# ELEKTRONN/ELEKTRONN2

Measured on AMD Instinct MI355X. Metric: training_input_voxels_per_sec, higher is better.
Workload: dtype f32; 1 GPU; neuro3d_lite (1,1,23,183,183)->(1,2,10,37,37) fwd+bwd+Adam, 1 sample/GPU; parallelism=dp1, hipgraph=True, steps_per_launch=10

## Files before the change

### elektronn2_amd/backend.py

```python
from __future__ import annotations

import ctypes as C
import os
from typing import Optional, Sequence

import numpy as np
import torch

_HERE = os.path.dirname(os.path.abspath(__file__))
LIB_PATH = os.environ.get("E2HIP_LIB") or os.path.join(_HERE, "libe2hip.so")

ACT = {"lin": 0, "linear": 0, "relu": 1, "tanh": 2, "sigmoid": 3, "sig": 3, "logistic": 3,
       "abs": 4, "elu": 5, "selu": 6, "soft+": 7}


class E2Error(RuntimeError):
    pass


POOL_MODE = {'avg': 1, 'sum': 2}


class Tensor5(C.Structure):
    _fields_ = [("ptr", C.c_void_p),
                ("n", C.c_int32), ("c", C.c_int32), ("d", C.c_int32),
                ("h", C.c_int32), ("w", C.c_int32),
                ("sn", C.c_int64), ("sc", C.c_int64), ("sd", C.c_int64),
                ("sh", C.c_int64)]


class Bf16Dst(C.Structure):
    _fields_ = [("cl", C.c_void_p), ("cl_kg", C.c_int32), ("cl_d", C.c_int32), ("cl_h", C.c_int32),
                ("cl_w", C.c_int32), ("cl_oz", C.c_int32), ("cl_oy", C.c_int32), ("cl_ox", C.c_int32),
                ("pl", C.c_void_p), ("pl_plane", C.c_int64), ("pl_pitch", C.c_int32)]


def bf16_dst(cl=None, cl_dims=None, cl_off=(0, 0, 0), pl=None, pl_plane=0, pl_pitch=0):
    d = Bf16Dst()
    d.cl = cl.data_ptr() if cl is not None else None
    if cl is not None:
        d.cl_kg, d.cl_d, d.cl_h, d.cl_w = (int(v) for v in cl_dims)
        d.cl_oz, d.cl_oy, d.cl_ox = (int(v) for v in cl_off)
    d.pl = pl.data_ptr() if pl is not None else None
    d.pl_plane, d.pl_pitch = int(pl_plane), int(pl_pitch)
    return d


class NllWeights(C.Structure):
    _fields_ = [("class_w", C.c_void_p), ("example_w", C.POINTER(Tensor5)),
                ("labelled", C.c_void_p), ("not_present", C.c_void_p)]


class LossTerm(C.Structure):
    _fields_ = [("kind", C.c_int), ("margin", C.c_void_p), ("scale_correction", C.c_void_p),
                ("subtract_label_entropy", C.c_int), ("sig_is_log", C.c_int)]


LOSS = {"squared": 0, "abs": 1, "binary_nll": 2, "gauss_nll": 3}
MAX_LOSS_TERMS = 8


def t5_shape(shape):
    n, c, d, h, w = (int(v) for v in shape)
    return Tensor5(None, n, c, d, h, w, c * d * h * w, d * h * w, h * w, w)


def _load():
    if not os.path.exists(LIB_PATH):
        raise E2Error(
            "libe2hip.so not found at %s -- build it with "
            "`python -c 'import __graft_entry__ as g; g.build()'` or "
            "`make -C elektronn2_amd/csrc`.  There is no CPU fallback." % LIB_PATH)
    lib = C.CDLL(LIB_PATH)
    P5 = C.POINTER(Tensor5)
    PW = C.POINTER(NllWeights)
    PL = C.POINTER(LossTerm)
    vp, i, sz, fp = C.c_void_p, C.c_int, C.c_size_t, C.c_void_p
    sig = {
        "e2_ctx_create": (C.c_int, [i, C.POINTER(vp)]),
        "e2_ctx_destroy": (C.c_int, [vp]),
        "e2_ctx_set_stream": (C.c_int, [vp, vp]),
        "e2_last_error": (C.c_char_p, []),
        "e2_version": (C.c_int, []),
        "e2_conv3d_workspace_bytes": (sz, [i, i, i, i, i]),
        "e2_conv3d_fwd": (C.c_int, [vp, P5, fp, i, i, i, i, P5, vp, sz]),
        "e2_conv3d_dgrad": (C.c_int, [vp, P5, fp, i, i, i, i, P5, vp, sz]),
        "e2_conv3d_pack": (C.c_int, [vp, fp, i, i, i, i, i, i, vp, sz]),
        "e2_conv3d_fwd_packed": (C.c_int, [vp, P5, vp, i, i, i, i, P5]),
        "e2_conv3d_dgrad_packed": (C.c_int, [vp, P5, vp, i, i, i, i, P5]),
        "e2_conv3d_fwd_packed_act": (C.c_int, [vp, P5, vp, i, i, i, i, fp, i, P5]),
        "e2_bias_act_bwd_out": (C.c_int, [vp, P5, P5, i, P5, fp]),
        "e2_conv3d_dgrad_packed_actbwd": (C.c_int, [vp, P5, vp, i, i, i, i, P5, i, fp, P5, i, i, i, fp]),
        "e2_conv3d_wgrad": (C.c_int, [vp, P5, P5, fp, i, i, i]),
        "e2_conv3d_wgrad_acc": (C.c_int, [vp, P5, P5, fp, i, i, i]),
        "e2_conv3d_wgrad_pad": (C.c_int, [vp, P5, P5, fp, i, i, i, i]),
        "e2_pack_job_bytes": (sz, []),
        "e2_pack_job_fill": (C.c_int, [vp, fp, vp, i, i, i, i, i, i]),
        "e2_pack_job_set_rows": (C.c_int, [vp, i]),
        "e2_pack_job_set_stride": (C.c_int, [vp, i]),
        "e2_set_image_rows": (C.c_int, [vp, i]),
        "e2_conv3d_pack_multi": (C.c_int, [vp, vp, i]),
        "e2_conv3d_pack_multi_ex": (C.c_int, [vp, vp, i, i]),
        "e2_head_supported": (C.c_int, [i, i]),
        "e2_head_fwd": (C.c_int, [vp, P5, fp, fp, i, P5, P5, fp]),
        "e2_head_bwd_workspace_bytes": (C.c_size_t, [i, i, i, i, i, i]),
        "e2_tail_supported": (C.c_int, [i, i, i]),
        "e2_tail_workspace_bytes": (C.c_size_t, [i, i, i, i, i, i, i]),
        "e2_tail_fwd_bwd": (C.c_int, [vp, P5, fp, fp, fp, i, fp, fp, i, P5, P5, P5, P5, i, P5, fp, fp,
                                      C.c_void_p, C.c_size_t, C.POINTER(C.c_int)]),
        "e2_tail_reduce": (C.c_int, [vp, C.c_void_p, i, i, i, fp, fp, fp, fp, fp, i, fp]),
        "e2_head_bwd": (C.c_int, [vp, P5, fp, P5, P5, fp, P5, i, fp, fp, fp, C.c_void_p,
                                  C.c_size_t]),
        "e2_malis_loss_weights": (C.c_int, [i, C.c_void_p, i, C.c_void_p, C.c_void_p,
                                            C.c_void_p, i, C.c_void_p]),
        "e2_malis_connected_components": (C.c_int, [i, i, C.c_void_p, C.c_void_p, C.c_void_p,
                                                    i, C.c_void_p]),
        "e2_warp_slice": (C.c_int, [vp, P5, C.POINTER(C.c_float), i, C.c_uint,
                                    C.POINTER(C.c_int), C.POINTER(C.c_float), P5]),
        "e2_grey_augment": (C.c_int, [vp, fp, C.c_size_t, C.c_float, C.c_float, C.c_float]),
        "e2_stream_fork": (C.c_int, [vp, C.c_void_p]),
        "e2_stream_join": (C.c_int, [vp, C.c_void_p]),
        "e2_conv1_supported": (C.c_int, [i, i, i, i, i, i, i]),
        "e2_conv1_pool_act_fwd": (C.c_int, [vp, P5, fp, fp, i, i, i, i, i, i, P5]),
        "e2_conv1_bwd_workspace_bytes": (C.c_size_t, [i, i, i, i, i, i, i]),
        "e2_conv1_pool_act_bwd": (C.c_int, [vp, P5, fp, fp, P5, i, i, i, i, i, fp, fp,
                                            C.c_void_p, C.c_size_t]),
        "e2_pool_bias_act_fwd": (C.c_int, [vp, P5, fp, i, i, i, i, P5]),
        "e2_conv3d_fwd_packed_parts": (C.c_int, [vp, P5, vp, i, i, i, i, P5, C.c_int64, i,
                                                 C.POINTER(C.c_int)]),
        "e2_conv3d_dgrad_packed_parts": (C.c_int, [vp, P5, vp, i, i, i, i, P5, C.c_int64, i,
                                                   C.POINTER(C.c_int)]),
        "e2_pool_bias_act_fwd_parts": (C.c_int, [vp, P5, C.c_int64, i, fp, i, i, i, i, P5]),
        "e2_pool_bias_act_bwd_parts": (C.c_int, [vp, P5, C.c_int64, i, P5, fp, i, i, i, i, P5, fp]),
        "e2_bias_act_bwd_out_parts": (C.c_int, [vp, P5, C.c_int64, i, P5, i, P5, fp]),
        "e2_pool_bias_act_bwd": (C.c_int, [vp, P5, P5, fp, i, i, i, i, P5, fp]),
        "e2_maxpool3d_fwd": (C.c_int, [vp, P5, i, i, i, P5]),
        "e2_maxpool3d_bwd": (C.c_int, [vp, P5, P5, i, i, i, P5, i]),
        "e2_pool3d_lin_fwd": (C.c_int, [vp, P5, i, i, i, i, i, i, i, P5]),
        "e2_pool3d_lin_bwd": (C.c_int, [vp, P5, i, i, i, i, i, i, i, P5, i]),
        "e2_upconv3d_workspace_bytes": (sz, [i, i, i, i, i, i, i, i, i]),
        "e2_upconv3d_fwd": (C.c_int, [vp, P5, fp, fp, i, i, i, i, i, P5, vp, sz]),
        "e2_upconv3d_bwd": (C.c_int, [vp, P5, fp, P5, P5, i, i, i, i, P5, fp, fp, vp, sz]),
        "e2_upconv3d_image_bytes": (sz, [i, i, i, i, i]),
        "e2_upconv3d_fwd_packed": (C.c_int, [vp, P5, fp, fp, i, i, i, i, i, P5]),
        "e2_upconv3d_bwd_packed": (C.c_int, [vp, P5, fp, P5, P5, i, i, i, i, P5, fp, fp, vp, sz, i]),
        "e2_transpose_ncdhw_to_ndhwc": (C.c_int, [vp, P5, fp]),
        "e2_transpose_ndhwc_to_ncdhw": (C.c_int, [vp, fp, P5]),
        "e2_copy5": (C.c_int, [vp, P5, P5, i]),
        "e2_set_dgrad_zinset": (C.c_int, [vp, i]),
        "e2_pad5": (C.c_int, [vp, P5, P5, i, i, i, C.c_float, i]),
        "e2_fill": (C.c_int, [vp, fp, sz, C.c_float]),
        "e2_softmax_nll_fwd": (C.c_int, [vp, P5, P5, P5, fp]),
        "e2_softmax_nll_bwd": (C.c_int, [vp, P5, P5, fp, P5, fp]),
        "e2_softmax_nll_fwd_w": (C.c_int, [vp, P5, P5, P5, fp, PW]),
        "e2_softmax_nll_bwd_w": (C.c_int, [vp, P5, P5, fp, P5, fp, PW]),
        "e2_softmax_nll_grouped_fwd": (C.c_int, [vp, P5, P5, P5, i, fp]),
        "e2_softmax_nll_grouped_bwd": (C.c_int, [vp, P5, P5, i, fp, P5, fp]),
        "e2_head_fwd_w": (C.c_int, [vp, P5, fp, fp, i, P5, P5, fp, PW]),
        "e2_head_bwd_w": (C.c_int, [vp, P5, fp, P5, P5, fp, P5, i, fp, fp, fp, C.c_void_p,
                                    sz, PW]),
        "e2_tail_fwd_bwd_w": (C.c_int, [vp, P5, fp, fp, fp, i, fp, fp, i, P5, P5, P5, P5, i, P5,
                                        fp, fp, C.c_void_p, sz, C.POINTER(C.c_int), PW]),
        "e2_malis_nll": (C.c_int, [vp, P5, fp, fp, fp, P5, fp]),
        "e2_fill_multi": (C.c_int, [vp, vp, vp, C.c_int, C.c_float]),
        "e2_set_skip_zero_fill": (C.c_int, [vp, C.c_int]),
        "e2_set_input_slack": (C.c_int, [vp, C.c_int]),
        "e2_conv_last_zero_fill": (C.c_int, [vp, C.POINTER(C.c_void_p), C.POINTER(C.c_size_t)]),
        "e2_set_mfma_dtype": (C.c_int, [vp, C.c_int]),
        "e2_set_tiling": (C.c_int, [vp, C.c_int, C.c_char_p]),
        "e2_last_launch": (C.c_int, [vp, C.c_char_p, C.c_int]),
        "e2_tiling_fallbacks": (C.c_uint, [vp]),
        "e2_conv3d_bf16_workspace_bytes": (sz, [i, i, i, i, i, i, i, i, i]),
        "e2_conv3d_fwd_bf16": (C.c_int, [vp, P5, fp, i, i, i, i, fp, i, P5, vp, sz]),
        "e2_conv3d_dgrad_bf16": (C.c_int, [vp, P5, fp, i, i, i, i, P5, vp, sz]),
        "e2_conv3d_wgrad_bf16_workspace_bytes": (sz, [i, i, i, i, i, i, i, i, i]),
        "e2_conv3d_wgrad_bf16": (C.c_int, [vp, P5, P5, fp, i, i, i, i, vp, sz]),
        "e2_conv3d_bf16_xkeep_bytes": (sz, [i, i, i, i, i, i, i]),
        "e2_conv3d_fwd_bf16_keep": (C.c_int, [vp, P5, fp, i, i, i, i, fp, i, P5, vp, sz, vp, sz]),
        "e2_conv3d_wgrad_bf16_xcl": (C.c_int, [vp, P5, vp, i, P5, fp, i, i, i, i, vp, sz]),
        "e2_pool_bias_act_bwd_bf16": (C.c_int, [vp, P5, C.c_int64, i, P5, fp, i, i, i, i, P5, fp, C.POINTER(Bf16Dst)]),
        "e2_pool_bias_act_fwd_bf16": (C.c_int, [vp, P5, C.c_int64, i, fp, i, i, i, i, P5, C.POINTER(Bf16Dst)]),
        "e2_conv1_pool_act_fwd_bf16": (C.c_int, [vp, P5, fp, fp, i, i, i, i, i, i, P5, vp, i]),
        "e2_conv3d_bf16_wb_bytes": (sz, [i, i, i, i, i, i, i, i, i]),
        "e2_bf16_wjob_bytes": (sz, []),
        "e2_bf16_wjob_fill": (C.c_int, [vp, fp, i, i, i, i, i, i, i, i, i, i, vp, sz]),
        "e2_conv3d_bf16_pack_w_multi": (C.c_int, [vp, vp, i]),
        "e2_conv3d_fwd_bf16_ex": (C.c_int, [vp, P5, fp, i, i, i, i, fp, i, P5, vp, sz, vp, sz, i, vp, vp, i]),
        "e2_conv3d_dgrad_bf16_ex": (C.c_int, [vp, P5, fp, i, i, i, i, P5, vp, sz, vp, vp]),
        "e2_conv3d_wgrad_bf16_geometry": (C.c_int, [i, i, i, i, i, i, i, i, i, C.POINTER(C.c_int64),
                                                    C.POINTER(C.c_size_t), C.POINTER(C.c_size_t)]),
        "e2_conv3d_wgrad_bf16_ex": (C.c_int, [vp, P5, vp, i, P5, vp, fp, fp, i, i, i, i, vp, sz]),
        "e2_dense_fwd": (C.c_int, [vp, fp, fp, fp, i, i, i]),
        "e2_dense_dgrad": (C.c_int, [vp, fp, fp, fp, i, i, i, i]),
        "e2_dense_wgrad": (C.c_int, [vp, fp, fp, fp, i, i, i, i]),
        "e2_batchnorm_act_fwd": (C.c_int, [vp, P5, fp, fp, fp, fp, i, i, i, P5, fp]),
        "e2_batchnorm_act_bwd": (C.c_int, [vp, P5, P5, fp, fp, fp, i, i, P5, fp, fp]),
        "e2_get_mfma_dtype": (C.c_int, [vp]),
        "e2_dropout_fwd": (C.c_int, [vp, P5, P5, i, fp, vp, C.c_uint32]),
        "e2_dropout_bwd": (C.c_int, [vp, P5, P5, i, fp, vp, C.c_uint32]),
        "e2_dropout_tick": (C.c_int, [vp, vp]),
        "e2_act_fwd": (C.c_int, [vp, P5, fp, i, P5]),
        "e2_act_bwd": (C.c_int, [vp, P5, P5, fp, i, P5, fp]),
        "e2_loss_partials": (sz, [vp, P5]),
        "e2_loss_fwd": (C.c_int, [vp, PL, P5, P5, P5, fp]),
        "e2_loss_mix": (C.c_int, [vp, i, PL, C.POINTER(C.c_void_p), C.POINTER(sz),
                                  C.POINTER(C.c_int64), fp, fp, fp, fp, fp]),
        "e2_loss_bwd": (C.c_int, [vp, PL, P5, P5, P5, fp, P5, P5, i]),
        "e2_adam_step": (C.c_int, [vp, fp, fp, fp, fp, sz, vp, fp, i, fp]),
        "e2_sgd_step": (C.c_int, [vp, fp, fp, fp, sz, vp, fp, i, fp]),
        "e2_set_loss_grad_mode": (C.c_int, [vp, i, fp]),
        "e2_upd_job_bytes": (sz, []),
        "e2_upd_rest_bytes": (sz, []),
        "e2_upd_job_fill": (C.c_int, [vp, C.c_long, vp, vp, i, i, i, i, i, C.c_float, i,
                                      C.POINTER(C.c_int), C.POINTER(C.c_size_t)]),
        "e2_upd_rest_fill": (C.c_int, [vp, C.c_long, C.c_long, C.c_float]),
        "e2_adam_pack_step": (C.c_int, [vp, fp, fp, fp, fp, vp, i, i, vp, i, fp, fp, C.c_float, i, sz]),
        "e2_adam_step_ex": (C.c_int, [vp, fp, fp, fp, fp, sz, vp, fp, i, fp, fp, C.c_float, i]),
        "e2_sgd_step_ex": (C.c_int, [vp, fp, fp, fp, sz, vp, fp, i, fp, fp, C.c_float, i]),
        "e2_step_prologue": (C.c_int, [vp, fp, i, C.c_size_t, fp, fp, i, fp, i, vp]),
        "e2_graph_begin": (C.c_int, [vp]),
        "e2_graph_end": (C.c_int, [vp, C.POINTER(vp)]),
        "e2_graph_launch": (C.c_int, [vp, vp]),
        "e2_graph_destroy": (C.c_int, [vp]),
        "e2_graph_debug_dot": (C.c_int, [vp, C.c_char_p, i]),
        "e2_event_create": (C.c_int, [C.POINTER(vp)]),
        "e2_event_record": (C.c_int, [vp, vp]),
        "e2_event_elapsed_ms": (C.c_int, [vp, vp, C.POINTER(C.c_float)]),
        "e2_event_destroy": (C.c_int, [vp]),
        "e2_stream_synchronize": (C.c_int, [vp]),
    }
    for name, (res, args) in sig.items():
        fn = getattr(lib, name)
        fn.restype = res
        fn.argtypes = args
    return lib, sorted(sig)


_lib, EXPORTED_SYMBOLS = _load()


def lib():
    return _lib


def _chk(rc: int, what: str):
    if rc != 0:
        msg = _lib.e2_last_error()
        raise E2Error("%s failed (rc=%d): %s" % (what, rc, msg.decode() if msg else "?"))


def t5(t: torch.Tensor) -> Tensor5:
    if t.dim() != 5:
        raise TypeError("expected a 5-D (b,f,z,x,y) tensor, got %s" % (tuple(t.shape),))
    if t.dtype != torch.float32:
        raise TypeError("expected float32, got %s" % t.dtype)
    if not t.is_cuda:
        raise E2Error("tensor is on %s; the HIP path needs a GPU tensor (no CPU fallback)"
                      % t.device)
    s = t.stride()
    if t.shape[4] > 1 and s[4] != 1:
        raise TypeError("innermost stride must be 1, got %s" % (s,))
    return Tensor5(t.data_ptr(), t.shape[0], t.shape[1], t.shape[2], t.shape[3],
                   t.shape[4], s[0], s[1], s[2], s[3])


def nll_weights(class_w=None, example_w=None, labelled=None, not_present=None):
    w = NllWeights()
    w._keep = (class_w, example_w, labelled, not_present)
    w.class_w = _fp(class_w)
    if example_w is not None:
        w._ew = t5(example_w)
        w.example_w = C.pointer(w._ew)
    w.labelled = _fp(labelled)
    w.not_present = _fp(not_present)
    return w


def loss_term(kind, margin=None, scale_correction=None, subtract_label_entropy=False,
              sig_is_log=False):
    if kind not in LOSS:
        raise ValueError("loss_term: unknown kind %r (one of %s)" % (kind, sorted(LOSS)))
    t = LossTerm()
    t._keep = (margin, scale_correction)
    t.kind = LOSS[kind]
    t.margin = _fp(margin)
    t.scale_correction = _fp(scale_correction)
    t.subtract_label_entropy = int(bool(subtract_label_entropy))
    t.sig_is_log = int(bool(sig_is_log))
    return t


def _fp(t: Optional[torch.Tensor]):
    if t is None:
        return None
    if t.dtype != torch.float32 or not t.is_cuda or not t.is_contiguous():
        raise TypeError("expected a contiguous float32 GPU tensor")
    return C.c_void_p(t.data_ptr())


class Context:

    def __init__(self, device: int = 0, stream: Optional[torch.cuda.Stream] = None):
        if not torch.cuda.is_available():
            raise E2Error("no GPU visible: the elektronn2_amd hot path is HIP-only")
        torch.cuda.set_device(device)
        h = C.c_void_p()
        _chk(_lib.e2_ctx_create(device, C.byref(h)), "e2_ctx_create")
        self.h = h
        self.device = torch.device("cuda", device)
        self.stream = None
        self.set_stream(stream if stream is not None else torch.cuda.current_stream(device))
        self._ws = {}

    def set_stream(self, stream: torch.cuda.Stream):
        self.stream = stream
        _chk(_lib.e2_ctx_set_stream(self.h, C.c_void_p(stream.cuda_stream)),
             "e2_ctx_set_stream")

    def stream_fork(self, side: torch.cuda.Stream):
        _chk(_lib.e2_stream_fork(self.h, C.c_void_p(side.cuda_stream)), "e2_stream_fork")

    def stream_join(self, side: torch.cuda.Stream):
        _chk(_lib.e2_stream_join(self.h, C.c_void_p(side.cuda_stream)), "e2_stream_join")

    def synchronize(self):
        _chk(_lib.e2_stream_synchronize(self.h), "e2_stream_synchronize")

    def workspace(self, key, nbytes: int) -> torch.Tensor:
        w = self._ws.get(key)
        if w is None or w.numel() * 4 < nbytes:
            w = torch.empty((nbytes + 3) // 4 + 64, dtype=torch.float32, device=self.device)
            self._ws[key] = w
        return w

    def conv_ws_bytes(self, cout, cin, k):
        return int(_lib.e2_conv3d_workspace_bytes(cout, cin, k[0], k[1], k[2]))

    def conv3d_fwd(self, x, w, y, ws=None):
        cout, cin, kd, kh, kw = w.shape
        nb = self.conv_ws_bytes(cout, cin, (kd, kh, kw))
        ws = ws if ws is not None else self.workspace("conv", nb)
        _chk(_lib.e2_conv3d_fwd(self.h, C.byref(t5(x)), _fp(w), cout, kd, kh, kw,
                                C.byref(t5(y)), C.c_void_p(ws.data_ptr()), ws.numel() * 4),
             "e2_conv3d_fwd")

    def conv3d_dgrad(self, dy_pad, w, dx, ws=None):
        cout, cin, kd, kh, kw = w.shape
        nb = self.conv_ws_bytes(cout, cin, (kd, kh, kw))
        ws = ws if ws is not None else self.workspace("conv", nb)
        _chk(_lib.e2_conv3d_dgrad(self.h, C.byref(t5(dy_pad)), _fp(w), cin, kd, kh, kw,
                                  C.byref(t5(dx)), C.c_void_p(ws.data_ptr()),
                                  ws.numel() * 4), "e2_conv3d_dgrad")

    def conv3d_pack(self, w, mode, ws):
        cout, cin, kd, kh, kw = w.shape
        _chk(_lib.e2_conv3d_pack(self.h, _fp(w), cout, cin, kd, kh, kw, mode,
                                 C.c_void_p(ws.data_ptr()), ws.numel() * 4),
             "e2_conv3d_pack")

    def conv3d_fwd_packed(self, x, wp, cout, k, y):
        _chk(_lib.e2_conv3d_fwd_packed(self.h, C.byref(t5(x)), C.c_void_p(wp.data_ptr()),
                                       cout, k[0], k[1], k[2], C.byref(t5(y))),
             "e2_conv3d_fwd_packed")

    def conv3d_dgrad_packed(self, dy_pad, wp, cin, k, dx):
        _chk(_lib.e2_conv3d_dgrad_packed(self.h, C.byref(t5(dy_pad)),
                                         C.c_void_p(wp.data_ptr()), cin, k[0], k[1], k[2],
                                         C.byref(t5(dx))), "e2_conv3d_dgrad_packed")

    def conv3d_fwd_packed_parts(self, x, wp, cout, k, y_parts):
        n = C.c_int(0)
        _chk(_lib.e2_conv3d_fwd_packed_parts(self.h, C.byref(t5(x)), C.c_void_p(wp.data_ptr()),
# ... 37 lines not shown

    def conv3d_dgrad_packed_actbwd(self, dy_pad, wp, cin, k, out_prev, act_prev, dy_pad_prev,
                                   pad_prev, dbias_prev, bias_prev=None):
        _chk(_lib.e2_conv3d_dgrad_packed_actbwd(
            self.h, C.byref(t5(dy_pad)), C.c_void_p(wp.data_ptr()), int(cin), int(k[0]),
            int(k[1]), int(k[2]), C.byref(t5(out_prev)), ACT[act_prev],
            _fp(bias_prev) if bias_prev is not None else None, C.byref(t5(dy_pad_prev)),
            int(pad_prev[0]), int(pad_prev[1]), int(pad_prev[2]),
            _fp(dbias_prev) if dbias_prev is not None else None),
            "e2_conv3d_dgrad_packed_actbwd")

    def bias_act_bwd_out(self, dout, out, act, dy, dbias):
        _chk(_lib.e2_bias_act_bwd_out(self.h, C.byref(t5(dout)), C.byref(t5(out)), ACT[act],
                                      C.byref(t5(dy)), _fp(dbias)), "e2_bias_act_bwd_out")

    def warp_slice(self, src, minv, perspective, nearest_mask, dest_off, src_off, dst):
        m = (C.c_float * 16)(*[float(v) for v in np.asarray(minv, np.float32).ravel()])
        do = (C.c_int * 3)(*[int(v) for v in dest_off])
        so = (C.c_float * 3)(*[float(v) for v in src_off])
        _chk(_lib.e2_warp_slice(self.h, C.byref(t5(src[None])), m, 1 if perspective else 0,
                                int(nearest_mask), do, so, C.byref(t5(dst[None]))),
             "e2_warp_slice")

    def grey_augment(self, chan, alpha, c, gamma):
        if not chan.is_contiguous():
            raise TypeError("grey_augment needs a dense channel")
        _chk(_lib.e2_grey_augment(self.h, _fp(chan), chan.numel(), float(alpha), float(c),
                                  float(gamma)), "e2_grey_augment")

    @staticmethod
    def head_supported(cin, ncls):
        return bool(_lib.e2_head_supported(int(cin), int(ncls)))

    def head_fwd(self, x, w, bias, target, probs, stats, weights=None):
        args = (self.h, C.byref(t5(x)), _fp(w), _fp(bias), probs.shape[1],
                C.byref(t5(target)) if target is not None else None,
                C.byref(t5(probs)), _fp(stats) if stats is not None else None)
        if weights is None:
            _chk(_lib.e2_head_fwd(*args), "e2_head_fwd")
        else:
            _chk(_lib.e2_head_fwd_w(*(args + (C.byref(weights),))), "e2_head_fwd_w")

    @staticmethod
    def head_bwd_ws_bytes(x_shape, ncls):
        n, cin, d, h, w = (int(v) for v in x_shape)
        return int(_lib.e2_head_bwd_workspace_bytes(n, cin, int(ncls), d, h, w))

    def head_bwd(self, x, w, probs, target, stats, dx, accumulate_dx, dw, dbias, loss_out,
                 ws=None, weights=None):
        if ws is None:
            ws = torch.empty(self.head_bwd_ws_bytes(x.shape, probs.shape[1]) // 4 + 16,
                             dtype=torch.float32, device=self.device)
        args = (self.h, C.byref(t5(x)), _fp(w), C.byref(t5(probs)),
                C.byref(t5(target)), _fp(stats),
                C.byref(t5(dx)) if dx is not None else None,
                1 if accumulate_dx else 0, _fp(dw), _fp(dbias),
                _fp(loss_out) if loss_out is not None else None,
                C.c_void_p(ws.data_ptr()), ws.numel() * 4)
        if weights is None:
            _chk(_lib.e2_head_bwd(*args), "e2_head_bwd")
        else:
            _chk(_lib.e2_head_bwd_w(*(args + (C.byref(weights),))), "e2_head_bwd_w")

    @staticmethod
    def tail_supported(c1, c2, ncls):
        return bool(_lib.e2_tail_supported(int(c1), int(c2), int(ncls)))

    @staticmethod
    def tail_ws_bytes(x_shape, c2, ncls):
        n, c1, d, h, w = (int(v) for v in x_shape)
        return int(_lib.e2_tail_workspace_bytes(n, c1, int(c2), int(ncls), d, h, w))

    def tail_fwd_bwd(self, x, wp_fwd, wp_dgrad, bias1, w_head, b_head, target, probs, dpre, dx,
                     stats, ws, gm_mode=0, gm_src=None, gm_bias=None, weights=None):
        n_slots = C.c_int(0)
        args = (self.h, C.byref(t5(x)), _fp(wp_fwd), _fp(wp_dgrad), _fp(bias1),
                dpre.shape[1], _fp(w_head), _fp(b_head), probs.shape[1],
                C.byref(t5(target)), C.byref(t5(probs)), C.byref(t5(dpre)),
                C.byref(t5(dx)) if dx is not None else None, int(gm_mode),
                C.byref(t5(gm_src)) if gm_src is not None else None,
                _fp(gm_bias), _fp(stats),
                C.c_void_p(ws.data_ptr()), ws.numel() * 4, C.byref(n_slots))
        if weights is None:
            _chk(_lib.e2_tail_fwd_bwd(*args), "e2_tail_fwd_bwd")
        else:
            _chk(_lib.e2_tail_fwd_bwd_w(*(args + (C.byref(weights),))), "e2_tail_fwd_bwd_w")
        return int(n_slots.value)

    def tail_reduce(self, ws, n_slots, c2, ncls, dw_head, db_head, db1, stats, loss_out,
                    db_parent=None):
        _chk(_lib.e2_tail_reduce(self.h, C.c_void_p(ws.data_ptr()), int(n_slots), int(c2),
                                 int(ncls), _fp(dw_head), _fp(db_head), _fp(db1), _fp(stats),
                                 _fp(loss_out) if loss_out is not None else None,
                                 0 if db_parent is None else int(db_parent.numel()),
                                 _fp(db_parent)), "e2_tail_reduce")

    def conv3d_wgrad(self, x, dy, dw, accumulate=False):
        kd, kh, kw = dw.shape[2:]
        fn = _lib.e2_conv3d_wgrad_acc if accumulate else _lib.e2_conv3d_wgrad
        _chk(fn(self.h, C.byref(t5(x)), C.byref(t5(dy)), _fp(dw), kd, kh, kw),
             "e2_conv3d_wgrad")

    def conv3d_wgrad_pad(self, x, dy_pad, dw, accumulate=False):
        kd, kh, kw = dw.shape[2:]
        _chk(_lib.e2_conv3d_wgrad_pad(self.h, C.byref(t5(x)), C.byref(t5(dy_pad)), _fp(dw),
                                      kd, kh, kw, 1 if accumulate else 0),
             "e2_conv3d_wgrad_pad")

    def set_image_rows(self, rows):
        _chk(_lib.e2_set_image_rows(self.h, int(rows or 0)), "e2_set_image_rows")

    def make_pack_jobs(self, jobs, rows=None, strides=None):
        rec = int(_lib.e2_pack_job_bytes())
        buf = (C.c_char * (rec * len(jobs)))()
        for n, (w, wp, mode) in enumerate(jobs):
            cout, cin, kd, kh, kw = w.shape
            _chk(_lib.e2_pack_job_fill(C.byref(buf, n * rec), _fp(w), C.c_void_p(wp.data_ptr()),
                                       cout, cin, kd, kh, kw, mode), "e2_pack_job_fill")
            if strides is not None and strides[n]:
                _chk(_lib.e2_pack_job_set_stride(C.byref(buf, n * rec), int(strides[n])), "e2_pack_job_set_stride")
            if rows is not None and rows[n]:
                _chk(_lib.e2_pack_job_set_rows(C.byref(buf, n * rec), int(rows[n])), "e2_pack_job_set_rows")
        host = torch.frombuffer(bytearray(buf), dtype=torch.uint8)
        dev = host.to(self.device)
        dev.max_taps = max(int(w.shape[2] * w.shape[3] * w.shape[4]) for w, _, _ in jobs)
        dev.keep = [(w, wp) for w, wp, _ in jobs]
        return dev, len(jobs)

    def conv3d_pack_multi(self, jobs_dev, njobs):
        _chk(_lib.e2_conv3d_pack_multi_ex(self.h, C.c_void_p(jobs_dev.data_ptr()), njobs,
                                          int(getattr(jobs_dev, 'max_taps', 248))),
             "e2_conv3d_pack_multi_ex")

    @staticmethod
    def conv1_supported(cin, k, pool):
        return bool(_lib.e2_conv1_supported(cin, k[0], k[1], k[2], pool[0], pool[1], pool[2]))

    def conv1_pool_act_fwd(self, x, w, bias, pool, act, out):
        _chk(_lib.e2_conv1_pool_act_fwd(self.h, C.byref(t5(x)), _fp(w), _fp(bias), w.shape[0],
                                        w.shape[3], w.shape[4], pool[1], pool[2], ACT[act],
                                        C.byref(t5(out))), "e2_conv1_pool_act_fwd")

    def conv1_pool_act_fwd_bf16(self, x, w, bias, pool, act, out, next_xb, next_kg):
        _chk(_lib.e2_conv1_pool_act_fwd_bf16(self.h, C.byref(t5(x)), _fp(w), _fp(bias), w.shape[0],
                                             w.shape[3], w.shape[4], pool[1], pool[2], ACT[act],
                                             C.byref(t5(out)), C.c_void_p(next_xb.data_ptr()),
                                             int(next_kg)), "e2_conv1_pool_act_fwd_bf16")

    @staticmethod
    def conv1_bwd_ws_bytes(dout_shape, k):
        n, cout, d, ho, wo = (int(v) for v in dout_shape)
        return int(_lib.e2_conv1_bwd_workspace_bytes(n, cout, d, ho, wo, k[1], k[2]))

    def conv1_pool_act_bwd(self, x, w, bias, dout, pool, act, dw, dbias, ws=None):
        if ws is None:
            ws = torch.empty(self.conv1_bwd_ws_bytes(dout.shape, w.shape[2:]) // 4 + 16,
                             dtype=torch.float32, device=self.device)
        _chk(_lib.e2_conv1_pool_act_bwd(self.h, C.byref(t5(x)), _fp(w), _fp(bias),
                                        C.byref(t5(dout)), w.shape[3], w.shape[4], pool[1],
                                        pool[2], ACT[act], _fp(dw), _fp(dbias),
                                        C.c_void_p(ws.data_ptr()), ws.numel() * 4),
             "e2_conv1_pool_act_bwd")

    def pool_bias_act_fwd(self, y, bias, pool, act, out):
        _chk(_lib.e2_pool_bias_act_fwd(self.h, C.byref(t5(y)), _fp(bias), pool[0], pool[1],
                                       pool[2], ACT[act], C.byref(t5(out))),
             "e2_pool_bias_act_fwd")

    def pool_bias_act_bwd(self, dout, y, bias, pool, act, dy, dbias):
        _chk(_lib.e2_pool_bias_act_bwd(self.h, C.byref(t5(dout)), C.byref(t5(y)), _fp(bias),
                                       pool[0], pool[1], pool[2], ACT[act], C.byref(t5(dy)),
                                       _fp(dbias)), "e2_pool_bias_act_bwd")

    def act_fwd(self, pre, bias, act, out):
        _chk(_lib.e2_act_fwd(self.h, C.byref(t5(pre)), _fp(bias), ACT[act], C.byref(t5(out))),
             "e2_act_fwd")

    def loss_partials(self, pred):
        n = int(_lib.e2_loss_partials(self.h, C.byref(t5(pred))))
        if n <= 0:
            raise E2Error("e2_loss_partials: empty prediction %s" % (tuple(pred.shape),))
        return n

    def loss_fwd(self, term, pred, sig, target, partials):
        if partials.numel() < 4 * self.loss_partials(pred):
            raise E2Error("loss_fwd: the partials slab is too small for this prediction")
        _chk(_lib.e2_loss_fwd(self.h, C.byref(term), C.byref(t5(pred)),
                              None if sig is None else C.byref(t5(sig)), C.byref(t5(target)),
                              _fp(partials)), "e2_loss_fwd")

    def loss_mix(self, terms, partials, n_tot, mix, coef, term_loss, count, loss_out):
        k = len(terms)
        if not (len(partials) == len(n_tot) == k):
            raise E2Error("loss_mix: %d terms, %d slabs, %d sizes" % (k, len(partials), len(n_tot)))
        if k > MAX_LOSS_TERMS:
            raise E2Error("loss_mix: %d terms, at most %d are supported" % (k, MAX_LOSS_TERMS))
        for t in (mix, coef, term_loss, count):
            if t.numel() < k:
                raise E2Error("loss_mix: mix / coef / term_loss / count need %d floats" % k)
        if loss_out.numel() < 1:
            raise E2Error("loss_mix: loss_out needs one float")
        ta = (LossTerm * max(k, 1))(*terms)
        pa = (C.c_void_p * max(k, 1))(*[_fp(p) for p in partials])
        ra = (C.c_size_t * max(k, 1))(*[int(p.numel()) // 4 for p in partials])
        na = (C.c_int64 * max(k, 1))(*[int(n) for n in n_tot])
        _chk(_lib.e2_loss_mix(self.h, k, ta, pa, ra, na, _fp(mix), _fp(coef), _fp(term_loss),
                              _fp(count), _fp(loss_out)), "e2_loss_mix")

    def loss_bwd(self, term, pred, sig, target, coef, dpred, dsig=None, accumulate=False):
        opt = lambda t: None if t is None else C.byref(t5(t))
        _chk(_lib.e2_loss_bwd(self.h, C.byref(term), C.byref(t5(pred)), opt(sig),
                              C.byref(t5(target)), _fp(coef), opt(dpred), opt(dsig),
                              int(bool(accumulate))), "e2_loss_bwd")

    def act_bwd(self, dout, pre, bias, act, dpre, dbias):
        _chk(_lib.e2_act_bwd(self.h, C.byref(t5(dout)), C.byref(t5(pre)), _fp(bias), ACT[act],
                             C.byref(t5(dpre)), _fp(dbias)), "e2_act_bwd")

    def maxpool3d_fwd(self, x, pool, out):
        _chk(_lib.e2_maxpool3d_fwd(self.h, C.byref(t5(x)), pool[0], pool[1], pool[2],
                                   C.byref(t5(out))), "e2_maxpool3d_fwd")

    def maxpool3d_bwd(self, dout, x, pool, dx, accumulate=False):
        _chk(_lib.e2_maxpool3d_bwd(self.h, C.byref(t5(dout)), C.byref(t5(x)), pool[0],
                                   pool[1], pool[2], C.byref(t5(dx)), int(accumulate)),
             "e2_maxpool3d_bwd")

    def pool_lin_fwd(self, x, pool, stride, mode, out):
        _chk(_lib.e2_pool3d_lin_fwd(self.h, C.byref(t5(x)), int(pool[0]), int(pool[1]),
                                    int(pool[2]), int(stride[0]), int(stride[1]), int(stride[2]),
                                    POOL_MODE.get(mode, mode), C.byref(t5(out))),
             "e2_pool3d_lin_fwd")

    def pool_lin_bwd(self, dout, pool, stride, mode, dx, accumulate=False):
        _chk(_lib.e2_pool3d_lin_bwd(self.h, C.byref(t5(dout)), int(pool[0]), int(pool[1]),
                                    int(pool[2]), int(stride[0]), int(stride[1]), int(stride[2]),
                                    POOL_MODE.get(mode, mode), C.byref(t5(dx)),
                                    int(bool(accumulate))), "e2_pool3d_lin_bwd")

    def upconv_ws_bytes(self, cout, cin, pool, x_shape):
        return int(_lib.e2_upconv3d_workspace_bytes(cout, cin, pool[0], pool[1], pool[2],
                                                    x_shape[0], x_shape[2], x_shape[3],
                                                    x_shape[4]))

    def upconv3d_fwd(self, x, w, bias, pool, act, y, ws=None):
        cout, cin = w.shape[:2]
        nb = self.upconv_ws_bytes(cout, cin, pool, x.shape)
        ws = ws if ws is not None else self.workspace("upconv", nb)
        _chk(_lib.e2_upconv3d_fwd(self.h, C.byref(t5(x)), _fp(w), _fp(bias), cout, pool[0],
                                  pool[1], pool[2], ACT[act], C.byref(t5(y)),
                                  C.c_void_p(ws.data_ptr()), ws.numel() * 4),
             "e2_upconv3d_fwd")

    def upconv3d_bwd(self, x, w, y, dout, pool, act, dx, dw, dbias, ws=None):
        cout, cin = w.shape[:2]
        nb = self.upconv_ws_bytes(cout, cin, pool, x.shape)
        ws = ws if ws is not None else self.workspace("upconv", nb)
        _chk(_lib.e2_upconv3d_bwd(self.h, C.byref(t5(x)), _fp(w), C.byref(t5(y)),
                                  C.byref(t5(dout)), pool[0], pool[1], pool[2], ACT[act],
                                  C.byref(t5(dx)) if dx is not None else None,
                                  _fp(dw), _fp(dbias), C.c_void_p(ws.data_ptr()),
                                  ws.numel() * 4), "e2_upconv3d_bwd")

    @staticmethod
    def upconv_image_bytes(cout, cin, pool):
        return int(_lib.e2_upconv3d_image_bytes(int(cout), int(cin), pool[0], pool[1], pool[2]))

    def upconv3d_fwd_packed(self, x, wp_fwd, bias, cout, pool, act, y):
        _chk(_lib.e2_upconv3d_fwd_packed(self.h, C.byref(t5(x)), _fp(wp_fwd), _fp(bias), int(cout),
                                         pool[0], pool[1], pool[2], ACT[act], C.byref(t5(y))),
             "e2_upconv3d_fwd_packed")

    def upconv3d_bwd_packed(self, x, wp_dgrad, y, dout, pool, act, dx, dw, dbias, ws,
                            accumulate=False):
        _chk(_lib.e2_upconv3d_bwd_packed(self.h, C.byref(t5(x)), _fp(wp_dgrad), C.byref(t5(y)),
                                         C.byref(t5(dout)), pool[0], pool[1], pool[2], ACT[act],
                                         C.byref(t5(dx)) if dx is not None else None,
                                         _fp(dw), _fp(dbias), C.c_void_p(ws.data_ptr()),
                                         ws.numel() * 4, int(bool(accumulate))),
             "e2_upconv3d_bwd_packed")

    def to_ndhwc(self, src, dst):
        _chk(_lib.e2_transpose_ncdhw_to_ndhwc(self.h, C.byref(t5(src)), _fp(dst)),
             "e2_transpose_ncdhw_to_ndhwc")

    def to_ncdhw(self, src, dst):
        _chk(_lib.e2_transpose_ndhwc_to_ncdhw(self.h, _fp(src), C.byref(t5(dst))),
             "e2_transpose_ndhwc_to_ncdhw")

    def copy5(self, src, dst, accumulate=False):
        _chk(_lib.e2_copy5(self.h, C.byref(t5(src)), C.byref(t5(dst)), int(accumulate)),
             "e2_copy5")

    def set_dgrad_zinset(self, planes):
        _chk(_lib.e2_set_dgrad_zinset(self.h, int(planes)), "e2_set_dgrad_zinset")

    def pad5(self, src, dst, pad, value=0.0, frame_only=False):
        _chk(_lib.e2_pad5(self.h, C.byref(t5(src)) if src is not None else None, C.byref(t5(dst)),
                          int(pad[0]), int(pad[1]), int(pad[2]), float(value), int(bool(frame_only))),
             "e2_pad5")

    def fill(self, t, value=0.0):
        if not t.is_contiguous():
            raise TypeError("fill needs a contiguous tensor")
        _chk(_lib.e2_fill(self.h, C.c_void_p(t.data_ptr()), t.numel(), float(value)),
             "e2_fill")

    @staticmethod
    def _drop_state(state):
        if not (isinstance(state, torch.Tensor) and state.is_cuda and state.dtype == torch.int32
                and state.numel() >= 4 and state.is_contiguous() and state.data_ptr() % 16 == 0):
            raise TypeError("dropout state: four int32 words in device memory, 16-byte aligned")
        return C.c_void_p(state.data_ptr())

    def dropout_fwd(self, x, out, rate, state, stream, feature_mode=False):
# ... 171 lines not shown
        _chk(_lib.e2_conv3d_wgrad_bf16_geometry(n, cin, d, h, w, int(cout), k[0], k[1], k[2],
                                                C.byref(pd), C.byref(db), C.byref(sb)),
             "e2_conv3d_wgrad_bf16_geometry")
        return int(pd.value), int(db.value), int(sb.value)

    def conv3d_wgrad_bf16_ex(self, x, dy, dw, accumulate=False, ws=None, xcl=None, dyc=None, sums=None):
        cout, cin, kd, kh, kw = dw.shape
        if ws is None and not (xcl is not None and dyc is not None and sums is not None):
            ws = self.workspace("wgrad_bf16", self.wgrad_bf16_ws_bytes(x.shape, cout, (kd, kh, kw)))
        _chk(_lib.e2_conv3d_wgrad_bf16_ex(
            self.h, C.byref(t5(x)), C.c_void_p(xcl.data_ptr()) if xcl is not None else None,
            (cin + 15) // 16 * 2, C.byref(t5(dy)),
            C.c_void_p(dyc.data_ptr()) if dyc is not None else None, _fp(sums), _fp(dw),
            kd, kh, kw, int(accumulate),
            C.c_void_p(ws.data_ptr()) if ws is not None else None,
            ws.numel() * ws.element_size() if ws is not None else 0), "e2_conv3d_wgrad_bf16_ex")

    def pool_bias_act_bwd_bf16(self, dout, src, bias, pool, act, dy, dbias, dst, parts=1, part_stride=0):
        dyv = t5(dy) if dy is not None else Tensor5(None, 0, 0, 0, 0, 0, 0, 0, 0, 0)
        _chk(_lib.e2_pool_bias_act_bwd_bf16(self.h, C.byref(t5(dout)), int(part_stride), int(parts),
                                            C.byref(t5(src)), _fp(bias), pool[0], pool[1], pool[2],
                                            ACT[act], C.byref(dyv), _fp(dbias), C.byref(dst)),
             "e2_pool_bias_act_bwd_bf16")

    def pool_bias_act_fwd_bf16(self, y, bias, pool, act, out, dst, parts=1, part_stride=0):
        _chk(_lib.e2_pool_bias_act_fwd_bf16(self.h, C.byref(t5(y)), int(part_stride), int(parts),
                                            _fp(bias), pool[0], pool[1], pool[2], ACT[act],
                                            C.byref(t5(out)), C.byref(dst)),
             "e2_pool_bias_act_fwd_bf16")

    def dense_fwd(self, x, w, y):
        n, k = x.shape
        _chk(_lib.e2_dense_fwd(self.h, _fp(x), _fp(w), _fp(y), n, k, w.shape[1]), "e2_dense_fwd")

    def dense_dgrad(self, dy, w, dx, accumulate=False):
        n, m = dy.shape
        _chk(_lib.e2_dense_dgrad(self.h, _fp(dy), _fp(w), _fp(dx), n, w.shape[0], m,
                                 int(accumulate)), "e2_dense_dgrad")

    def dense_wgrad(self, x, dy, dw, accumulate=False):
        n, k = x.shape
        _chk(_lib.e2_dense_wgrad(self.h, _fp(x), _fp(dy), _fp(dw), n, k, dy.shape[1],
                                 int(accumulate)), "e2_dense_wgrad")

    def batchnorm_act_fwd(self, x, gamma, bias, run_mean, run_std, train, update_running, act,
                          out, save=None):
        _chk(_lib.e2_batchnorm_act_fwd(self.h, C.byref(t5(x)), _fp(gamma), _fp(bias),
                                       _fp(run_mean), _fp(run_std), int(bool(train)),
                                       int(bool(update_running)), ACT[act], C.byref(t5(out)),
                                       _fp(save)), "e2_batchnorm_act_fwd")

    def batchnorm_act_bwd(self, dout, x, gamma, bias, save, train, act, dx, dgamma, dbias):
        _chk(_lib.e2_batchnorm_act_bwd(self.h, C.byref(t5(dout)), C.byref(t5(x)), _fp(gamma),
                                       _fp(bias), _fp(save), int(bool(train)), ACT[act],
                                       C.byref(t5(dx)) if dx is not None else None,
                                       _fp(dgamma), _fp(dbias)), "e2_batchnorm_act_bwd")

    def set_tiling(self, kind, cfg):
        code = {'igemm': 0, 'wgrad': 1}[kind]
        _chk(_lib.e2_set_tiling(self.h, code, (cfg or "").encode()), "e2_set_tiling")
        self._tiling = getattr(self, '_tiling', {})
        self._tiling[kind] = cfg or ""

    def last_launch(self):
        buf = C.create_string_buffer(160)
        _chk(_lib.e2_last_launch(self.h, buf, 160), "e2_last_launch")
        parts = buf.value.decode().split(" ")
        return tuple(parts) if len(parts) == 3 else None

    def tiling_fallbacks(self):
        return int(_lib.e2_tiling_fallbacks(self.h))

    def bf16_memory_form(self):
        return getattr(self, '_tiling', {}).get('igemm', '').startswith('32,')

    def set_mfma_dtype(self, dtype):
        code = {'f32': 0, 'float32': 0, 'bf16': 1, 'bfloat16': 1}.get(dtype)
        if code is None:
            raise ValueError("mfma dtype must be 'f32' or 'bf16', got %r" % (dtype,))
        _chk(_lib.e2_set_mfma_dtype(self.h, code), "e2_set_mfma_dtype")
        self._mfma = 'bf16' if code else 'f32'

    @property
    def mfma_dtype(self):
        m = getattr(self, '_mfma', None)
        if m is None:
            m = self._mfma = 'bf16' if _lib.e2_get_mfma_dtype(self.h) == 1 else 'f32'
        return m

    def malis_nll(self, probs, pos, neg, norm, dlogits, loss_sum):
        _chk(_lib.e2_malis_nll(self.h, C.byref(t5(probs)), _fp(pos), _fp(neg), _fp(norm),
                               C.byref(t5(dlogits)) if dlogits is not None else None,
                               _fp(loss_sum)), "e2_malis_nll")

    def set_loss_grad_mode(self, sum_mode, count_out=None):
        _chk(_lib.e2_set_loss_grad_mode(self.h, int(bool(sum_mode)), _fp(count_out)),
             "e2_set_loss_grad_mode")

    def adam_step(self, p, g, m, s, seg_off, seg_reg, hyper, gdiv=None, gmul=1.0, zero_g=False):
        _chk(_lib.e2_adam_step_ex(self.h, _fp(p), _fp(g), _fp(m), _fp(s), p.numel(),
                                  C.c_void_p(seg_off.data_ptr()), _fp(seg_reg),
                                  seg_reg.numel(), _fp(hyper), _fp(gdiv), float(gmul),
                                  int(bool(zero_g))), "e2_adam_step_ex")

    def make_upd_jobs(self, jobs, rests):
        rj, rr = int(_lib.e2_upd_job_bytes()), int(_lib.e2_upd_rest_bytes())
        bj = (C.c_char * max(rj * len(jobs), 1))()
        br = (C.c_char * max(rr * len(rests), 1))()
        tile0, lds = 0, 16
        keep = []
        for n, (off, wf, wd_, shape, reg) in enumerate(jobs):
            nt, lb = C.c_int(), C.c_size_t()
            cout, cin, kd, kh, kw = (int(v) for v in shape)
            _chk(_lib.e2_upd_job_fill(C.byref(bj, n * rj), int(off),
                                      C.c_void_p(wf.data_ptr()) if wf is not None else None,
                                      C.c_void_p(wd_.data_ptr()) if wd_ is not None else None,
                                      cout, cin, kd, kh, kw, float(reg), tile0, C.byref(nt), C.byref(lb)),
                 "e2_upd_job_fill")
            tile0 += nt.value
            lds = max(lds, int(lb.value))
            keep += [wf, wd_]
        for n, (off, cnt, reg) in enumerate(rests):
            _chk(_lib.e2_upd_rest_fill(C.byref(br, n * rr), int(off), int(cnt), float(reg)), "e2_upd_rest_fill")
        return dict(jobs=torch.frombuffer(bytearray(bj), dtype=torch.uint8).to(self.device), njobs=len(jobs),
                    ntiles=tile0, rest=torch.frombuffer(bytearray(br), dtype=torch.uint8).to(self.device),
                    nrest=len(rests), lds=lds, keep=keep)

    def adam_pack_step(self, p, g, m, s, upd, hyper, gdiv=None, gmul=1.0, zero_g=False):
        _chk(_lib.e2_adam_pack_step(self.h, _fp(p), _fp(g), _fp(m), _fp(s),
                                    C.c_void_p(upd['jobs'].data_ptr()), upd['njobs'], upd['ntiles'],
                                    C.c_void_p(upd['rest'].data_ptr()), upd['nrest'], _fp(hyper),
                                    _fp(gdiv), float(gmul), int(bool(zero_g)), upd['lds']),
             "e2_adam_pack_step")

    def sgd_step(self, p, g, d, seg_off, seg_reg, hyper, gdiv=None, gmul=1.0, zero_g=False):
        _chk(_lib.e2_sgd_step_ex(self.h, _fp(p), _fp(g), _fp(d), p.numel(),
                                 C.c_void_p(seg_off.data_ptr()), _fp(seg_reg),
                                 seg_reg.numel(), _fp(hyper), _fp(gdiv), float(gmul),
                                 int(bool(zero_g))), "e2_sgd_step_ex")

    def step_prologue(self, state, ring=None, dst=None, src=None, hist=None):
        assert state.dtype == torch.int64 and state.numel() >= 2 and state.is_contiguous()
        if ring is not None:
            assert ring.dim() == 2 and ring.is_contiguous() and ring.dtype == torch.float32
            assert dst is not None and dst.is_contiguous() and dst.numel() >= ring.shape[1]
        if hist is not None:
            assert hist.dim() == 2 and hist.is_contiguous() and src is not None and src.numel() >= hist.shape[1]
        _chk(_lib.e2_step_prologue(self.h, _fp(ring), int(ring.shape[0]) if ring is not None else 0,
                                   int(ring.shape[1]) if ring is not None else 0, _fp(dst), _fp(src),
                                   int(hist.shape[1]) if hist is not None else 0, _fp(hist),
                                   int(hist.shape[0]) if hist is not None else 0,
                                   C.c_void_p(state.data_ptr())), "e2_step_prologue")

    def graph_begin(self):
        _chk(_lib.e2_graph_begin(self.h), "e2_graph_begin")

    def graph_end(self):
        g = C.c_void_p()
        _chk(_lib.e2_graph_end(self.h, C.byref(g)), "e2_graph_end")
        return g

    def graph_launch(self, g):
        _chk(_lib.e2_graph_launch(self.h, g), "e2_graph_launch")

    def graph_destroy(self, g):
        _chk(_lib.e2_graph_destroy(g), "e2_graph_destroy")

    def graph_debug_dot(self, g, path, verbose=True):
        _chk(_lib.e2_graph_debug_dot(g, str(path).encode(), 1 if verbose else 0), "e2_graph_debug_dot")

    def event(self):
        e = C.c_void_p()
        _chk(_lib.e2_event_create(C.byref(e)), "e2_event_create")
        return e

    def record(self, e):
        _chk(_lib.e2_event_record(self.h, e), "e2_event_record")

    def elapsed_ms(self, e0, e1) -> float:
        ms = C.c_float()
        _chk(_lib.e2_event_elapsed_ms(e0, e1, C.byref(ms)), "e2_event_elapsed_ms")
        return float(ms.value)
```

### elektronn2_amd/csrc/conv_first.hip

```cpp
#include "common.hpp"
#include <algorithm>

struct First {
  const float* x;
  const float* w;
  const float* bias;
  float* out;
  const float* dout;
  float* dw;
  float* dbias;
  int N, Cout, D, Ho, Wo;
  long xsN, xsD, xsH;
  long osN, osC, osD, osH;
  int act;
  int tilesX, tilesY;
};

template <int KH, int KW, int PY, int PX>
__device__ __forceinline__ float first_conv(const float (&win)[PY + KH - 1][PX + KW - 1],
                                            const float* __restrict__ wc, int a, int b) {
  float s = 0.f;
#pragma unroll
  for (int ty = 0; ty < KH; ++ty)
#pragma unroll
// ... 100 lines not shown
      for (int i = 0; i < 16; ++i) {
        const int t = t0 + i;
        float acc = 0.f;
        if (t < T) {
          const int ty = t / KW, tx = t % KW;
#pragma unroll
          for (int a = 0; a < PY; ++a)
#pragma unroll
            for (int b = 0; b < PX; ++b)
              acc = fmaf((c[a][b] == m) ? g : 0.f, win[a + ty][b + tx], acc);
        }
        v[i] = acc;
      }
      ff_butterfly16(v, lane);
      const int l15 = lane & 15;
      const int tap = t0 + ((l15 & 1) << 3 | (l15 & 2) << 1 | (l15 & 4) >> 1 | (l15 & 8) >> 3);
      if (tap < T) rb[grp][tap] = v[0];
    }
    float gs = g;
#pragma unroll
    for (int o = 8; o > 0; o >>= 1) gs += __shfl_xor(gs, o, 64);
    if ((lane & 15) == 0) rb[grp][T] = gs;
    __syncthreads();
    if (threadIdx.x <= T) {
      float sum = 0.f;
#pragma unroll
      for (int k = 0; k < 16; ++k) sum += rb[k][threadIdx.x];
      part[((long)tile * p.Cout + co) * (T + 1) + threadIdx.x] = sum;
    }
  }
}

__global__ __launch_bounds__(256) void first_bwd_reduce_kernel(const float* __restrict__ part,
                                                               int nTiles, int Cout, int T,
                                                               float* dw, float* dbias) {
  const int per = (nTiles + gridDim.y - 1) / gridDim.y;
  const int t0 = blockIdx.y * per, t1 = min(t0 + per, nTiles);
  const int idx = blockIdx.x * blockDim.x + threadIdx.x;
  const int total = Cout * (T + 1);
  if (idx >= total) return;
  float s = 0.f;
  for (int t = t0; t < t1; ++t) s += part[(long)t * total + idx];
  const int co = idx / (T + 1), k = idx - co * (T + 1);
  if (s != 0.f) {
    if (k < T) unsafeAtomicAdd(dw + co * T + (T - 1 - k), s);
    else unsafeAtomicAdd(dbias + co, s);
  }
}

__global__ __launch_bounds__(256) void first_bwd_reduce_sm_kernel(const float* __restrict__ part,
                                                                  int nSlots, int Cout, int T,
                                                                  float* dw, float* dbias) {
  const int idx = blockIdx.x * 4 + (threadIdx.x >> 6), lane = threadIdx.x & 63;
  if (idx >= Cout * (T + 1)) return;
  const float* row = part + (long)idx * nSlots;
  float s = 0.f;
#pragma unroll 4
  for (int b = lane; b < nSlots; b += 64) s += row[b];
#pragma unroll
  for (int o = 32; o > 0; o >>= 1) s += __shfl_xor(s, o, 64);
  if (lane != 0) return;
  const int co = idx / (T + 1), k = idx - co * (T + 1);
  if (k < T) dw[co * T + (T - 1 - k)] += s;
  else dbias[co] += s;
}

int e2i_firstm_mg(int cout);
size_t e2i_firstm_ws_floats(long nTiles, int cout, int T);
int e2i_firstm_fwd(e2_ctx*, int v, const e2_tensor5* x, const float* w, const float* bias, int cout,
                   int py, int px, int act, const e2_tensor5* out, void* next_xb, int next_kg);
int e2i_firstm_bwd(e2_ctx*, int v, const e2_tensor5* x, const float* w, const float* bias,
                   const e2_tensor5* dout, int py, int px, int act, float* part, int* nslots);

static int first_supported(int kd, int kh, int kw, int pz, int py, int px) {
  if (kd != 1 || pz != 1) return 0;
  if (kh == 4 && kw == 4 && py == 2 && px == 2) return 1;
  if (kh == 6 && kw == 6 && py == 2 && px == 2) return 2;
  if (kh == 3 && kw == 3 && py == 1 && px == 1) return 3;
  return 0;
}

extern "C" int e2_conv1_supported(int cin, int kd, int kh, int kw, int pz, int py, int px) {
  return cin == 1 && first_supported(kd, kh, kw, pz, py, px) != 0;
}

static int first_fill(First& p, const e2_tensor5* x, const e2_tensor5* o, int cout, int kh,
                      int kw, int py, int px, const char* name) {
  E2_REQUIRE(x && x->ptr && o && o->ptr, "%s: null tensor", name);
  E2_REQUIRE(x->c == 1, "%s: needs exactly one input channel", name);
  E2_REQUIRE(o->n == x->n && o->c == cout && o->d == x->d &&
                 o->h == (x->h - kh + 1) / py && o->w == (x->w - kw + 1) / px &&
                 (x->h - kh + 1) % py == 0 && (x->w - kw + 1) % px == 0,
             "%s: pooled output is (%d,%d,%d,%d,%d), input (%d,1,%d,%d,%d), kernel %dx%d pool %dx%d",
             name, o->n, o->c, o->d, o->h, o->w, x->n, x->d, x->h, x->w, kh, kw, py, px);
  p.x = x->ptr;
  p.N = x->n; p.Cout = cout; p.D = x->d; p.Ho = o->h; p.Wo = o->w;
  p.xsN = x->sn; p.xsD = x->sd; p.xsH = x->sh;
  p.osN = o->sn; p.osC = o->sc; p.osD = o->sd; p.osH = o->sh;
  p.tilesX = e2_cdiv(o->w, 32);
  p.tilesY = e2_cdiv(o->h, 8);
  return 0;
}

static int conv1_fwd(e2_ctx* ctx, const e2_tensor5* x, const float* w, const float* bias, int cout,
                     int kh, int kw, int py, int px, int act, const e2_tensor5* out, void* next_xb,
                     int next_kg);

extern "C" int e2_conv1_pool_act_fwd(e2_ctx* ctx, const e2_tensor5* x, const float* w,
                                     const float* bias, int cout, int kh, int kw, int py,
                                     int px, int act, const e2_tensor5* out) {
  return conv1_fwd(ctx, x, w, bias, cout, kh, kw, py, px, act, out, nullptr, 0);
}

extern "C" int e2_conv1_pool_act_fwd_bf16(e2_ctx* ctx, const e2_tensor5* x, const float* w,
                                          const float* bias, int cout, int kh, int kw, int py,
                                          int px, int act, const e2_tensor5* out, void* next_xb,
                                          int next_kg) {
  E2_REQUIRE(next_xb, "conv1_pool_act_fwd_bf16: null copy");
  return conv1_fwd(ctx, x, w, bias, cout, kh, kw, py, px, act, out, next_xb, next_kg);
}

static int conv1_fwd(e2_ctx* ctx, const e2_tensor5* x, const float* w, const float* bias, int cout,
                     int kh, int kw, int py, int px, int act, const e2_tensor5* out, void* next_xb,
                     int next_kg) {
  E2_REQUIRE(ctx && w && bias, "conv1_pool_act_fwd: null argument");
  const int v = first_supported(1, kh, kw, 1, py, px);
  E2_REQUIRE(v, "conv1_pool_act_fwd: unsupported kernel/pool %dx%d / %dx%d", kh, kw, py, px);
  First p{};
  if (int rc = first_fill(p, x, out, cout, kh, kw, py, px, "conv1_pool_act_fwd")) return rc;
  p.w = w; p.bias = bias; p.out = out->ptr; p.act = act;
  if (e2i_firstm_mg(cout) && (next_xb || !e2_dbg_env("E2_FIRST_VALU")))
    return e2i_firstm_fwd(ctx, v, x, w, bias, cout, py, px, act, out, next_xb, next_kg);
  E2_REQUIRE(!next_xb, "conv1_pool_act_fwd_bf16: %d output channels (matrix-core form: <= 32)", cout);
  const long nTiles = (long)p.N * p.D * p.tilesY * p.tilesX;
  const int grid = (int)std::min<long>(nTiles, ctx->num_cu * 8);
  if (v == 1)
    hipLaunchKernelGGL((first_fwd_kernel<4, 4, 2, 2>), dim3(grid), dim3(256), 0, ctx->stream, p, (int)nTiles);
  else if (v == 2)
    hipLaunchKernelGGL((first_fwd_kernel<6, 6, 2, 2>), dim3(grid), dim3(256), 0, ctx->stream, p, (int)nTiles);
  else
    hipLaunchKernelGGL((first_fwd_kernel<3, 3, 1, 1>), dim3(grid), dim3(256), 0, ctx->stream, p, (int)nTiles);
  E2_CHECK_HIP(hipGetLastError());
  return 0;
}

extern "C" size_t e2_conv1_bwd_workspace_bytes(int n, int cout, int d, int ho, int wo, int kh,
                                               int kw) {
  const long tiles = (long)n * d * e2_cdiv(ho, 8) * e2_cdiv(wo, 32);
  const long tilesM = (long)n * d * e2_cdiv(ho, 4) * e2_cdiv(wo * 2, 64);
  const size_t valu = (size_t)tiles * cout * (kh * kw + 1);
  return sizeof(float) * std::max(valu, e2i_firstm_ws_floats(tilesM, cout, kh * kw));
}

extern "C" int e2_conv1_pool_act_bwd(e2_ctx* ctx, const e2_tensor5* x, const float* w,
                                     const float* bias, const e2_tensor5* dout, int kh, int kw,
                                     int py, int px, int act, float* dw, float* dbias,
                                     void* ws, size_t ws_bytes) {
  E2_REQUIRE(ctx && w && bias && dw && dbias && ws, "conv1_pool_act_bwd: null argument");
  const int v = first_supported(1, kh, kw, 1, py, px);
  E2_REQUIRE(v, "conv1_pool_act_bwd: unsupported kernel/pool %dx%d / %dx%d", kh, kw, py, px);
  First p{};
  if (int rc = first_fill(p, x, dout, dout ? dout->c : 0, kh, kw, py, px, "conv1_pool_act_bwd"))
    return rc;
  p.w = w; p.bias = bias; p.dout = dout->ptr; p.dw = dw; p.dbias = dbias; p.act = act;
  const long nTiles = (long)p.N * p.D * p.tilesY * p.tilesX;
  E2_REQUIRE(nTiles < (1L << 31), "conv1_pool_act_bwd: too many tiles");
  E2_REQUIRE(ws_bytes >= e2_conv1_bwd_workspace_bytes(p.N, p.Cout, p.D, p.Ho, p.Wo, kh, kw),
             "conv1_pool_act_bwd: workspace too small");
  float* part = (float*)ws;
  if (e2i_firstm_mg(p.Cout) && !e2_dbg_env("E2_FIRST_VALU")) {
    int nslots = 0;
    if (int rc = e2i_firstm_bwd(ctx, v, x, w, bias, dout, py, px, act, part, &nslots)) return rc;
    const int T = kh * kw, total = p.Cout * (T + 1);
    hipLaunchKernelGGL(first_bwd_reduce_sm_kernel, dim3(e2_cdiv(total, 4)), dim3(256), 0, ctx->stream,
                       part, nslots, p.Cout, T, dw, dbias);
    E2_CHECK_HIP(hipGetLastError());
    return 0;
  }
  if (v == 1)
    hipLaunchKernelGGL((first_bwd_kernel<4, 4, 2, 2>), dim3((int)nTiles), dim3(256), 0, ctx->stream, p, part);
  else if (v == 2)
    hipLaunchKernelGGL((first_bwd_kernel<6, 6, 2, 2>), dim3((int)nTiles), dim3(256), 0, ctx->stream, p, part);
  else
    hipLaunchKernelGGL((first_bwd_kernel<3, 3, 1, 1>), dim3((int)nTiles), dim3(256), 0, ctx->stream, p, part);
  E2_CHECK_HIP(hipGetLastError());
  const int T = kh * kw, total = p.Cout * (T + 1);
  const int slices = (int)std::min<long>(nTiles, 64);
  hipLaunchKernelGGL(first_bwd_reduce_kernel, dim3(e2_cdiv(total, 256), slices), dim3(256), 0,
                     ctx->stream, part, (int)nTiles, p.Cout, T, dw, dbias);
  E2_CHECK_HIP(hipGetLastError());
  return 0;
}
```

### elektronn2_amd/neuromancer/loss.py

```python
from __future__ import annotations

import numpy as np

from .graphutils import TaggedShape, floatX
from .node_basic import Node, Sym
from .variables import VariableParam

__all__ = ['Softmax', 'MultinoulliNLL', 'MalisNLL', 'SquaredLoss', 'AbsLoss', 'BinaryNLL',
           'GaussianNLL', 'AggregateLoss', 'Classification', 'Errors']

MAX_LOSS_TERMS = 8

EPS = 1e-5


class Softmax(Node):
    def __init__(self, parent, n_class='auto', n_indep=1, name="softmax", print_repr=True):
        super(Softmax, self).__init__(parent, name, print_repr)
        n_f = parent.shape['f']
        if hasattr(parent, 'activation_func'):
            if parent.activation_func != 'lin':
                raise ValueError("The parent of a Softmax-node must have a "
                                 "linear activation function.")
        if n_class == 'auto':
# ... 65 lines not shown
                parents.append(extra)
        super(MultinoulliNLL, self).__init__(parents, name, print_repr)
        if not isinstance(pred, Softmax):
            raise ValueError("The prob input to a MultinoulliNLL-node must be "
                             "a Softmax-Node.")
        if pred.n_indep != 1 and (len(parents) > 2 or cw_param is not None):
            raise NotImplementedError("MultinoulliNLL over n_indep > 1 takes the plain sparse "
                                      "target only: the other options have no defined meaning "
                                      "for several independent softmaxes")
        if weakness:
            raise NotImplementedError("weak training (weakness != 0) is outside the HIP "
                                      "hot path")
        if not target_is_sparse:
            raise NotImplementedError("dense (one-hot) targets are outside the HIP hot path")
        self.target = target
        self.pred = pred
        self.axis = pred.shape.tag2index('f')
        self.n_class = pred.n_class
        self.n_indep = pred.n_indep
        self.target_is_sparse = target_is_sparse
        k = self.n_class
        if self.n_indep != 1:
            want = tuple(self.n_indep if t == 'f' else s
                         for s, t in zip(pred.shape.shape, pred.shape.tags))
            if tuple(target.shape.tags) != tuple(pred.shape.tags) or \
                    tuple(target.shape.shape) != want:
                raise ValueError("MultinoulliNLL over %i independent softmaxes: the sparse target "
                                 "must be %s (one class id per softmax) for the prediction %s, "
                                 "got %s" % (self.n_indep, want, pred.shape, target.shape))
        if cw_param is not None:
            if cw_param.shape != (k,):
                raise ValueError("class_weights: %i values given, the prediction has %i "
                                 "classes" % (int(np.prod(cw_param.shape)), k))
            self.params['class_weights'] = cw_param
            class_weights = cw_param
        elif class_weights is not None:
            if tuple(class_weights.shape.tags) != ('f',) or \
                    tuple(class_weights.shape.shape) != (k,):
                raise ValueError("class_weights node: an Input((%i,), 'f') is needed, got %s"
                                 % (k, class_weights.shape))
        for what, m in (('mask_class_labeled', mask_class_labeled),
                        ('mask_class_not_present', mask_class_not_present)):
            if m is not None and (tuple(m.shape.tags) != ('b', 'f') or m.shape['f'] != k
                                  or m.shape['b'] != pred.shape['b']):
                raise ValueError("%s: an Input((%r, %i), 'b,f') is needed, got %s"
                                 % (what, pred.shape['b'], k, m.shape))
        if example_weights is not None:
            tags = tuple(t for t in pred.shape.tags if t != 'f')
            shape = tuple(s for s, t in zip(pred.shape.shape, pred.shape.tags) if t != 'f')
            if tuple(example_weights.shape.tags) != tags or \
                    tuple(example_weights.shape.shape) != shape:
                raise ValueError("example_weights: an Input(%s, '%s') is needed (the target's "
                                 "shape without the class axis), got %s"
                                 % (shape, ",".join(tags), example_weights.shape))
        self.class_weights = class_weights
        self.example_weights = example_weights
        self.weakness = 0
        self.mask_class_labeled = mask_class_labeled
        self.mask_class_not_present = mask_class_not_present

    @property
    def weighted(self):
        return any(v is not None for v in (self.class_weights, self.example_weights,
                                           self.mask_class_labeled,
                                           self.mask_class_not_present))

    def _weights(self, plan):
        if not self.weighted:
            return None
        w = plan.scratch.get((self, 'weights'))
        if w is None:
            from .. import backend
            cw = self.class_weights
            if isinstance(cw, VariableParam):
                cw = plan.param(cw).reshape(-1)
            elif cw is not None:
                cw = plan.out[cw].reshape(-1)
            dev = lambda node: None if node is None else plan.out[node]
            lab, npr = dev(self.mask_class_labeled), dev(self.mask_class_not_present)
            w = backend.nll_weights(class_w=cw, example_w=dev(self.example_weights),
                                    labelled=None if lab is None else lab.reshape(lab.shape[0], -1),
                                    not_present=None if npr is None else npr.reshape(npr.shape[0], -1))
            plan.scratch[self, 'weights'] = w
        return w

    def _calc_shape(self):
        self.shape = self.parent[0].shape.updateshape(self.axis, 1)

    def _calc_comp_cost(self):
        self.computational_cost = self.parent[0].shape.stripnone_prod

    def _plan_alloc(self, plan):
        plan.scratch[self.pred, 'fused_nll'] = True
        plan.scratch[self, 'loss'] = plan.zeros_flat(1)
        head = self.pred._head(plan)
        if head is not None and plan.training and self._tail(plan) is None:
            nb = plan.ctx.head_bwd_ws_bytes(plan.out_shape(head.parent), self.n_class)
            plan.scratch[self, 'head_ws'] = plan.empty_flat(nb // 4 + 16)
        plan.out[self] = None

    def _tail(self, plan):
        head = self.pred._head(plan)
        if head is None:
            return None
        c = head.parent
        f = getattr(c, '_tail', None)
        t = f(plan) if f is not None else None
        return c if (t is not None and t[2] is self) else None

    def _plan_fwd(self, plan):
        stats = plan.scratch[self.pred, 'stats']
        tail = self._tail(plan)
        if tail is not None:
            head = self.pred._head(plan)
            par = tail.parent
            plan.join_side()
            dx = plan.grad[par] if plan.needs_grad(par) else None
            gm = tail._tail_gm(plan) if dx is not None else None
            kw = {}
            if gm is not None:
                dx = plan.scratch[par, 'dy']
                kw = dict(gm_mode=gm[0], gm_src=gm[1], gm_bias=gm[2])
            with plan.loss_grad_mode():
                plan.scratch[self, 'tail_slots'] = plan.ctx.tail_fwd_bwd(
                    plan.out[par], plan.scratch[tail, 'wp_f'], plan.scratch.get((tail, 'wp_d')),
                    plan.param(tail.b), plan.param(head.w).reshape(head.n_f, -1),
                    plan.param(head.b), plan.out[self.target], plan.out[self.pred],
                    plan.scratch[tail, 'dy'], dx, stats, plan.scratch[tail, 'tail_ws'],
                    weights=self._weights(plan), **kw)
            return
        plan.zero_early(stats)
        head = self.pred._head(plan)
        if head is not None:
            plan.ctx.head_fwd(plan.out[head.parent], plan.param(head.w), plan.param(head.b),
                              plan.out[self.target], plan.out[self.pred], stats,
                              weights=self._weights(plan))
            return
        if self.n_indep != 1:
            plan.ctx.softmax_nll_grouped_fwd(plan.out[self.pred.parent], plan.out[self.target],
                                             plan.out[self.pred], self.n_indep, stats)
            return
        plan.ctx.softmax_nll_fwd(plan.out[self.pred.parent], plan.out[self.target],
                                 plan.out[self.pred], stats, weights=self._weights(plan))

    def _plan_bwd(self, plan):
        with plan.loss_grad_mode():
            self._plan_bwd_launches(plan)

    def _plan_bwd_launches(self, plan):
        head = self.pred._head(plan)
        tail = self._tail(plan)
        if tail is not None:
            par = tail.parent
            gm = tail._tail_gm(plan) if plan.needs_grad(par) else None
            plan.ctx.tail_reduce(plan.scratch[tail, 'tail_ws'], plan.scratch[self, 'tail_slots'],
                                 tail.n_f, head.n_f, plan.pgrad(head.w).reshape(head.n_f, -1),
                                 plan.pgrad(head.b), plan.pgrad(tail.b),
                                 plan.scratch[self.pred, 'stats'], plan.scratch[self, 'loss'],
                                 db_parent=plan.pgrad(par.b) if gm is not None else None)
            return
        if head is not None:
            dst, first = (plan.grad_slot(head.parent) if plan.needs_grad(head.parent)
                          else (None, True))
            plan.ctx.head_bwd(plan.out[head.parent], plan.param(head.w), plan.out[self.pred],
                              plan.out[self.target], plan.scratch[self.pred, 'stats'], dst,
                              not first, plan.pgrad(head.w), plan.pgrad(head.b),
                              plan.scratch[self, 'loss'], ws=plan.scratch[self, 'head_ws'],
                              weights=self._weights(plan))
            return
        logits = self.pred.parent
        dst, first = plan.grad_slot(logits)
        if not first:
            raise NotImplementedError("logits consumed by several nodes")
        if self.n_indep != 1:
            plan.ctx.softmax_nll_grouped_bwd(plan.out[self.pred], plan.out[self.target],
                                             self.n_indep, plan.scratch[self.pred, 'stats'], dst,
                                             plan.scratch[self, 'loss'])
            return
        plan.ctx.softmax_nll_bwd(plan.out[self.pred], plan.out[self.target],
                                 plan.scratch[self.pred, 'stats'], dst,
                                 plan.scratch[self, 'loss'], weights=self._weights(plan))

    def loss_value(self, plan):
        s = plan.scratch[self.pred, 'stats']
        return s[0] / (s[1] + EPS)


class MalisNLL(Node):

    def __init__(self, pred, aff_gt, seg_gt, nhood, unrestrict_neg=True, class_weights=None,
                 example_weights=None, name="nll", print_repr=True):
        super(MalisNLL, self).__init__([pred, aff_gt, seg_gt], name, print_repr)
        if not isinstance(pred, Softmax):
            raise ValueError("The prob input to a MultinoulliNLL-node must be "
                             "a Softmax-Node.")
        if pred.shape['b'] != 1:
            raise NotImplementedError("Malis can only be used with batch size 1.")
        if class_weights is not None or example_weights is not None:
            raise NotImplementedError("class / example weights are outside the HIP hot path")
        if pred.n_class != 2:
            raise NotImplementedError("MalisNLL needs 2-class softmaxes (one per edge)")
        self.aff_gt = aff_gt
        self.seg_gt = seg_gt
        self.pred = pred
        self.nhood = np.asarray(nhood, dtype=np.int32)
        if self.nhood.shape != (pred.n_indep, 3):
            raise ValueError("nhood must be (%i, 3) for this prediction" % pred.n_indep)
        self.unrestrict_neg = unrestrict_neg
        self.axis = pred.shape.tag2index('f')
        self.n_class = pred.n_class
        self.n_indep = pred.n_indep
        self.class_weights = None
        self.example_weights = None
        self.rand_index = self.false_splits = self.false_merges = None
        self.pos_count = self.neg_count = None

    def _calc_shape(self):
        self.shape = self.parent[0].shape.updateshape(self.axis, 1)

    def _calc_comp_cost(self):
        self.computational_cost = self.parent[0].shape.stripnone_prod

    def _plan_alloc(self, plan):
        plan.scratch[self.pred, 'loss_writes_dlogits'] = True
        sh = plan.out_shape(self.pred)
        n = self.n_indep * int(np.prod(sh[2:]))
        plan.scratch[self, 'pos'] = plan.zeros_flat(n)
        plan.scratch[self, 'neg'] = plan.zeros_flat(n)
        plan.scratch[self, 'norm'] = plan.zeros_flat(4)
        plan.scratch[self, 'loss'] = plan.zeros_flat(1)
        plan.out[self] = None

    def _plan_fwd(self, plan):
        pass

    def _plan_host(self, plan):
        import torch
        from .. import malis
        plan.stream.synchronize()
        probs = plan.out[self.pred]
        aff = probs[0, 1::2].cpu().numpy()
        aff_gt = plan.out[self.aff_gt][0].cpu().numpy().astype(np.int16)
        seg_gt = plan.out[self.seg_gt][0, 0].cpu().numpy().astype(np.int32)
        pos, neg = malis.malis_weights(aff, aff_gt, seg_gt, self.nhood, self.unrestrict_neg)
        n_pos, n_neg = float(pos.sum(dtype=np.float64)), float(neg.sum(dtype=np.float64))
        n_tot = n_pos + n_neg
        norm = np.array([1.0 / (n_tot + EPS), n_tot, n_pos, n_neg], np.float32)
        plan.scratch[self, 'pos'].copy_(torch.from_numpy(pos.astype(np.float32).ravel()))
        plan.scratch[self, 'neg'].copy_(torch.from_numpy(neg.astype(np.float32).ravel()))
        plan.scratch[self, 'norm'].copy_(torch.from_numpy(norm))
        self.pos_count, self.neg_count = pos, neg
        self.false_splits = int(pos[aff < 0.5].sum(dtype=np.uint64))
        self.false_merges = int(neg[aff > 0.5].sum(dtype=np.uint64))
        self.rand_index = np.float32((self.false_splits + self.false_merges) / (n_tot + EPS))

    def _launch(self, plan, dlogits):
        plan.ctx.fill(plan.scratch[self, 'loss'], 0.0)
        plan.ctx.malis_nll(plan.out[self.pred], plan.scratch[self, 'pos'],
                           plan.scratch[self, 'neg'], plan.scratch[self, 'norm'], dlogits,
                           plan.scratch[self, 'loss'])

    def _plan_fwd_post(self, plan):
        if not plan.training:
            self._launch(plan, None)

    def _plan_bwd(self, plan):
        logits = self.pred.parent
        dst, first = plan.grad_slot(logits)
        if not first:
            raise NotImplementedError("logits consumed by several nodes")
        self._launch(plan, dst)

    def loss_value(self, plan):
        return plan.scratch[self, 'loss'][0]


class _ElementLoss(Node):
    kind = None

    def _check_shapes(self, pred, others):
        if 's' in pred.shape.tags:
            raise NotImplementedError("%s: the 's' sample axis is outside the HIP hot path"
                                      % type(self).__name__)
        for what, n in others:
            if tuple(n.shape.shape) != tuple(pred.shape.shape) or \
                    tuple(n.shape.tags) != tuple(pred.shape.tags):
                raise ValueError("%s: the %s must have the prediction's shape %s, got %s"
                                 % (type(self).__name__, what, pred.shape, n.shape))
        self._last_plan = None

    def _calc_comp_cost(self):
        self.computational_cost = self.parent[0].shape.stripnone_prod

    def _views(self, plan):
        return plan.out[self.pred], None, plan.out[self.target]

    def _grad_targets(self):
        return (self.pred,)

    def _term(self, plan):
        t = plan.scratch.get((self, 'term'))
        if t is None:
            from .. import backend
            dev = lambda p: None if p is None else plan.param(p).reshape(-1)
            t = backend.loss_term(self.kind, margin=dev(getattr(self, 'margin', None)),
                                  scale_correction=dev(getattr(self, 'scale_correction', None)),
# ... 266 lines not shown
```

### elektronn2_amd/neuromancer/neural.py

```python
from __future__ import annotations

import logging

import numpy as np

from .graphutils import floatX, TaggedShape
from .. import autotune
from . import bf16_ahead
from .node_basic import Node, Concat, Add, Sym
from .variables import VariableWeight, ConstantParam, VariableParam

logger = logging.getLogger('elektronn2log')

__all__ = ['Conv', 'UpConv', 'Pool', 'Crop', 'Pad', 'AutoMerge', 'UpConvMerge', 'NeuralLayer',
           'FragmentsToDense', 'Perceptron']

_PLAIN_ACTS = ('relu', 'lin', 'linear')
_HIP_ACTS = _PLAIN_ACTS + ('tanh', 'sigmoid', 'sig', 'logistic', 'abs', 'elu', 'selu', 'soft+')


def check_activation(activation_func):
    if activation_func not in _HIP_ACTS:
        raise NotImplementedError("activation_func=%r: only %s are on the HIP hot path"
                                  % (activation_func, _HIP_ACTS))
# ... 531 lines not shown
        if not any(q):
            return dyp
        D, H, W = dyp.shape[2:]
        return dyp[:, :, q[0]:D - q[0], q[1]:H - q[1], q[2]:W - q[2]]

    def _sig_wgrad(self, plan):
        x, dy = self._x(plan), plan.scratch[self, 'dy']
        return (self.n_f, self.parent.shape['f']) + tuple(self._k3) + tuple(dy.shape[2:]) + \
            (x.stride(3), dy.stride(3))

    def _need_f32_dy(self, plan):
        b = plan.bf16a.get((self, 'dy'))
        if b is not None and not b['want_f32'] and plan._dy_ready.get(self):
            raise RuntimeError("bf16 mode: the tiling of a gradient launch of %s changed after its "
                               "operands were planned as bf16 images only (re-build the plan)" % self.name)

    def _bf16_fwd(self, plan, x, out, bias=None, act='lin'):
        ctx = plan.ctx
        a = plan.bf16a.get((self, 'fwd'))
        w5 = self._w5(plan.param(self.w))
        if a is None or a['tile'] != ctx.current_tiling('igemm'):
            ctx.conv3d_fwd_bf16(x, w5, out, bias=bias, act=act, ws=plan.bf16_ws(self),
                                xkeep=plan.bf16_xkeep(self))
            return
        nx = bf16_ahead.next_image(plan, self) if bias is not None else None
        plan.ensure_wb()
        ctx.conv3d_fwd_bf16_ex(x, w5, out, bias=bias, act=act, ws=plan.bf16_ws(self),
                               xkeep=plan.bf16_xkeep(self), x_ready=plan._xb_ready.get(self, False),
                               wb=a['wb'] if plan._wb_ready else None,
                               next_xb=nx[0] if nx else None, next_kg=nx[1] if nx else 0)
        if nx:
            plan._xb_ready[nx[2]] = True

    def _plan_fwd(self, plan):
        ctx = plan.ctx
        if self._fused_head(plan) is not None:
            return
        x = self._x(plan)
        if plan.scratch.get((self, 'xf_launch')):
            ctx.pad5(plan.out[self.parent], x, self._q3)
        if self._fused_first(plan):
            nx = bf16_ahead.next_image(plan, self)
            if nx is not None:
                ctx.conv1_pool_act_fwd_bf16(x, self._w5(plan.param(self.w)), plan.param(self.b),
                                            self._p3, self.activation_func, plan.out[self], nx[0], nx[1])
                plan._xb_ready[nx[2]] = True
            else:
                ctx.conv1_pool_act_fwd(x, self._w5(plan.param(self.w)), plan.param(self.b), self._p3,
                                       self.activation_func, plan.out[self])
            return
        if self._tail(plan) is not None:
            return
        wp = plan.scratch[self, 'wp_f']
        plan.join_side()
        cin = self.parent.shape['f']
        if self._fused_act(plan):
            out = plan.out[self]
            sig = (2, self.n_f, cin) + tuple(self._k3) + tuple(out.shape[2:]) + \
                (x.stride(3),)
            def fwd_act():
                if ctx.bf16_memory_form():
                    self._bf16_fwd(plan, x, out, bias=plan.param(self.b), act=self.activation_func)
                    plan.bf16_xkeep_valid(self, True)
                else:
                    plan.bf16_xkeep_valid(self, False)
                    with plan.image(wp):
                        ctx.conv3d_fwd_packed_act(x, wp, self.n_f, self._k3, plan.param(self.b),
                                                  self.activation_func, out)
            plan.tuned('igemm', sig,
                       autotune.igemm_candidates(self.n_f, cin, self._k3,
                                                 out.shape[2:], split_k=False) +
                       plan.bf16_cands(cin), fwd_act)
            return
        y = plan.scratch[self, 'y']
        sig = (0, self.n_f, cin) + tuple(self._k3) + tuple(y.shape[2:]) + \
            (x.stride(3),)
        yp = plan.scratch[self, 'y_parts']
        got = [1]

        def fwd_plain():
            plan.bf16_xkeep_valid(self, ctx.bf16_memory_form())
            if ctx.bf16_memory_form():
                self._bf16_fwd(plan, x, y)
                got[0] = 1
            elif yp.shape[0] > 1:
                with plan.image(wp):
                    got[0] = ctx.conv3d_fwd_packed_parts(x, wp, self.n_f, self._k3, yp)
            else:
                with plan.image(wp):
                    ctx.conv3d_fwd_packed(x, wp, self.n_f, self._k3, y)
        plan.tuned('igemm', sig,
                   autotune.igemm_candidates(self.n_f, cin, self._k3, y.shape[2:]) +
                   plan.bf16_cands(cin), fwd_plain, out=y)
        y_nparts = got[0]
        if self._bn():
            lin = y
            if any(p != 1 for p in self._p3):
                if self._mfp_pool():
                    raise NotImplementedError("MFP together with batch normalisation")
                lin = plan.scratch[self, 'lin']
                ctx.maxpool3d_fwd(y, self._p3, lin)
            train = self.batch_normalisation == 'train'
            pre = plan.scratch.get((self, 'pre'), plan.out[self])
            ctx.batchnorm_act_fwd(lin, plan.param(self.gamma), plan.param(self.b),
                                  plan.param(self.mean), plan.param(self.std), train,
                                  train and plan.step in ('SGD', 'Adam'), self._lin_act(),
                                  pre, plan.scratch[self, 'bn_save'])
            if not self._plain_act():
                ctx.act_fwd(pre, None, self.activation_func, plan.out[self])
            return
        if self._mfp_pool():
            from itertools import product
            out, n_in = plan.out[self], y.shape[0]
            pz, px, py = self._p3
            D, H, W = y.shape[2:]
            for i, (iz, ix, iy) in enumerate(product(range(pz), range(px), range(py))):
                src = y[:, :, iz:iz + D - pz + 1, ix:ix + H - px + 1, iy:iy + W - py + 1]
                ctx.pool_bias_act_fwd(src, plan.param(self.b), self._p3,
                                      self._lin_act(), out[i * n_in:(i + 1) * n_in])
            if not self._plain_act():
                ctx.act_fwd(out, None, self.activation_func, out)
            return
        if not self._plain_act():
            out = plan.out[self]
            if all(p == 1 for p in self._p3):
                ctx.act_fwd(y, plan.param(self.b), self.activation_func, out)
            elif (self, 'lin') in plan.scratch:
                ctx.maxpool3d_fwd(y, self._p3, plan.scratch[self, 'lin'])
                ctx.act_fwd(plan.scratch[self, 'lin'], plan.param(self.b), self.activation_func, out)
            else:
                ctx.pool_bias_act_fwd(y, plan.param(self.b), self._p3, 'lin', out)
                ctx.act_fwd(out, None, self.activation_func, out)
            return
        ndst = bf16_ahead.next_dst(plan, self)
        if ndst is not None:
            ctx.pool_bias_act_fwd_bf16(yp[0], plan.param(self.b), self._p3, self.activation_func,
                                       plan.out[self], ndst, parts=y_nparts, part_stride=yp.stride(0))
            plan._xb_ready[plan.bf16a[self, 'next']['consumer']] = True
        elif y_nparts > 1:
            ctx.pool_bias_act_fwd_parts(yp, y_nparts, plan.param(self.b), self._p3,
                                        self.activation_func, plan.out[self])
        else:
            ctx.pool_bias_act_fwd(y, plan.param(self.b), self._p3, self.activation_func,
                                  plan.out[self])

    def _plan_bwd(self, plan):
        ctx = plan.ctx
        if self._fused_head(plan) is not None:
            return
        x = self._x(plan)
        if self._fused_first(plan):
            if plan.opt['side_join_first']:
                plan.join_side()
            ctx.conv1_pool_act_bwd(x, self._w5(plan.param(self.w)), plan.param(self.b), plan.grad[self],
                                   self._p3, self.activation_func, plan.pgrad(self.w),
                                   plan.pgrad(self.b), ws=plan.scratch[self, 'ws1'])
            return
        dy = plan.scratch[self, 'dy']
        tail = self._tail(plan) is not None
        if tail:
            if plan.needs_grad(self.parent):
                plan.grad_slot(self.parent)
                if self._tail_gm(plan) is not None:
                    plan.scratch[self.parent, 'dy_by_tail'] = True
        elif self._bn():
            train = self.batch_normalisation == 'train'
            pooled = any(p != 1 for p in self._p3)
            lin = plan.scratch[self, 'lin'] if pooled else plan.scratch[self, 'y']
            dlin = plan.scratch[self, 'dlin'] if pooled else dy
            if not self._plain_act():
                ctx.act_bwd(plan.grad[self], plan.scratch[self, 'pre'], None, self.activation_func,
                            plan.grad[self], None)
            ctx.batchnorm_act_bwd(plan.grad[self], lin, plan.param(self.gamma),
                                  plan.param(self.b), plan.scratch[self, 'bn_save'], train,
                                  self._lin_act(), dlin,
                                  plan.pgrad(self.gamma) if self.gamma.apply_train else None,
                                  plan.pgrad(self.b))
            if pooled:
                ctx.maxpool3d_bwd(dlin, plan.scratch[self, 'y'], self._p3, dy)
        elif not self._plain_act():
            g = plan.grad[self]
            if all(p == 1 for p in self._p3):
                ctx.act_bwd(g, plan.scratch[self, 'y'], plan.param(self.b), self.activation_func,
                            dy, plan.pgrad(self.b))
            else:
                dlin = plan.scratch[self, 'dlin']
                ctx.act_bwd(g, plan.scratch[self, 'lin'], plan.param(self.b),
                            self.activation_func, dlin, plan.pgrad(self.b))
                ctx.maxpool3d_bwd(dlin, plan.scratch[self, 'y'], self._p3, dy)
        elif plan.scratch.get((self, 'dy_done')) or plan.scratch.get((self, 'dy_by_tail')):
            pass
        elif (self, 'dy') in plan.bf16a:
            b = plan.bf16a[self, 'dy']
            gn = plan.scratch.get((self, 'grad_nparts'), 1)
            gp = plan.scratch.get((self, 'grad_parts'))
            dout = gp[0] if (gn > 1 and gp is not None) else plan.grad[self]
            fused = self._fused_act(plan)
            ctx.pool_bias_act_bwd_bf16(dout, plan.out[self] if fused else plan.scratch[self, 'y'],
                                       None if fused else plan.param(self.b), self._p3,
                                       self.activation_func, dy if b['want_f32'] else None,
                                       plan.pgrad(self.b), b['dst'], parts=gn,
                                       part_stride=gp.stride(0) if (gn > 1 and gp is not None) else 0)
            plan._dy_ready[self] = True
        elif self._fused_act(plan):
            gn = plan.scratch.get((self, 'grad_nparts'), 1)
            if gn > 1:
                ctx.bias_act_bwd_out_parts(plan.scratch[self, 'grad_parts'], gn, plan.out[self],
                                           self.activation_func, dy, plan.pgrad(self.b))
            else:
                ctx.bias_act_bwd_out(plan.grad[self], plan.out[self], self.activation_func, dy,
                                     plan.pgrad(self.b))
        else:
            gn = plan.scratch.get((self, 'grad_nparts'), 1)
            if gn > 1:
                ctx.pool_bias_act_bwd_parts(plan.scratch[self, 'grad_parts'], gn,
                                            plan.scratch[self, 'y'], plan.param(self.b),
                                            self._p3, self.activation_func, dy,
                                            plan.pgrad(self.b))
            else:
                ctx.pool_bias_act_bwd(plan.grad[self], plan.scratch[self, 'y'],
                                      plan.param(self.b), self._p3, self.activation_func, dy,
                                      plan.pgrad(self.b))
        cin = self.parent.shape['f']
        dw = self._w5(plan.pgrad(self.w))
        dyp = plan.scratch[self, 'dy_pad']
        sigw = (self.n_f, cin) + tuple(self._k3) + tuple(dy.shape[2:]) + \
            (x.stride(3), dy.stride(3))
        wcands = plan.bf16_wgrad_cands(cin, self._k3)
        wws = plan.bf16_wgrad_ws(self) if wcands else None

        def wgrad(accumulate):
            if ctx.bf16_memory_wgrad():
                aw = plan.bf16a.get((self, 'wgrad'))
                if aw is not None and plan._dy_ready.get(self) and aw['tile'] == ctx.current_tiling('wgrad'):
                    ctx.conv3d_wgrad_bf16_ex(x, dy, dw, accumulate=accumulate, ws=wws,
                                             xcl=plan.bf16_xkeep(self, only_valid=True),
                                             dyc=aw['dyc'], sums=aw['sums'])
                else:
                    self._need_f32_dy(plan)
                    ctx.conv3d_wgrad_bf16(x, dy, dw, accumulate=accumulate, ws=wws,
                                          xcl=plan.bf16_xkeep(self, only_valid=True))
            else:
                self._need_f32_dy(plan)
                ctx.conv3d_wgrad_pad(x, dyp, dw, accumulate=accumulate)
        slack = min(4 * plan.SLACK, plan.slack_behind(x))

        def wgrad_launch():
            ctx.set_input_slack(slack)
            try:
                plan.tuned('wgrad', sigw,
                           autotune.wgrad_candidates(self.n_f, cin, self._k3, dy.shape[2:]) + wcands,
                           lambda: wgrad(True), fn_tune=lambda: wgrad(False))
            finally:
                ctx.set_input_slack(0)
        plan.on_side(wgrad_launch, defer=True, force=plan.side_forced(self))
        if plan.needs_grad(self.parent) and not tail:
            wp = plan.scratch[self, 'wp_d']
            dyp = plan.scratch[self, 'dy_pad']
            par = self.parent
            if self._actbwd_into_parent(plan):
                pdyp = plan.scratch[par, 'dy_pad']
                ppad = [kk - 1 for kk in par._k3]
                if par._fused_act(plan):
                    src, pb = plan.out[par], None
                else:
                    src, pb = plan.scratch[par, 'y'], plan.param(par.b)
                osp = plan.out_shape(par)[2:]
                sig = (1, cin, self.n_f) + tuple(self._k3) + tuple(osp) + \
                    (dyp.stride(3),)
                plan._grad_written.add(id(par))
                plan.scratch[par, 'dy_done'] = True

                def launch(dbias):
                    with plan.image(wp):
                        ctx.conv3d_dgrad_packed_actbwd(dyp, wp, cin, self._k3, src,
                                                       par.activation_func, pdyp, ppad, dbias,
                                                       bias_prev=pb)
                plan.tuned('igemm', sig,
                           autotune.igemm_candidates(cin, self.n_f, self._k3, osp),
                           lambda: launch(plan.pgrad(par.b)), fn_tune=lambda: launch(None),
                           fn_once=lambda: launch(plan.pgrad(par.b)), out=pdyp)
                return
            dst, first = plan.grad_slot(self.parent)
            out = dst if first else plan.tmp_like(dst)
            gparts = plan.scratch.get((self.parent, 'grad_parts')) if first else None
            got = [1]
            sig = (1, cin, self.n_f) + tuple(self._k3) + tuple(out.shape[2:]) + \
                (dyp.stride(3),)
            dyi = self._dy_inset(plan)
            zin = self._q3[0]

            def dgrad():
                if zin:
                    ctx.set_dgrad_zinset(zin)
                try:
                    dgrad_launch()
                finally:
                    if zin:
                        ctx.set_dgrad_zinset(0)

            def dgrad_launch():
                if ctx.bf16_memory_form():
                    ad = plan.bf16a.get((self, 'dgrad'))
                    if ad is not None and plan._dy_ready.get(self) and ad['tile'] == ctx.current_tiling('igemm'):
                        plan.ensure_wb()
                        ctx.conv3d_dgrad_bf16_ex(dyi, self._w5(plan.param(self.w)), out,
                                                 ws=plan.bf16_ws(self), dy_cl=ad['cl'],
                                                 wb=ad['wb'] if plan._wb_ready else None)
                    else:
# ... 513 lines not shown
```

### elektronn2_amd/neuromancer/optimiser.py

```python
from __future__ import annotations

import numpy as np

from . import graphutils
from .variables import VariableParam

__all__ = ['Optimiser', 'SGD', 'Adam']


class Optimiser(object):
    global_lr = VariableParam(value=1, name='lr', dtype=graphutils.floatX)
    global_weight_decay = VariableParam(value=0, name='weight_decay', dtype=graphutils.floatX)
    global_mom = VariableParam(value=0.9, name='mom', dtype=graphutils.floatX)

    @classmethod
    def setlr(cls, val):
        cls.global_lr.set_value(graphutils.as_floatX(val))

    @classmethod
    def setwd(cls, val):
        cls.global_weight_decay.set_value(graphutils.as_floatX(val))

    @classmethod
    def setmom(cls, val):
# ... 61 lines not shown
    def steps(self, k, sync=True):
        plan = self.step.func
        if plan is None or not plan._built:
            raise RuntimeError("steps: run one ordinary step first (it builds the plan)")
        import torch
        plan.stream.wait_stream(torch.cuda.current_stream(plan.ctx.device))
        with torch.cuda.stream(plan.stream):
            self._ensure_state(plan)
            self._sync_hyper(plan)
        plan.keep_loss_history()
        n0 = plan._n_runs
        plan.run_steps(k)
        one = plan._n_runs - n0 == k
        if sync:
            losses = plan.loss_history(k)
            t = plan.ctx.elapsed_ms(plan._ev0, plan._ev1) * 1e-3 if one else 0.0
            self.last_exec_time = t
            self.step.last_exec_time = t
            self._steps_async = None
            return losses, t
        a = getattr(self, '_steps_async', None)
        if a is None:
            ns = plan._hist.shape[0]
            a = self._steps_async = dict(n=0, slots=[dict(
                hist=torch.empty(ns, dtype=torch.float32).pin_memory(),
                state=torch.empty(2, dtype=torch.int64).pin_memory(),
                loss=torch.empty(1, dtype=torch.float32).pin_memory(),
                ev=torch.cuda.Event(), k=0, evs=None) for _ in range(2)])
        cur, prev = a['slots'][a['n'] & 1], a['slots'][(a['n'] & 1) ^ 1]
        with torch.cuda.stream(plan.stream):
            cur['hist'].copy_(plan._hist[:, 0], non_blocking=True)
            cur['state'].copy_(plan._step_state, non_blocking=True)
            cur['loss'].copy_(plan._loss_dev().reshape(1), non_blocking=True)
            cur['ev'].record(plan.stream)
        cur['k'], cur['evs'] = k, (plan._ev0, plan._ev1) if one else None
        a['n'] += 1
        if prev['k'] == 0:
            return None, None
        prev['ev'].synchronize()
        t_cnt, ns, kk = int(prev['state'][0]), prev['hist'].numel(), prev['k']
        h = prev['hist'].numpy()
        import numpy as np
        losses = np.array([h[(t_cnt - kk + j) % ns] for j in range(kk - 1)] + [float(prev['loss'][0])], np.float32)
        t = plan.ctx.elapsed_ms(*prev['evs']) * 1e-3 if prev['evs'] else 0.0
        prev['k'] = 0
        self.last_exec_time = t
        self.step.last_exec_time = t
        return losses, t

    def _ensure_state(self, plan):
        raise NotImplementedError

    def device_update(self, plan):
        raise NotImplementedError

    def _grad_scaling(self, plan):
        kw = dict(zero_g=plan._upd_zeroes_g())
        sc = plan._dp_scale()
        if sc is not None:
            if sc[0] == 'sum':
                kw['gdiv'] = self.model.G_spare
            else:
                kw['gmul'] = sc[1]
        return kw

    def state_dict(self):
        return {}

    def load_state_dict(self, d):
        pass

    def _apply_pending_hyper(self):
        pass


class SGD(Optimiser):
    step_name = 'SGD'

    def __init__(self, *a):
        self.last_dir = None
        self._pending = None
        super(SGD, self).__init__(*a)

    def _ensure_state(self, plan):
        if self.last_dir is None:
            self.last_dir = plan.zeros_flat(max(self.model.n_train, 4))
        if self._pending is not None:
            self._apply(self._pending)
            self._pending = None

    def device_update(self, plan):
        m = self.model
        plan.ctx.sgd_step(m.P[:m.n_train] if m.n_train < m.P.numel() else m.P, m.G,
                          self.last_dir, m.seg_off, m.seg_reg, self._hyper,
                          **self._grad_scaling(plan))

    def clear_last_dir(self):
        if self.last_dir is not None:
            self.last_dir.zero_()

    def state_dict(self):
        if self.last_dir is None:
            if self._pending is not None and 'last_dir' in self._pending:
                return {'last_dir': np.array(self._pending['last_dir'], dtype=np.float32)}
            return {}
        return {'last_dir': self.last_dir.cpu().numpy()}

    def _apply(self, d):
        import torch
        if 'last_dir' in d:
            v = np.ascontiguousarray(d['last_dir'], dtype=np.float32)
            if v.size != self.last_dir.numel():
                raise ValueError("SGD state of %i elements does not fit this model (%i)"
                                 % (v.size, self.last_dir.numel()))
            self.last_dir.copy_(torch.from_numpy(v))

    def load_state_dict(self, d):
        if self.last_dir is None:
            self._pending = dict(d)
        else:
            self._apply(d)


class Adam(Optimiser):
    step_name = 'Adam'

    def __init__(self, *a):
        self.beta2 = VariableParam(value=0.999, name='beta2', dtype=graphutils.floatX)
        self.squared_accum = None
        self.momentum = None
        self._pending = None
        self._pending_t = None
        super(Adam, self).__init__(*a)
        self.meta_params['beta2'] = self.beta2

    def _beta2(self):
        return self.beta2.get_value()

    def _ensure_state(self, plan):
        if self.momentum is None:
            n = max(self.model.n_train, 4)
            self.momentum = plan.zeros_flat(n)
            self.squared_accum = plan.zeros_flat(n)
        if self._pending is not None:
            self._apply(self._pending)
            self._pending = None

    def device_update(self, plan):
        m = self.model
        if getattr(plan, '_upd', None) is not None:
            plan.ctx.adam_pack_step(m.P, m.G, self.momentum, self.squared_accum, plan._upd,
                                    self._hyper, **self._grad_scaling(plan))
            return
        plan.ctx.adam_step(m.P[:m.n_train] if m.n_train < m.P.numel() else m.P, m.G,
                           self.momentum, self.squared_accum, m.seg_off, m.seg_reg,
                           self._hyper, **self._grad_scaling(plan))

    @property
    def t(self):
        if self._hyper is None:
            return 0.0 if self._pending_t is None else float(self._pending_t)
        return float(self._hyper[4].item())

    def state_dict(self):
        if self.momentum is None:
            if self._pending is not None and 'm' in self._pending:
                return {'m': np.array(self._pending['m'], dtype=np.float32),
                        's': np.array(self._pending['s'], dtype=np.float32),
                        't': np.array(self.t)}
            return {}
        return {'m': self.momentum.cpu().numpy(), 's': self.squared_accum.cpu().numpy(),
                't': np.array(self.t)}

    def _apply(self, d):
        import torch
        if 'm' in d:
            m = np.ascontiguousarray(d['m'], dtype=np.float32)
            s = np.ascontiguousarray(d['s'], dtype=np.float32)
            if m.size != self.momentum.numel() or s.size != self.momentum.numel():
                raise ValueError("Adam state of %i elements does not fit this model (%i)"
                                 % (m.size, self.momentum.numel()))
            self.momentum.copy_(torch.from_numpy(m))
            self.squared_accum.copy_(torch.from_numpy(s))

    def _apply_pending_hyper(self):
        if self._pending_t is not None:
            self._hyper[4] = float(self._pending_t)
            self._pending_t = None

    def load_state_dict(self, d):
        if self.momentum is None:
            self._pending = {k: d[k] for k in ('m', 's') if k in d} or None
        else:
            self._apply(d)
        if 't' in d:
            self._pending_t = float(np.asarray(d['t']))
            if self._hyper is not None:
                self._apply_pending_hyper()
```

### elektronn2_amd/neuromancer/options.py

```python
import contextlib
import os


def _b(v):
    return str(v).strip().lower() not in ("0", "", "false", "off", "no")


def _tri(v):
    return None if v is None or str(v) == "" else _b(v)


SPEC = {
    "graph": ("E2_NO_GRAPH", lambda v: not _b(v), True,
              "capture the step into hipGraphs after one eager call (E2_NO_GRAPH=1 turns it off)"),
    "side_stream": ("E2_SIDE_STREAM", _tri, None,
                    "weight gradients on a second stream; None = only in bf16 mode (DESIGN finding 7)"),
    "side_join_first": ("E2_SIDE_JOIN_FIRST", _b, False,
                        "side stream on: the fused first layer's backward waits for the weight gradients on the "
                        "side stream (it runs 62 instead of 35 us beside them, VERDICT r4 weak 9) -- measured: "
                        "bf16 lite183 0.813 -> 0.821 ms, neuro3d 1.144 -> 1.149, unet132 equal: the overlap is "
                        "worth more than the slowdown; off"),
    "side_defer": ("E2_SIDE_DEFER", _b, True,
                   "side stream on: a weight gradient's launches are ISSUED behind the main stream's next "
                   "launches (same dependencies): in the captured graph the main chain then stays on one "
                   "hardware queue (DESIGN finding 54)"),
    "side_mask": ("E2_SIDE_MASK", int, 0,
                  "side stream OFF (f32 mode): bit r set = the weight gradient of the r-th conv layer (forward "
                  "order, fused first layer and head not counted) runs on the side stream all the same"),
    "side_table": ("E2_SIDE_TABLE", _b, True,
                   "side stream OFF (f32 mode): weight gradients whose problem carries a 'side|...' entry in the "
                   "tuning table run on the side stream (tools/tune_side.py measured them inside the step: "
                   "neuro3d_lite's three 200-channel layers, -1.3 % of its step; DESIGN finding 56)"),
    "debug_poison": ("E2_DEBUG_POISON", _b, False,
                     "debugging: the plan's uninitialised buffers (Plan.empty / empty_flat) start as NaN, so "
                     "that a launch reading one before its first writer shows up in the results"),
    "wb_on_side": ("E2_WB_ON_SIDE", _b, True,
                   "bf16 mode: the per-step pack of the bf16 filter rows runs on the side stream beside the "
                   "fused first layer (with the f32 image repack) instead of behind it (finding 54)"),
    "side_pack": ("E2_SIDE_PACK", _b, False, "weight repack as a parallel branch (measured slower)"),
    "fuse_actbwd": ("E2_FUSE_ACTBWD", int, 0, "relu backward in the consumer's dgrad epilogue (finding 17)"),
    "fuse_tail": ("E2_FUSE_TAIL", _b, True, "last 1x1x1 conv + head + loss in one launch (finding 33)"),
    "bf16_tail": ("E2_BF16_TAIL", _b, True,
                  "bf16 mode: the tail launch too (its two GEMMs round their operands in registers)"),
    "tail_gm": ("E2_TAIL_GM", _b, True, "the tail launch carries its parent's activation backward"),
    "upconv_packed": ("E2_UPCONV_PACKED", _b, True, "UpConv weight images packed by the plan's one repack launch"),
    "concat_alias": ("E2_CONCAT_ALIAS", _b, True, "a concat hands channel slices to parents only it consumes"),
    "pad_inplace": ("E2_PAD_INPLACE", _b, True,
                    "a 'same' / 'full' conv finds its parent's output inside its zero-framed input image "
                    "wherever the parent's producing launch writes a strided view (no pad launch); off: "
                    "every such conv pads by one e2_pad5 launch per step"),
    "zero_in_update": ("E2_ZERO_IN_UPDATE", _b, True, "the optimiser launch clears the gradient arena (finding 38)"),
    "image_stride": ("E2_IMAGE_STRIDE", _b, True,
                     "once a conv launch's tiling is known its packed weight image gets rows as long as that "
                     "tiling's tiles reach (+ 16), not the any-tiling formula (e2_set_image_rows; finding 52)"),
    "pack_rows": ("E2_PACK_ROWS", _b, False,
                  "the repack rewrites the padding rows the TUNED tiling of each launch fetches, not the "
                  "worst case over all tilings (e2_pack_job_set_rows): the repack itself 31 -> 24 us on "
                  "neuro3d, in the step -7 us (neuro3d), -13 us (unet3d_lite), +6 us (neuro3d_lite), "
                  "+-0 (unet3d) -- below the gate; off (DESIGN finding 51)"),
    "adam_pack": ("E2_ADAM_PACK", _b, False,
                  "the Adam launch writes the packed weight images (e2_adam_pack_step); measured slower "
                  "than the two launches it replaces (DESIGN finding 46): off"),
    "dp_overlap": ("E2_DP_OVERLAP", _b, True, "exchange the late layers' gradients under the early backward"),
    "dp_fused_scale": ("E2_DP_FUSED_SCALE", _b, True, "collectives only sum, the optimiser kernel normalises"),
    "bf16_ahead": ("E2_BF16_AHEAD", _b, True, "bf16 mode: producers write the GEMM operands (finding 43)"),
    "bf16_ahead_min": ("E2_BF16_AHEAD_MIN", float, 0.0,
                       "... only when this share of the GEMM launches are memory forms (round 4: 0.6, neuro3d's "
                       "11 of 25 stayed out; with the side stream on a queue of its own -- finding 54 -- engaging "
                       "them pays there too: neuro3d 0.948 -> 0.930 ms, unet3d 6.12 -> 5.84, neuro3d_lite 0.682 -> "
                       "0.640; unet3d_lite 2.44 -> 2.47 is the one that loses)"),
    "bf16_ahead_wgrad_only": ("E2_BF16_AHEAD_WGRAD_ONLY", _b, False, "... gradient images for the weight gradient alone"),
    "bf16_xkeep": ("E2_BF16_XKEEP", _b, True, "bf16 mode: the forward's channels-last copy of x serves the wgrad"),
    "bf16_wpack": ("E2_BF16_WPACK", str, "step", "'step': one filter-row pack launch per step; 'call': per launch"),
    "dense_act_gib": ("E2_DENSE_ACT_GIB", float, 48.0, "activation budget of tiled dense prediction (GiB)"),
}

_set = {}


def get(name):
    if name in _set:
        return _set[name]
    env, parse, default, _ = SPEC[name]
    v = os.environ.get(env)
    return default if v is None else parse(v)


def snapshot(overrides=None):
    d = {k: get(k) for k in SPEC}
    for k, v in (overrides or {}).items():
        if k not in SPEC:
            raise KeyError("unknown plan option %r (known: %s)" % (k, ", ".join(sorted(SPEC))))
        d[k] = v
    return d


def set_plan_options(**kw):
    reset = kw.pop("reset", ())
    for k in reset:
        _set.pop(k, None)
    for k, v in kw.items():
        if k not in SPEC:
            raise KeyError("unknown plan option %r (known: %s)" % (k, ", ".join(sorted(SPEC))))
        if v is None and k != "side_stream":
            _set.pop(k, None)
        else:
            _set[k] = v


@contextlib.contextmanager
def plan_options(**kw):
    old = dict(_set)
    try:
        set_plan_options(**kw)
        yield
    finally:
        _set.clear()
        _set.update(old)
```

### elektronn2_amd/neuromancer/plan.py

```python
from __future__ import annotations

import os

import numpy as np
import torch

from .. import backend

_ctx = None


def get_ctx():
    global _ctx
    if _ctx is None:
        import os
        from .. import parallel
        dev = parallel.local_device()
        _ctx = backend.Context(dev)
        if os.environ.get("E2_MFMA_DTYPE", "f32") not in ("f32", "float32"):
            _ctx.set_mfma_dtype(os.environ["E2_MFMA_DTYPE"])
    return _ctx


def set_mfma_dtype(dtype):
# ... 268 lines not shown
            uniq = [(p, n) for p, n in lst if ptrs.count(p) == 1]
            if len(uniq) < 2:
                continue
            dev = self.ctx.device
            jobs[seg] = (torch.tensor([p for p, _ in uniq], dtype=torch.int64, device=dev),
                         torch.tensor([n for _, n in uniq], dtype=torch.int64, device=dev),
                         len(uniq))
            self._zero_batched[seg] = set(p for p, _ in uniq)
        return jobs

    def on_side(self, fn, always=False, defer=False, force=False):
        if not (self.use_side or force or (always and self.use_side_pack)):
            return fn()
        self._flush_side()
        self.ctx.stream_fork(self.side)
        self._side_dirty = True
        if defer and self.opt['side_defer']:
            self._side_pending = fn
            return
        self._run_side(fn)

    def side_rank(self, node):
        if self._side_order is None:
            from .neural import Conv
            self._side_order = [n for n in self.nodes if type(n) is Conv and hasattr(n, '_k3')
                                and n.parent is not None and not n._fused_first(self)
                                and n._fused_head(self) is None]
        try:
            return self._side_order.index(node)
        except ValueError:
            return 1 << 30

    def side_forced(self, node):
        if self.use_side or self.opt['side_stream'] is False:
            return False
        m = int(self.opt['side_mask'])
        if m:
            r = self.side_rank(node)
            return r < 62 and bool((m >> r) & 1)
        if not self.opt['side_table']:
            return False
        from .. import autotune
        try:
            return autotune.side_flag(self.ctx, node._sig_wgrad(self))
        except Exception:
            return False

    def _run_side(self, fn):
        ctx = self.ctx
        main = ctx.stream
        ctx.set_stream(self.side)
        try:
            with torch.cuda.stream(self.side):
                fn()
        finally:
            ctx.set_stream(main)

    def _flush_side(self):
        fn, self._side_pending = self._side_pending, None
        if fn is not None:
            self._run_side(fn)

    def join_side(self):
        self._flush_side()
        if self._side_dirty:
            self.ctx.stream_join(self.side)
            self._side_dirty = False

    def grad_slot(self, node):
        first = id(node) not in self._grad_written
        self._grad_written.add(id(node))
        return self.grad[node], first

    def add_grad(self, node, src):
        if not self.needs_grad(node):
            return
        dst, first = self.grad_slot(node)
        self.ctx.copy5(src, dst, accumulate=not first)

    def add_grad_region(self, node, slicer, src):
        if not self.needs_grad(node):
            return
        dst, first = self.grad_slot(node)
        if first:
            self.zero_early(dst)
        self.ctx.copy5(src, dst[slicer], accumulate=True)

    def build(self, batch):
        self.ctx = get_ctx()
        for g in list(getattr(self, '_graphs', None) or []) + list(getattr(self, '_multi', {}).values()):
            self.ctx.graph_destroy(g)
        self._graphs = None
        self.batch = int(batch)
        self.stream = torch.cuda.Stream(device=self.ctx.device)
        self.side = torch.cuda.Stream(device=self.ctx.device)
        self._side_dirty = False
        self._side_pending = None
        self._side_order = None
        self.use_side = self.opt['side_stream'] if self.opt['side_stream'] is not None else \
            (getattr(self.ctx, 'mfma_dtype', 'f32') == 'bf16')
        self.use_side_pack = bool(self.opt['side_pack'])
        self.fuse_actbwd = int(self.opt['fuse_actbwd'])
        self.out, self.grad, self.scratch = {}, {}, {}
        self.bf16a, self._bf16_wjobs = {}, None
        self._xb_ready, self._dy_ready, self._wb_ready = {}, {}, False
        self._bf16_ahead_on = bool(self.opt['bf16_ahead'])
        self._xkeep_valid = {}
        self.pack_jobs = []
        self.pack_nodes = {}
        self._pack_rows_done = False
        self._img_stride = {}
        self.model.ensure_arena(self.ctx)
        order = dict((id(n), i) for i, n in enumerate(self.model.dropout_nodes()))
        self._drop_ordinal = dict((n, order[id(n)]) for n in self._drop_nodes)
        if self._drop_nodes:
            self.model.dropout_state_dev()
        with torch.cuda.stream(self.stream):
            offs, tot = [], 0
            for n in self.inputs:
                offs.append(tot)
                tot += (int(np.prod(self.out_shape(n))) + 3) // 4 * 4
            self.input_arena = self.empty_flat(max(tot, 4))
            self.input_slices = {}
            for n, o in zip(self.inputs, offs):
                sh = self.out_shape(n)
                self.out[n] = self.input_arena[o:o + int(np.prod(sh))].view(sh)
                self.input_slices[n] = (o, int(np.prod(sh)))
            for n in self.nodes:
                n._plan_alloc(self)
            if getattr(self.ctx, 'mfma_dtype', 'f32') == 'bf16':
                self._bf16_ws_alloc()
            self._pack_dev = self._pack_dev_up = self._upd = None
            if self.pack_jobs:
                jobs = [(self._w5(self.param(w)), wp, mode) for (w, wp, mode) in self.pack_jobs]
                self._pack_dev = self.ctx.make_pack_jobs(jobs)
                self._plan_fused_update(jobs)
        self._graphs = None
        self._segs = None
        self._segs_key = None
        self._dp_scale_mode = False
        self._seg_idx = 0
        self._zero_seen, self._zero_batched, self._zero_keep = [], {}, None
        self._capturing = False
        self._calls = 0
        self._grad_written = set()
        self._ev_pairs = [(self.ctx.event(), self.ctx.event()), (self.ctx.event(), self.ctx.event())]
        self._ev_idx = 0
        self._n_runs = 0
        self._async = None
        self._ring = None
        self._hist = None
        self._step_state = None
        self._multi = {}
        self._built = True

    @property
    def _ev0(self):
        return self._ev_pairs[self._ev_idx][0]

    @property
    def _ev1(self):
        return self._ev_pairs[self._ev_idx][1]

    def _plan_fused_update(self, jobs):
        if self.step != 'Adam' or not self.opt['adam_pack']:
            return
        m = self.model
        by_param, order, up = {}, [], []
        for (w, wp, mode), (w5, _, _) in zip(self.pack_jobs, jobs):
            if mode in (0, 1):
                if id(w) not in by_param:
                    if not getattr(w, 'apply_train', False) or id(w) not in m._slots:
                        return
                    by_param[id(w)] = [w, tuple(int(v) for v in w5.shape), None, None]
                    order.append(id(w))
                by_param[id(w)][2 + mode] = wp
            else:
                up.append((w5, wp, mode))
        if not order:
            return

        def mult(p):
            r = p.apply_reg
            return float(r) if (r and r is not True) else (1.0 if r else 0.0)
        ujobs = [(m._slots[k][0], by_param[k][2], by_param[k][3], by_param[k][1], mult(by_param[k][0]))
                 for k in order]
        rests = [(m._slots[id(p)][0], m._slots[id(p)][1], mult(p)) for p in m._param_list
                 if p.apply_train and id(p) not in by_param]
        self._upd = self.ctx.make_upd_jobs(ujobs, rests)
        self._pack_dev_up = self.ctx.make_pack_jobs(up) if up else None

    def image(self, wp):
        plan, rows = self, self._img_stride.get(id(wp), 0)

        class _I(object):
            def __enter__(self_):
                if rows:
                    plan.ctx.set_image_rows(rows)

            def __exit__(self_, *a):
                if rows:
                    plan.ctx.set_image_rows(0)
        return _I()

    @staticmethod
    def _tile_rows(tiling, m):
        if not tiling:
            return 0
        try:
            v = [int(t) for t in tiling.split(",")]
        except ValueError:
            return 0
        if len(v) == 4:
            per = 16 * v[0]
        elif len(v) == 8 and v[0] == 4:
            per = 4 * v[1] * v[5]
        elif len(v) in (3, 5) and v[0] == 1:
            per = 16 * v[1]
        elif v[0] == 32:
            per = 16
        else:
            return 0
        return -(-(-(-m // per) * per) // 32) * 32

    def _refine_pack_rows(self):
        self._pack_rows_done = True
        want_rows, want_stride = self.opt['pack_rows'], self.opt['image_stride'] and self._upd is None
        if not (want_rows or want_stride) or self._pack_dev is None:
            return
        from .. import autotune
        rows, strides, any_ = [], [], False
        self._img_stride = {}
        for (w, wp, mode) in self.pack_jobs:
            r = st = 0
            ent = self.pack_nodes.get(id(wp))
            if ent is not None:
                node, md = ent
                try:
                    if md == 0:
                        t, m = autotune.known(self.ctx, 'igemm', node._sig_fwd(self)), node.n_f
                    elif self.needs_grad(node.parent):
                        t, m = autotune.known(self.ctx, 'igemm', node._sig_dgrad(self)), node.parent.shape['f']
                    else:
                        t, m = None, 0
                    r = self._tile_rows(t, m)
                    v = [int(q) for q in t.split(",")] if t else []
                    if want_stride and r and (len(v) == 4 or (len(v) in (3, 5) and v[0] == 1)):
                        st = -(-max(r, -(-m // 16) * 16) // 16) * 16
                except Exception:
                    r = st = 0
            rows.append(r if want_rows else 0)
            strides.append(st)
            if st:
                self._img_stride[id(wp)] = st
            any_ = any_ or st > 0 or (want_rows and r > 0)
        if any_:
            jobs = [(self._w5(self.param(w)), wp, mode) for (w, wp, mode) in self.pack_jobs]
            for (w5, wp, mode), st in zip(jobs, strides):
                if st:
                    wp.zero_()
            self._pack_dev = self.ctx.make_pack_jobs(jobs, rows, strides)

    def _emit_forward(self):
        if self._upd is not None:
            if self._pack_dev_up is not None:
                self.on_side(lambda: self.ctx.conv3d_pack_multi(*self._pack_dev_up), always=True)
        self._xb_ready, self._dy_ready = {}, {}
        self._wb_ready = False
        if self._upd is None and self._pack_dev is not None:
            def packs():
                self.ctx.conv3d_pack_multi(*self._pack_dev)
                if self.use_side and self.opt['wb_on_side']:
                    self.ensure_wb()
            self.on_side(packs, always=True)
        drop = self._drop_ids
        for n in self.nodes:
            n._plan_fwd(self)
            if id(n) in drop:
                n._drop_fwd(self)
        self.join_side()

    def ensure_wb(self):
        if not self._wb_ready and self._bf16_wjobs is not None and \
                self.opt['bf16_wpack'] == "step":
            self.ctx.conv3d_bf16_pack_w_multi(*self._bf16_wjobs)
            self._wb_ready = True
        return self._wb_ready

    def _bwd_nodes(self):
        return [n for n in reversed(self.nodes)
                if id(n) in self._loss_anc and (self.needs_grad(n) or n is self.loss_node)]

    def _emit_backward(self, part=None):
        nodes = self._bwd_nodes()
        if part is not None:
            k = self._dp_cut()[0]
            nodes = nodes[:k] if part == 0 else nodes[k:]
        if part in (None, 0):
            if not self._upd_zeroes_g():
                self.zero_early(self.model.G)
            self._grad_written = set()
        drop = self._drop_ids
        for n in nodes:
            if id(n) in drop:
                n._drop_bwd(self)
            n._plan_bwd(self)
        self.join_side()

    def _dp_cut(self):
        if self._dp_cut_cache is not False:
            return self._dp_cut_cache
        self._dp_cut_cache = None
        m = self.model
        if not self.opt['dp_overlap'] or m.n_train < (1 << 16):
            return None
        nodes = self._bwd_nodes()
        last = {}
        for i, n in enumerate(nodes):
            for p in n.params.values():
                if getattr(p, 'apply_train', False) and id(p) in m._slots:
                    last[id(p)] = i
        slots = sorted(((m._slots[q][0], q) for q in last), reverse=True)
        for k in range(1, len(nodes) - 1):
            lo = m.n_train
            for off, q in slots:
                if last[q] >= k:
                    break
                lo = off
            if m.n_train - lo >= 0.75 * m.n_train:
                self._dp_cut_cache = (k, lo)
                break
        return self._dp_cut_cache

    def _labelled_count(self):
        ln = self.loss_node
        kids = ln.parent if isinstance(ln.parent, (list, tuple)) else [ln.parent]
        if len(kids) != 1 or type(kids[0]).__name__ != 'MultinoulliNLL':
            return None
        st = self.scratch.get((kids[0].pred, 'stats'))
        return None if st is None else st[1:2]

    def _emit_update(self):
        if self.step in ('Adam', 'SGD'):
            self.model.optimisers[self.step].device_update(self)

    def _upd_zeroes_g(self):
        return (self.training and self.step in ('Adam', 'SGD') and bool(self.opt['zero_in_update']))

    def _dp_key(self):
        m = self.model
        rank = (m.dp_rank(),) if self._drop_nodes else ()
        if not self.training:
            return (1,) + rank
        return (m.dp_world(), bool(getattr(m, '_dp_weighted', False)), bool(getattr(m, '_dp_force', False)),
                id(getattr(m, '_dp_group', None))) + rank

    def _dp_scale_now(self):
        if not (self.training and self.step in ('Adam', 'SGD') and self.model.dp_world() > 1
                and self.opt['dp_fused_scale'] and self.model.G.is_cuda):
            return None
        if getattr(self.model, '_dp_weighted', False):
            return ('sum',) if self._labelled_count() is not None else None
        import torch.distributed as dist
        return ('mean', 1.0 / dist.get_world_size(self.model._dp_group))

    def _dp_scale(self):
        if self._dp_scale_mode is False:
            self._dp_scale_mode = self._dp_scale_now()
        return self._dp_scale_mode

    def loss_grad_mode(self):
        plan = self

        class _M(object):
            def __enter__(self_):
                self_.on = plan._dp_scale() == ('sum',)
                if self_.on:
                    plan.ctx.set_loss_grad_mode(True, plan.model.G_spare)

            def __exit__(self_, *a):
                if self_.on:
                    plan.ctx.set_loss_grad_mode(False, None)
        return _M()

    def _segments(self):
        dp = self.training and self.step in ('Adam', 'SGD') and self.model.dp_world() > 1
        self._dp_scale_mode = self._dp_scale_now()
        host = [n for n in self.nodes if hasattr(n, '_plan_host')]
        upd = self.training and self.step in ('Adam', 'SGD')
        segs = []
        if host:
            def host_steps():
                for n in host:
                    n._plan_host(self)

            def rest():
                for n in host:
                    n._plan_fwd_post(self)
                if self.training:
                    self._emit_backward()
                    if upd and not dp:
                        self._emit_update()
            segs.append((self._emit_forward, host_steps))
            segs.append((rest, (lambda: self.model.allreduce_grads(
                self._labelled_count(), raw=self._dp_scale() is not None)) if dp else None))
            if dp:
                segs.append((self._emit_update, None))
            return segs
        cut = self._dp_cut() if dp else None
        if cut:
            n_train = self.model.G.numel()

            def seg0():
                self._emit_forward()
                self._emit_backward(0)

            def start_tail():
                self._ex = self.model.grad_exchange(self._labelled_count(),
                                                    raw=self._dp_scale() is not None)
                self._ex.start(cut[1], n_train)

            def finish():
                self._ex.start(0, cut[1])
                self._ex.finish()
            return [(seg0, start_tail), (lambda: self._emit_backward(1), finish),
                    (self._emit_update, None)]

        def whole():
            self._emit_forward()
            if self.training:
                self._emit_backward()
                if upd and not dp:
                    self._emit_update()
        segs.append((whole, (lambda: self.model.allreduce_grads(
            self._labelled_count(), raw=self._dp_scale() is not None)) if dp else None))
        if dp:
            segs.append((self._emit_update, None))
        return segs

    def _run_device(self):
        ctx = self.ctx
        key = self._dp_key()
        if self._segs is None or self._segs_key != key:
            self._segs, self._segs_key = self._segments(), key
            for g in list(self._graphs or []) + list(self._multi.values()):
                ctx.graph_destroy(g)
            self._multi = {}
            if self._graphs is not None:
                self._calls = 0
            self._graphs = None
            self._dp_cut_cache = False
        if self.training:
            if self._upd_zeroes_g() and not self.model._g_clean:
                ctx.fill(self.model.G, 0.0)
            self.model._g_clean = False
        if self._upd is not None and getattr(self.model, '_img_owner', None) is not self:
            ctx.conv3d_pack_multi(*self._pack_dev)
        if self._graphs is None:
            from . import bf16_ahead
            bf16_ahead.prepare(self)
            if self._calls >= 1 and not self._pack_rows_done:
                self._refine_pack_rows()
            elif self._calls == 0 and self._img_stride:
                self._img_stride, self._pack_rows_done = {}, False
                jobs = [(self._w5(self.param(w)), wp, mode) for (w, wp, mode) in self.pack_jobs]
                for (_, wp, _) in jobs:
                    wp.zero_()
                self._pack_dev = self.ctx.make_pack_jobs(jobs)
        capture = self.use_graph and self._calls >= 1
        if capture and self._graphs is None:
            graphs = []
            zero_jobs = self._zero_jobs()
            self._zero_keep = zero_jobs
            ctx.record(self._ev0)
            try:
                for i, (emit, after) in enumerate(self._segs):
                    self._seg_idx = i
                    self._capturing = True
                    ctx.graph_begin()
                    try:
                        self._emit_seg(i, emit, zero_jobs)
                    except BaseException:
                        self._capturing = False
                        try:
                            ctx.graph_destroy(ctx.graph_end())
                        except Exception:
                            pass
                        raise
                    g = ctx.graph_end()
                    self._capturing = False
                    graphs.append(g)
                    ctx.graph_launch(g)
                    if after is not None:
                        after()
            except BaseException:
                for g in graphs:
                    ctx.graph_destroy(g)
                raise
            self._graphs = graphs
            from .. import autotune
            autotune.save()
            ctx.record(self._ev1)
            self._calls += 1
            self.model._g_clean = self._upd_zeroes_g()
            self.model._img_owner = self if self._upd is not None else None
            return
        ctx.record(self._ev0)
        if not capture:
            self._zero_seen = []
        for i, (emit, after) in enumerate(self._segs):
            self._seg_idx = i
            if capture:
                ctx.graph_launch(self._graphs[i])
            else:
                self._emit_seg(i, emit, None)
            if after is not None:
                after()
        ctx.record(self._ev1)
        self._calls += 1
        if self.training:
            self.model._g_clean = self._upd_zeroes_g()
            if self.step in ('Adam', 'SGD'):
                self.model._img_owner = self if self._upd is not None else None

    def _emit_seg(self, i, emit, zero_jobs):
        ctx = self.ctx
        if i == 0 and self._drop_nodes:
            ctx.dropout_tick(self.model.dropout_state_dev())
        if i == 0 and (self._ring is not None or self._hist is not None):
            ctx.step_prologue(self._step_state, ring=self._ring, dst=self.input_arena,
                              src=self._loss_dev() if self._hist is not None else None, hist=self._hist)
        if zero_jobs and i in zero_jobs:
            ctx.fill_multi(*zero_jobs[i])
        emit()

    def _loss_dev(self):
        f = getattr(self.loss_node, 'loss_dev', None)
        if f is not None:
            return f(self)
        nll = self.loss_node.parent[0] if isinstance(self.loss_node.parent, (list, tuple)) \
            else self.loss_node.parent
        return self.scratch[nll, 'loss']

    def _drop_graphs(self):
        if self._graphs or self._multi:
            self.stream.synchronize()
        for g in list(self._graphs or []) + list(self._multi.values()):
            self.ctx.graph_destroy(g)
        self._graphs, self._multi = None, {}

    def set_input_ring(self, ring):
        if ring is not None:
            if not self._built:
                raise RuntimeError("set_input_ring: build the plan first (set_inputs / one step)")
            if not (isinstance(ring, torch.Tensor) and ring.is_cuda and ring.dtype == torch.float32
                    and ring.dim() == 2 and ring.is_contiguous()
                    and ring.shape[1] == self.input_arena.numel() and ring.data_ptr() % 16 == 0):
                raise ValueError("set_input_ring: a contiguous float32 device tensor (n_slots, %d) is needed"
                                 % self.input_arena.numel())
            self._ring = ring
        else:
            self._ring = None
        self._state_alloc()
        self._drop_graphs()

    def _state_alloc(self):
        if self._step_state is None:
            self._step_state = torch.zeros(2, dtype=torch.int64, device=self.ctx.device)

    def ring_position(self):
        if self._step_state is None:
            return 0
        self.stream.synchronize()
        return int(self._step_state[0].item())

    def keep_loss_history(self, n_slots=256):
        if not self.training:
            raise RuntimeError("keep_loss_history: a training plan is needed")
        if self._hist is None or self._hist.shape[0] != int(n_slots):
            self._hist = torch.zeros(int(n_slots), 1, device=self.ctx.device)
            self._state_alloc()
            self._hist_from = self.ring_position()
            self._drop_graphs()

    def loss_history(self, n):
        if self._hist is None:
            raise RuntimeError("loss_history: call keep_loss_history() before the steps")
        t = self.ring_position()
        ns = self._hist.shape[0]
        if n < 1 or n > min(t - self._hist_from, ns + 1):
            raise ValueError("loss_history: %d steps asked for, %d kept" % (n, min(t - self._hist_from, ns + 1)))
        h = self._hist[:, 0].cpu().numpy()
        out = [h[(t - n + j) % ns] for j in range(n - 1)] + [float(self._loss_dev().item())]
        return np.array(out, np.float32)

    def run_steps(self, k):
        k = int(k)
        if k < 1:
            return
        if not self.training:
            raise RuntimeError("run_steps: a training plan is needed")
        if self._hist is None:
            self.keep_loss_history()
        while k > 0 and (self._graphs is None or not self.use_graph or len(self._segs) != 1
                         or self._segs[0][1] is not None or self._segs_key != self._dp_key()):
            self.run()
            k -= 1
            if not self.use_graph or (self._segs is not None and
                                      (len(self._segs) != 1 or self._segs[0][1] is not None)):
                for _ in range(k):
                    self.run()
                return
        if k == 0:
            return
        if k == 1:
            return self.run()
        self._ev_idx ^= 1
        ctx = self.ctx
        old = ctx.stream
        ctx.set_stream(self.stream)
        try:
            with torch.cuda.stream(self.stream):
                if self._upd_zeroes_g() and not self.model._g_clean:
                    ctx.fill(self.model.G, 0.0)
                self.model._g_clean = False
                if self._upd is not None and getattr(self.model, '_img_owner', None) is not self:
                    ctx.conv3d_pack_multi(*self._pack_dev)
                g = self._multi.get(k)
                if g is None:
                    emit = self._segs[0][0]
                    self._seg_idx = 0
                    self._capturing = True
                    ctx.graph_begin()
                    try:
                        for _ in range(k):
                            self._emit_seg(0, emit, self._zero_keep)
                    except BaseException:
                        self._capturing = False
                        try:
                            ctx.graph_destroy(ctx.graph_end())
                        except Exception:
                            pass
                        raise
                    g = ctx.graph_end()
                    self._capturing = False
                    self._multi[k] = g
                ctx.record(self._ev0)
                ctx.graph_launch(g)
                ctx.record(self._ev1)
                self._calls += k
                self._n_runs += k
                self.model._g_clean = self._upd_zeroes_g()
                if self.step in ('Adam', 'SGD'):
                    self.model._img_owner = self if self._upd is not None else None
        finally:
            ctx.set_stream(old)

    def set_inputs(self, args):
        if len(args) != len(self.inputs):
            raise TypeError("%s: %i inputs required, %i were given."
                            % (self.name, len(self.inputs), len(args)))
        batch = None
        for node, a in zip(self.inputs, args):
            decl = node.shape.shape
            if len(a.shape) != len(decl):
                raise TypeError("input '%s': rank %i given, %i required"
                                % (node.name, len(a.shape), len(decl)))
            for d, (s, g) in enumerate(zip(decl, a.shape)):
                if s is None:
                    if node.shape.tags[d] == 'b':
                        batch = g if batch is None else batch
                elif int(s) != int(g):
                    raise TypeError("input '%s': shape %s given, %s required"
                                    % (node.name, tuple(a.shape), tuple(decl)))
            if node.shape.hastag('b') and decl[node.shape.tag2index('b')] is not None:
                batch = decl[node.shape.tag2index('b')] if batch is None else batch
        if batch is None:
            batch = 1
        if not self._built or batch != self.batch:
            self.build(batch)
        self.stream.wait_stream(torch.cuda.current_stream(self.ctx.device))
        with torch.cuda.stream(self.stream):
            for node, a in zip(self.inputs, args):
                dst = self.out[node]
                if isinstance(a, torch.Tensor):
                    if a.data_ptr() == dst.data_ptr():
                        continue
                    if a.is_cuda:
                        a.record_stream(self.stream)
                    dst.copy_(a.to(torch.float32).reshape(dst.shape), non_blocking=True)
                else:
                    h = torch.from_numpy(np.ascontiguousarray(a, dtype=np.float32))
                    dst.copy_(h.reshape(dst.shape), non_blocking=False)

    def run(self):
        self._ev_idx ^= 1
        self._n_runs += 1
        old = self.ctx.stream
        self.ctx.set_stream(self.stream)
        try:
            with torch.cuda.stream(self.stream):
                self._run_device()
        finally:
            self.ctx.set_stream(old)

    def fetch(self):
        self.stream.synchronize()
        self.last_device_time = self.ctx.elapsed_ms(self._ev0, self._ev1) * 1e-3
        rets = []
        with torch.cuda.stream(self.stream):
            for o in self.outputs:
                if self.training and o is self.loss_node:
                    rets.append(np.float32(self._loss_dev().item()))
                elif hasattr(o, 'host_value'):
                    rets.append(o.host_value(self))
                elif self.out.get(o) is None:
                    raise NotImplementedError("output of node %s is not materialised"
                                              % (o.name,))
                else:
                    rets.append(self.user_view(o, self.out[o]).detach().cpu().numpy().copy())
        if self.step == 'grad':
            return [g.detach().cpu().numpy().copy()
                    for g in self.model.device_grads_list()]
        return rets

    def fetch_async(self):
        if not self.training:
            raise RuntimeError("fetch_async: a training plan is needed")
        dev_loss = self._loss_dev()
        if self._async is None:
            self._async = dict(pin=[torch.empty(1, dtype=torch.float32).pin_memory() for _ in range(2)],
                               ev=[torch.cuda.Event(), torch.cuda.Event()], n=0, run=[-1, -1])
        a = self._async
        slot = a['n'] & 1
        with torch.cuda.stream(self.stream):
            a['pin'][slot].copy_(dev_loss.reshape(1), non_blocking=True)
            a['ev'][slot].record(self.stream)
        a['run'][slot] = self._n_runs
        prev = None, None
        if a['n'] > 0 and a['run'][slot ^ 1] == self._n_runs - 1:
            a['ev'][slot ^ 1].synchronize()
            e0, e1 = self._ev_pairs[self._ev_idx ^ 1]
            prev = np.float32(a['pin'][slot ^ 1].item()), self.ctx.elapsed_ms(e0, e1) * 1e-3
        a['n'] += 1
        return prev

    def __call__(self, *args):
        self.set_inputs(args)
        self.run()
        return self.fetch()

    def input_buffer(self, node, batch=1):
        if not self._built or (batch is not None and int(batch) != self.batch):
            self.build(batch)
        return self.out[node]


def _input_alloc(self, plan):
    if self not in plan.out:
        plan.out[self] = plan.empty(plan.out_shape(self))


from .node_basic import Input as _Input
_Input._plan_alloc = _input_alloc
```

### include/e2hip.h

```cpp
#ifndef E2HIP_H
#define E2HIP_H

#include <stddef.h>
#include <stdint.h>

#ifdef __cplusplus
extern "C" {
#endif

typedef struct e2_ctx e2_ctx;

typedef struct e2_tensor5 {
  float*  ptr;
  int32_t n, c, d, h, w;
  int64_t sn, sc, sd, sh;
} e2_tensor5;

enum { E2_ACT_LIN = 0, E2_ACT_RELU = 1, E2_ACT_TANH, E2_ACT_SIGMOID, E2_ACT_ABS,
       E2_ACT_ELU, E2_ACT_SELU, E2_ACT_SOFTPLUS };
enum { E2_MFMA_F32 = 0, E2_MFMA_BF16 = 1 };
enum { E2_TILING_IGEMM = 0, E2_TILING_WGRAD = 1 };

int  e2_ctx_create(int device, e2_ctx** out);
int  e2_ctx_destroy(e2_ctx* ctx);
int  e2_ctx_set_stream(e2_ctx* ctx, void* stream);
const char* e2_last_error(void);
int  e2_version(void);
int  e2_set_mfma_dtype(e2_ctx* ctx, int dtype);
int  e2_get_mfma_dtype(const e2_ctx* ctx);
int  e2_set_tiling(e2_ctx* ctx, int kind, const char* cfg);
int  e2_last_launch(e2_ctx* ctx, char* buf, int n);
unsigned e2_tiling_fallbacks(const e2_ctx* ctx);

size_t e2_conv3d_workspace_bytes(int cout, int cin, int kd, int kh, int kw);

int e2_conv3d_fwd(e2_ctx*, const e2_tensor5* x, const float* w,
                  int cout, int kd, int kh, int kw,
                  const e2_tensor5* y, void* ws, size_t ws_bytes);

int e2_conv3d_dgrad(e2_ctx*, const e2_tensor5* dy_pad, const float* w,
                    int cin, int kd, int kh, int kw,
                    const e2_tensor5* dx, void* ws, size_t ws_bytes);

int e2_conv3d_pack(e2_ctx*, const float* w, int cout, int cin, int kd, int kh,
                   int kw, int mode, void* ws, size_t ws_bytes);
int e2_conv3d_fwd_packed(e2_ctx*, const e2_tensor5* x, const void* wp, int cout,
                         int kd, int kh, int kw, const e2_tensor5* y);
int e2_conv3d_dgrad_packed(e2_ctx*, const e2_tensor5* dy_pad, const void* wp,
                           int cin, int kd, int kh, int kw, const e2_tensor5* dx);
int e2_conv3d_fwd_packed_act(e2_ctx*, const e2_tensor5* x, const void* wp, int cout,
                             int kd, int kh, int kw, const float* bias, int act,
                             const e2_tensor5* out);
int e2_bias_act_bwd_out(e2_ctx*, const e2_tensor5* dout, const e2_tensor5* out, int act,
                        const e2_tensor5* dy, float* dbias);
int e2_conv3d_dgrad_packed_actbwd(e2_ctx*, const e2_tensor5* dy_pad, const void* wp, int cin,
                                  int kd, int kh, int kw, const e2_tensor5* out_prev,
                                  int act_prev, const float* bias_prev,
                                  const e2_tensor5* dy_pad_prev, int pd, int ph, int pw,
                                  float* dbias_prev);

int e2_conv3d_wgrad(e2_ctx*, const e2_tensor5* x, const e2_tensor5* dy,
                    float* dw, int kd, int kh, int kw);
int e2_conv3d_wgrad_acc(e2_ctx*, const e2_tensor5* x, const e2_tensor5* dy,
                        float* dw, int kd, int kh, int kw);
int e2_conv3d_wgrad_pad(e2_ctx*, const e2_tensor5* x, const e2_tensor5* dy_pad,
                        float* dw, int kd, int kh, int kw, int accumulate);

size_t e2_pack_job_bytes(void);
int e2_pack_job_fill(void* rec, const float* w, void* wp, int cout, int cin,
                     int kd, int kh, int kw, int mode);
int e2_set_image_rows(e2_ctx* ctx, int rows);
int e2_pack_job_set_stride(void* rec, int rows);
int e2_pack_job_set_rows(void* rec, int rows);
int e2_conv3d_pack_multi(e2_ctx*, const void* jobs_dev, int njobs);
int e2_conv3d_pack_multi_ex(e2_ctx*, const void* jobs_dev, int njobs, int max_taps);

int e2_conv1_supported(int cin, int kd, int kh, int kw, int pz, int py, int px);
int e2_conv1_pool_act_fwd(e2_ctx*, const e2_tensor5* x, const float* w,
                          const float* bias, int cout, int kh, int kw, int py,
                          int px, int act, const e2_tensor5* out);
size_t e2_conv1_bwd_workspace_bytes(int n, int cout, int d, int ho, int wo, int kh, int kw);
int e2_conv1_pool_act_bwd(e2_ctx*, const e2_tensor5* x, const float* w,
                          const float* bias, const e2_tensor5* dout, int kh,
                          int kw, int py, int px, int act, float* dw, float* dbias,
                          void* ws, size_t ws_bytes);

int e2_conv3d_fwd_packed_parts(e2_ctx*, const e2_tensor5* x, const void* wp, int cout, int kd,
                               int kh, int kw, const e2_tensor5* y, int64_t part_stride,
                               int max_parts, int* nparts);
int e2_conv3d_dgrad_packed_parts(e2_ctx*, const e2_tensor5* dy_pad, const void* wp, int cin,
                                 int kd, int kh, int kw, const e2_tensor5* dx,
                                 int64_t part_stride, int max_parts, int* nparts);
int e2_pool_bias_act_fwd_parts(e2_ctx*, const e2_tensor5* y, int64_t part_stride, int nparts,
                               const float* bias, int pz, int py, int px, int act,
                               const e2_tensor5* out);
int e2_pool_bias_act_bwd_parts(e2_ctx*, const e2_tensor5* dout, int64_t dout_part_stride,
                               int dout_parts, const e2_tensor5* y, const float* bias, int pz,
                               int py, int px, int act, const e2_tensor5* dy, float* dbias);
int e2_bias_act_bwd_out_parts(e2_ctx*, const e2_tensor5* dout, int64_t dout_part_stride,
                              int dout_parts, const e2_tensor5* out, int act,
                              const e2_tensor5* dy, float* dbias);

int e2_pool_bias_act_fwd(e2_ctx*, const e2_tensor5* y, const float* bias,
                         int pz, int py, int px, int act,
                         const e2_tensor5* out);
int e2_pool_bias_act_bwd(e2_ctx*, const e2_tensor5* dout, const e2_tensor5* y,
                         const float* bias, int pz, int py, int px, int act,
                         const e2_tensor5* dy, float* dbias);

int e2_maxpool3d_fwd(e2_ctx*, const e2_tensor5* x, int pz, int py, int px,
                     const e2_tensor5* out);
int e2_maxpool3d_bwd(e2_ctx*, const e2_tensor5* dout, const e2_tensor5* x,
                     int pz, int py, int px, const e2_tensor5* dx,
                     int accumulate);

enum { E2_POOL_AVG = 1, E2_POOL_SUM = 2 };
int e2_pool3d_lin_fwd(e2_ctx*, const e2_tensor5* x, int pz, int py, int px, int sz, int sy,
                      int sx, int mode, const e2_tensor5* out);
int e2_pool3d_lin_bwd(e2_ctx*, const e2_tensor5* dout, int pz, int py, int px, int sz, int sy,
                      int sx, int mode, const e2_tensor5* dx, int accumulate);

size_t e2_upconv3d_workspace_bytes(int cout, int cin, int pz, int py, int px,
                                   int n, int d, int h, int w);
int e2_upconv3d_fwd(e2_ctx*, const e2_tensor5* x, const float* w,
                    const float* bias, int cout, int pz, int py, int px,
                    int act, const e2_tensor5* y, void* ws, size_t ws_bytes);
int e2_upconv3d_bwd(e2_ctx*, const e2_tensor5* x, const float* w,
                    const e2_tensor5* y, const e2_tensor5* dout,
                    int pz, int py, int px, int act,
                    const e2_tensor5* dx, float* dw, float* dbias,
                    void* ws, size_t ws_bytes);
size_t e2_upconv3d_image_bytes(int cout, int cin, int pz, int py, int px);
int e2_upconv3d_fwd_packed(e2_ctx*, const e2_tensor5* x, const float* wp_fwd,
                           const float* bias, int cout, int pz, int py, int px, int act,
                           const e2_tensor5* y);
int e2_upconv3d_bwd_packed(e2_ctx*, const e2_tensor5* x, const float* wp_dgrad,
                           const e2_tensor5* y, const e2_tensor5* dout, int pz, int py, int px,
                           int act, const e2_tensor5* dx, float* dw, float* dbias, void* ws,
                           size_t ws_bytes, int accumulate);

int e2_transpose_ncdhw_to_ndhwc(e2_ctx*, const e2_tensor5* src, float* dst);
int e2_transpose_ndhwc_to_ncdhw(e2_ctx*, const float* src, const e2_tensor5* dst);
int e2_copy5(e2_ctx*, const e2_tensor5* src, const e2_tensor5* dst,
             int accumulate);
int e2_fill(e2_ctx*, float* ptr, size_t n, float value);

int e2_pad5(e2_ctx*, const e2_tensor5* src, const e2_tensor5* dst, int pz, int py, int px,
            float value, int frame_only);

int e2_fill_multi(e2_ctx*, const void* ptrs_dev, const void* counts_dev, int nregions,
                  float value);
int e2_set_skip_zero_fill(e2_ctx*, int on);

int e2_step_prologue(e2_ctx*, const float* ring, int n_slots, size_t slot_floats, float* dst,
                     const float* src, int n_vals, float* hist, int hist_slots, void* state);
int e2_set_input_slack(e2_ctx*, int bytes);
int e2_conv_last_zero_fill(const e2_ctx*, void** ptr, size_t* n);
int e2_set_dgrad_zinset(e2_ctx*, int planes);

int e2_head_supported(int cin, int ncls);
int e2_head_fwd(e2_ctx*, const e2_tensor5* x, const float* w, const float* bias, int ncls,
                const e2_tensor5* target, const e2_tensor5* probs, float* stats);
size_t e2_head_bwd_workspace_bytes(int n, int cin, int ncls, int d, int h, int w);
int e2_head_bwd(e2_ctx*, const e2_tensor5* x, const float* w, const e2_tensor5* probs,
                const e2_tensor5* target, const float* stats, const e2_tensor5* dx,
                int accumulate_dx, float* dw, float* dbias, float* loss_out, void* ws,
                size_t ws_bytes);

int e2_tail_supported(int c1, int c2, int ncls);
size_t e2_tail_workspace_bytes(int n, int c1, int c2, int ncls, int d, int h, int w);
int e2_tail_fwd_bwd(e2_ctx*, const e2_tensor5* x, const float* wp_fwd, const float* wp_dgrad,
                    const float* bias1, int c2, const float* w_head, const float* b_head,
                    int ncls, const e2_tensor5* target, const e2_tensor5* probs,
                    const e2_tensor5* dpre, const e2_tensor5* dx, int gm_mode,
                    const e2_tensor5* gm_src, const float* gm_bias, float* stats, void* ws,
                    size_t ws_bytes, int* n_slots);
int e2_tail_reduce(e2_ctx*, const void* ws, int n_slots, int c2, int ncls, float* dw_head,
                   float* db_head, float* db1, float* stats, float* loss_out, int c1_gm,
                   float* db_parent);

int e2_softmax_nll_fwd(e2_ctx*, const e2_tensor5* logits,
                       const e2_tensor5* target, const e2_tensor5* probs,
                       float* stats);
int e2_softmax_nll_bwd(e2_ctx*, const e2_tensor5* probs,
                       const e2_tensor5* target, const float* stats,
                       const e2_tensor5* dlogits, float* loss_out);

int e2_softmax_nll_grouped_fwd(e2_ctx*, const e2_tensor5* logits, const e2_tensor5* target,
                               const e2_tensor5* probs, int n_indep, float* stats);
int e2_softmax_nll_grouped_bwd(e2_ctx*, const e2_tensor5* probs, const e2_tensor5* target,
                               int n_indep, const float* stats, const e2_tensor5* dlogits,
                               float* loss_out);

typedef struct e2_nll_weights {
  const float*      class_w;
  const e2_tensor5* example_w;
  const float*      labelled;
  const float*      not_present;
} e2_nll_weights;
int e2_softmax_nll_fwd_w(e2_ctx*, const e2_tensor5* logits, const e2_tensor5* target,
                         const e2_tensor5* probs, float* stats, const e2_nll_weights* wts);
int e2_softmax_nll_bwd_w(e2_ctx*, const e2_tensor5* probs, const e2_tensor5* target,
                         const float* stats, const e2_tensor5* dlogits, float* loss_out,
                         const e2_nll_weights* wts);
int e2_head_fwd_w(e2_ctx*, const e2_tensor5* x, const float* w, const float* bias, int ncls,
                  const e2_tensor5* target, const e2_tensor5* probs, float* stats,
                  const e2_nll_weights* wts);
int e2_head_bwd_w(e2_ctx*, const e2_tensor5* x, const float* w, const e2_tensor5* probs,
                  const e2_tensor5* target, const float* stats, const e2_tensor5* dx,
                  int accumulate_dx, float* dw, float* dbias, float* loss_out, void* ws,
                  size_t ws_bytes, const e2_nll_weights* wts);
int e2_tail_fwd_bwd_w(e2_ctx*, const e2_tensor5* x, const float* wp_fwd, const float* wp_dgrad,
                      const float* bias1, int c2, const float* w_head, const float* b_head,
                      int ncls, const e2_tensor5* target, const e2_tensor5* probs,
                      const e2_tensor5* dpre, const e2_tensor5* dx, int gm_mode,
                      const e2_tensor5* gm_src, const float* gm_bias, float* stats, void* ws,
                      size_t ws_bytes, int* n_slots, const e2_nll_weights* wts);

int e2_malis_nll(e2_ctx*, const e2_tensor5* probs, const float* pos, const float* neg,
                 const float* norm, const e2_tensor5* dlogits, float* loss_sum);

int e2_adam_step(e2_ctx*, float* p, const float* g, float* m, float* s,
                 size_t n, const int64_t* seg_off, const float* seg_reg,
                 int n_seg, const float* hyper );
int e2_sgd_step(e2_ctx*, float* p, const float* g, float* d, size_t n,
                const int64_t* seg_off, const float* seg_reg, int n_seg,
                const float* hyper );

int e2_set_loss_grad_mode(e2_ctx*, int sum_mode, float* count_out);

int e2_adam_step_ex(e2_ctx*, float* p, float* g, float* m, float* s, size_t n,
                    const int64_t* seg_off, const float* seg_reg, int n_seg,
                    const float* hyper, const float* gdiv, float gmul, int zero_g);
int e2_sgd_step_ex(e2_ctx*, float* p, float* g, float* d, size_t n, const int64_t* seg_off,
                   const float* seg_reg, int n_seg, const float* hyper, const float* gdiv,
                   float gmul, int zero_g);

size_t e2_upd_job_bytes(void);
size_t e2_upd_rest_bytes(void);
int e2_upd_job_fill(void* rec, long off, void* wp_f, void* wp_d, int cout, int cin, int kd, int kh,
                    int kw, float reg, int tile0, int* ntiles, size_t* lds_bytes);
int e2_upd_rest_fill(void* rec, long off, long n, float reg);
int e2_adam_pack_step(e2_ctx*, float* p, float* g, float* m, float* s, const void* jobs_dev,
                      int njobs, int ntiles, const void* rest_dev, int nrest, float* hyper,
                      const float* gdiv, float gmul, int zero_g, size_t lds_bytes);

typedef struct e2_graph e2_graph;
int e2_graph_begin(e2_ctx*);
int e2_graph_end(e2_ctx*, e2_graph** out);
int e2_graph_launch(e2_ctx*, e2_graph*);
int e2_graph_destroy(e2_graph*);
int e2_graph_debug_dot(e2_graph*, const char* path, int verbose);

int e2_warp_slice(e2_ctx*, const e2_tensor5* src, const float* minv, int perspective,
                  unsigned nearest_mask, const int* dest_off, const float* src_off,
                  const e2_tensor5* dst);
int e2_grey_augment(e2_ctx*, float* d, size_t n, float alpha, float c, float gamma);

int e2_malis_loss_weights(int n_vert, const int32_t* seg, int n_edge, const int32_t* node1,
                          const int32_t* node2, const float* edge_weight, int pos,
                          uint64_t* counts);
int e2_malis_connected_components(int n_vert, int n_edge, const int32_t* node1,
                                  const int32_t* node2, const float* edge_weight,
                                  int size_thresh, int32_t* seg);

typedef struct e2_event e2_event;
int e2_event_create(e2_event** out);
int e2_event_record(e2_ctx*, e2_event*);
int e2_event_elapsed_ms(e2_event* start, e2_event* stop, float* ms);
int e2_event_destroy(e2_event*);
int e2_stream_synchronize(e2_ctx*);
int e2_stream_fork(e2_ctx*, void* side_stream);
int e2_stream_join(e2_ctx*, void* side_stream);

size_t e2_conv3d_bf16_workspace_bytes(int n, int cin, int d, int h, int w, int cout, int kd,
                                      int kh, int kw);
int e2_conv3d_fwd_bf16(e2_ctx*, const e2_tensor5* x, const float* w, int cout, int kd, int kh,
                       int kw, const float* bias, int act, const e2_tensor5* out, void* ws,
                       size_t ws_bytes);
int e2_conv3d_dgrad_bf16(e2_ctx*, const e2_tensor5* dy_pad, const float* w, int cin, int kd,
                         int kh, int kw, const e2_tensor5* dx, void* ws, size_t ws_bytes);
size_t e2_conv3d_wgrad_bf16_workspace_bytes(int n, int cin, int d, int h, int w, int cout,
                                            int kd, int kh, int kw);
int e2_conv3d_wgrad_bf16(e2_ctx*, const e2_tensor5* x, const e2_tensor5* dy, float* dw, int kd,
                         int kh, int kw, int accumulate, void* ws, size_t ws_bytes);
size_t e2_conv3d_bf16_xkeep_bytes(int n, int cin, int d, int h, int w, int kh, int kw);
int e2_conv3d_fwd_bf16_keep(e2_ctx*, const e2_tensor5* x, const float* w, int cout, int kd,
                            int kh, int kw, const float* bias, int act, const e2_tensor5* out,
                            void* ws, size_t ws_bytes, void* xkeep, size_t xkeep_bytes);
int e2_conv3d_wgrad_bf16_xcl(e2_ctx*, const e2_tensor5* x_shape, const void* xcl,
                             int kg_per_plane, const e2_tensor5* dy, float* dw, int kd, int kh,
                             int kw, int accumulate, void* ws, size_t ws_bytes);

typedef struct e2_bf16_dst {
  void* cl;
  int cl_kg, cl_d, cl_h, cl_w;
  int cl_oz, cl_oy, cl_ox;
  void* pl;
  int64_t pl_plane;
  int pl_pitch;
} e2_bf16_dst;
int e2_pool_bias_act_bwd_bf16(e2_ctx*, const e2_tensor5* dout, int64_t part_stride, int parts,
                              const e2_tensor5* src, const float* bias, int pz, int py, int px,
                              int act, const e2_tensor5* dy, float* dbias, const e2_bf16_dst* dst);
int e2_pool_bias_act_fwd_bf16(e2_ctx*, const e2_tensor5* y, int64_t part_stride, int parts,
                              const float* bias, int pz, int py, int px, int act,
                              const e2_tensor5* out, const e2_bf16_dst* dst);
int e2_conv1_pool_act_fwd_bf16(e2_ctx*, const e2_tensor5* x, const float* w, const float* bias,
// ... 67 lines not shown
```

Measured before the change: 522.2 million voxels/s.

## Fuse slot-partial reductions, Adam update, loss stats and next-step input fetch into one kernel

Adds a step-boundary kernel that reduces the per-workgroup partial sums left by the first conv backward and the tail/head backward, applies Adam to the whole parameter vector, writes the loss and history, and copies the next step's input from the ring. The separate reduce kernels, Adam kernel and step prologue are no longer launched. Within a multi-step graph, the input fetch for step j+1 is done at the end of step j. The aim is fewer kernel launches and serial tail kernels per step. In exchange the fused kernel is more complex, relies on a grid-wide arrival counter, and adds capture-time state handling.

```diff
diff --git a/elektronn2_amd/backend.py b/elektronn2_amd/backend.py
--- a/elektronn2_amd/backend.py
+++ b/elektronn2_amd/backend.py
@@ -125,6 +125,8 @@
         "e2_conv1_bwd_workspace_bytes": (C.c_size_t, [i, i, i, i, i, i, i]),
         "e2_conv1_pool_act_bwd": (C.c_int, [vp, P5, fp, fp, P5, i, i, i, i, i, fp, fp,
                                             C.c_void_p, C.c_size_t]),
+        "e2_conv1_pool_act_bwd_slots": (C.c_int, [vp, P5, fp, fp, P5, i, i, i, i, i, fp, fp,
+                                            C.c_void_p, C.c_size_t, C.POINTER(C.c_int)]),
         "e2_pool_bias_act_fwd": (C.c_int, [vp, P5, fp, i, i, i, i, P5]),
         "e2_conv3d_fwd_packed_parts": (C.c_int, [vp, P5, vp, i, i, i, i, P5, C.c_int64, i,
                                                  C.POINTER(C.c_int)]),
@@ -218,6 +220,10 @@
         "e2_adam_step_ex": (C.c_int, [vp, fp, fp, fp, fp, sz, vp, fp, i, fp, fp, C.c_float, i]),
         "e2_sgd_step_ex": (C.c_int, [vp, fp, fp, fp, sz, vp, fp, i, fp, fp, C.c_float, i]),
         "e2_step_prologue": (C.c_int, [vp, fp, i, C.c_size_t, fp, fp, i, fp, i, vp]),
+        "e2_boundary_seg_bytes": (sz, []),
+        "e2_boundary_seg_fill": (C.c_int, [vp, i, C.c_long, i, vp, i, i, i]),
+        "e2_step_boundary": (C.c_int, [vp, fp, fp, fp, fp, sz, vp, fp, i, fp, fp, C.c_float, i, vp, i, i,
+                                       fp, fp, fp, fp, i, fp, i, C.c_size_t, fp, i, vp]),
         "e2_graph_begin": (C.c_int, [vp]),
         "e2_graph_end": (C.c_int, [vp, C.POINTER(vp)]),
         "e2_graph_launch": (C.c_int, [vp, vp]),
@@ -561,15 +567,20 @@
         n, cout, d, ho, wo = (int(v) for v in dout_shape)
         return int(_lib.e2_conv1_bwd_workspace_bytes(n, cout, d, ho, wo, k[1], k[2]))
 
-    def conv1_pool_act_bwd(self, x, w, bias, dout, pool, act, dw, dbias, ws=None):
+    def conv1_pool_act_bwd(self, x, w, bias, dout, pool, act, dw, dbias, ws=None, slots=False):
         if ws is None:
             ws = torch.empty(self.conv1_bwd_ws_bytes(dout.shape, w.shape[2:]) // 4 + 16,
                              dtype=torch.float32, device=self.device)
-        _chk(_lib.e2_conv1_pool_act_bwd(self.h, C.byref(t5(x)), _fp(w), _fp(bias),
-                                        C.byref(t5(dout)), w.shape[3], w.shape[4], pool[1],
-                                        pool[2], ACT[act], _fp(dw), _fp(dbias),
-                                        C.c_void_p(ws.data_ptr()), ws.numel() * 4),
-             "e2_conv1_pool_act_bwd")
+        args = (self.h, C.byref(t5(x)), _fp(w), _fp(bias), C.byref(t5(dout)), w.shape[3], w.shape[4],
+                pool[1], pool[2], ACT[act], _fp(dw), _fp(dbias), C.c_void_p(ws.data_ptr()),
+                ws.numel() * 4)
+        if slots:
+            n_slots = C.c_int(0)
+            _chk(_lib.e2_conv1_pool_act_bwd_slots(*(args + (C.byref(n_slots),))),
+                 "e2_conv1_pool_act_bwd_slots")
+            return int(n_slots.value)
+        _chk(_lib.e2_conv1_pool_act_bwd(*args), "e2_conv1_pool_act_bwd")
+        return 0
 
     def pool_bias_act_fwd(self, y, bias, pool, act, out):
         _chk(_lib.e2_pool_bias_act_fwd(self.h, C.byref(t5(y)), _fp(bias), pool[0], pool[1],
@@ -1047,6 +1058,61 @@
                                    int(hist.shape[0]) if hist is not None else 0,
                                    C.c_void_p(state.data_ptr())), "e2_step_prologue")
 
+    SLOT_PLAIN, SLOT_LOSS, SLOT_FIRST_W, SLOT_FIRST_B = 0, 1, 2, 3
+
+    def make_boundary_segs(self, entries, seg_off=None):
+        if not 0 < len(entries) <= 16:
+            raise ValueError("make_boundary_segs: 1..16 entries, got %d" % len(entries))
+        rec = int(_lib.e2_boundary_seg_bytes())
+        buf = (C.c_char * (rec * len(entries)))()
+        row0, keep = 0, []
+        for n, (kind, off, count, part, first_row, n_slots, taps) in enumerate(entries):
+            off, count, first_row, n_slots, taps = int(off), int(count), int(first_row), int(n_slots), int(taps)
+            if part.dtype != torch.float32 or not part.is_cuda or not part.is_contiguous():
+                raise TypeError("make_boundary_segs: contiguous float32 GPU partial sums are needed")
+            rows = {self.SLOT_FIRST_W: (count // max(taps, 1)) * (taps + 1),
+                    self.SLOT_FIRST_B: count * (taps + 1)}.get(kind, first_row + count)
+            if first_row < 0 or n_slots < 1 or rows * n_slots > part.numel():
+                raise ValueError("make_boundary_segs: entry %d reads %d rows of %d slots out of %d floats"
+                                 % (n, rows, n_slots, part.numel()))
+            if kind != self.SLOT_LOSS and seg_off is not None:
+                so = [int(v) for v in seg_off]
+                if off not in so[:-1] or not any(v >= off + count for v in so) or \
+                        min(v for v in so if v >= off + count) - (off + count) >= 4:
+                    raise ValueError("make_boundary_segs: entry %d [%d, %d) is not a run of whole tensors"
+                                     % (n, off, off + count))
+            ptr = part.data_ptr() + (4 * first_row * n_slots if kind in (self.SLOT_PLAIN, self.SLOT_LOSS) else 0)
+            _chk(_lib.e2_boundary_seg_fill(C.byref(buf, n * rec), int(kind), off, count, C.c_void_p(ptr),
+                                           n_slots, taps, row0), "e2_boundary_seg_fill")
+            row0 += count
+            keep.append(part)
+        dev = torch.frombuffer(bytearray(buf), dtype=torch.uint8).to(self.device)
+        dev.keep = keep
+        return dev, len(entries), row0
+
+    def step_boundary(self, p, g, m, s, seg_off, seg_reg, hyper, segs=None, stats=None, loss_out=None,
+                      count_out=None, hist=None, state=None, ring=None, dst=None, advance=False,
+                      gdiv=None, gmul=1.0, zero_g=False):
+        if state is not None:
+            assert state.dtype == torch.int64 and state.numel() >= 2 and state.is_contiguous()
+        if ring is not None:
+            assert ring.dim() == 2 and ring.is_contiguous() and ring.dtype == torch.float32
+            assert dst is not None and dst.is_contiguous() and dst.numel() >= ring.shape[1]
+        if hist is not None:
+            assert hist.dim() == 2 and hist.is_contiguous() and hist.shape[1] == 1 and state is not None
+        sd, ns, nr = segs if segs is not None else (None, 0, 0)
+        _chk(_lib.e2_step_boundary(self.h, _fp(p), _fp(g), _fp(m), _fp(s), p.numel(),
+                                   C.c_void_p(seg_off.data_ptr()), _fp(seg_reg), seg_reg.numel(),
+                                   _fp(hyper), _fp(gdiv), float(gmul), int(bool(zero_g)),
+                                   C.c_void_p(sd.data_ptr()) if sd is not None else None, ns, nr,
+                                   _fp(stats), _fp(loss_out), _fp(count_out), _fp(hist),
+                                   int(hist.shape[0]) if hist is not None else 0,
+                                   _fp(ring), int(ring.shape[0]) if ring is not None else 0,
+                                   int(ring.shape[1]) if ring is not None else 0, _fp(dst),
+                                   int(bool(advance)),
+                                   C.c_void_p(state.data_ptr()) if state is not None else None),
+             "e2_step_boundary")
+
     def graph_begin(self):
         _chk(_lib.e2_graph_begin(self.h), "e2_graph_begin")
 
diff --git a/elektronn2_amd/csrc/conv_first.hip b/elektronn2_amd/csrc/conv_first.hip
--- a/elektronn2_amd/csrc/conv_first.hip
+++ b/elektronn2_amd/csrc/conv_first.hip
@@ -276,10 +276,29 @@
   return sizeof(float) * std::max(valu, e2i_firstm_ws_floats(tilesM, cout, kh * kw));
 }
 
+static int conv1_bwd(e2_ctx* ctx, const e2_tensor5* x, const float* w, const float* bias,
+                     const e2_tensor5* dout, int kh, int kw, int py, int px, int act, float* dw,
+                     float* dbias, void* ws, size_t ws_bytes, int* n_slots);
+
 extern "C" int e2_conv1_pool_act_bwd(e2_ctx* ctx, const e2_tensor5* x, const float* w,
                                      const float* bias, const e2_tensor5* dout, int kh, int kw,
                                      int py, int px, int act, float* dw, float* dbias,
                                      void* ws, size_t ws_bytes) {
+  return conv1_bwd(ctx, x, w, bias, dout, kh, kw, py, px, act, dw, dbias, ws, ws_bytes, nullptr);
+}
+
+extern "C" int e2_conv1_pool_act_bwd_slots(e2_ctx* ctx, const e2_tensor5* x, const float* w,
+                                           const float* bias, const e2_tensor5* dout, int kh,
+                                           int kw, int py, int px, int act, float* dw,
+                                           float* dbias, void* ws, size_t ws_bytes, int* n_slots) {
+  E2_REQUIRE(n_slots, "conv1_pool_act_bwd_slots: null argument");
+  *n_slots = 0;
+  return conv1_bwd(ctx, x, w, bias, dout, kh, kw, py, px, act, dw, dbias, ws, ws_bytes, n_slots);
+}
+
+static int conv1_bwd(e2_ctx* ctx, const e2_tensor5* x, const float* w, const float* bias,
+                     const e2_tensor5* dout, int kh, int kw, int py, int px, int act, float* dw,
+                     float* dbias, void* ws, size_t ws_bytes, int* n_slots) {
   E2_REQUIRE(ctx && w && bias && dw && dbias && ws, "conv1_pool_act_bwd: null argument");
   const int v = first_supported(1, kh, kw, 1, py, px);
   E2_REQUIRE(v, "conv1_pool_act_bwd: unsupported kernel/pool %dx%d / %dx%d", kh, kw, py, px);
@@ -295,6 +314,7 @@
   if (e2i_firstm_mg(p.Cout) && !e2_dbg_env("E2_FIRST_VALU")) {
     int nslots = 0;
     if (int rc = e2i_firstm_bwd(ctx, v, x, w, bias, dout, py, px, act, part, &nslots)) return rc;
+    if (n_slots) { *n_slots = nslots; return 0; }
     const int T = kh * kw, total = p.Cout * (T + 1);
     hipLaunchKernelGGL(first_bwd_reduce_sm_kernel, dim3(e2_cdiv(total, 4)), dim3(256), 0, ctx->stream,
                        part, nslots, p.Cout, T, dw, dbias);
diff --git a/elektronn2_amd/csrc/step_boundary.hip b/elektronn2_amd/csrc/step_boundary.hip
--- /dev/null
+++ b/elektronn2_amd/csrc/step_boundary.hip
@@ -0,0 +1,216 @@
+#include "common.hpp"
+#include <algorithm>
+
+#define E2_EPS_ADAM 1e-5f
+#ifndef E2_EPS_NLL
+#define E2_EPS_NLL 1e-5f
+#endif
+
+namespace {
+
+constexpr int kOptMaxSeg = 1024;
+constexpr int kMaxSlotSeg = 16;
+
+enum { kSlotPlain = 0, kSlotLoss = 1, kSlotFirstW = 2, kSlotFirstB = 3 };
+
+struct SlotSeg {
+  long off;
+  const float* part;
+  int count;
+  int nslots;
+  int kind;
+  int T;
+  int row0;
+  int pad_;
+};
+
+struct BoundaryP {
+  float *p, *g, *m, *s;
+  size_t n;
+  const int64_t* seg_off; const float* seg_reg; int n_seg;
+  float* hyper; const float* gdiv; float gmul; int zero_g;
+  const SlotSeg* segs; int n_slot_seg; int n_rows;
+  float *stats, *loss_out, *count_out, *hist; int hist_slots;
+  const float* ring; int n_slots; long slot_floats; float* dst; int advance;
+  unsigned long long* state;
+};
+
+__device__ __forceinline__ int seg_find_lds(const long* so, int n_seg, size_t i) {
+  int lo = 0, hi = n_seg - 1;
+  while (lo < hi) {
+    const int mid = (lo + hi + 1) >> 1;
+    if ((size_t)so[mid] <= i) lo = mid; else hi = mid - 1;
+  }
+  return lo;
+}
+
+__global__ __launch_bounds__(256) void step_boundary_kernel(BoundaryP q) {
+  __shared__ long so[kOptMaxSeg];
+  __shared__ float sr[kOptMaxSeg];
+  __shared__ unsigned char skip[kOptMaxSeg];
+  __shared__ SlotSeg ss[kMaxSlotSeg];
+  for (int i = threadIdx.x; i < q.n_seg; i += blockDim.x) { so[i] = q.seg_off[i]; sr[i] = q.seg_reg[i]; }
+  if ((int)threadIdx.x < q.n_slot_seg) ss[threadIdx.x] = q.segs[threadIdx.x];
+  const float lr = q.hyper[0], mom = q.hyper[1], b2 = q.hyper[2], wd = q.hyper[3];
+  const float t = q.hyper[4] + 1.f;
+  const float fac = sqrtf(1.f - powf(b2, t)) / (1.f - powf(mom, t));
+  const float gs = q.gdiv ? q.gmul / (q.gdiv[0] + 1e-5f) : q.gmul;
+  const unsigned long long L = q.state ? *(volatile unsigned long long*)q.state : 0ull;
+  __syncthreads();
+  for (int i = threadIdx.x; i < q.n_seg; i += blockDim.x) {
+    unsigned char sk = 0;
+    for (int j = 0; j < q.n_slot_seg; ++j)
+      if (ss[j].kind != kSlotLoss && so[i] >= ss[j].off && so[i] < ss[j].off + ss[j].count) sk = 1;
+    skip[i] = sk;
+  }
+  __syncthreads();
+
+  const int lane = threadIdx.x & 63;
+  for (int r = blockIdx.x * 4 + (threadIdx.x >> 6); r < q.n_rows; r += gridDim.x * 4) {
+    int j = 0;
+    while (j + 1 < q.n_slot_seg && r >= ss[j + 1].row0) ++j;
+    const SlotSeg sg = ss[j];
+    const int e = r - sg.row0;
+    long row = e;
+    if (sg.kind == kSlotFirstW) { const int co = e / sg.T; row = (long)co * (sg.T + 1) + (sg.T - 1 - (e - co * sg.T)); }
+    else if (sg.kind == kSlotFirstB) row = (long)e * (sg.T + 1) + sg.T;
+    const float* src = sg.part + row * sg.nslots;
+    const size_t i = sg.kind == kSlotLoss ? 0 : (size_t)sg.off + e;
+    const float g0 = q.g[i], m0 = q.m[i], s0 = q.s[i], pi = q.p[i];
+    float sum = 0.f;
+#pragma unroll 4
+    for (int b = lane; b < sg.nslots; b += 64) sum += src[b];
+#pragma unroll
+    for (int o = 32; o > 0; o >>= 1) sum += __shfl_xor(sum, o, 64);
+    if (lane != 0) continue;
+    if (sg.kind == kSlotLoss) {
+      const float cnt = q.stats[1];
+      const float loss = sum / (cnt + E2_EPS_NLL);
+      q.stats[0] = sum;
+      if (q.loss_out) q.loss_out[0] = loss;
+      if (q.count_out) q.count_out[0] = cnt;
+      if (q.hist && L > 0) q.hist[(long)((L - 1) % (unsigned long long)q.hist_slots)] = loss;
+      continue;
+    }
+    const float gsum = g0 + sum;
+    const float gi = gsum * gs;
+    q.g[i] = q.zero_g ? 0.f : gsum;
+    const float nm = mom * m0 + (1.f - mom) * gi;
+    const float ns = b2 * s0 + (1.f - b2) * gi * gi;
+    float dir = fac * nm / sqrtf(ns + E2_EPS_ADAM);
+    const float mult = sr[seg_find_lds(so, q.n_seg, i)] * wd;
+    if (mult != 0.f) dir += mult * pi;
+    q.m[i] = nm; q.s[i] = ns; q.p[i] = pi - lr * dir;
+  }
+
+  if (q.ring && q.advance) {
+    const float* src = q.ring + (long)(L % (unsigned long long)q.n_slots) * q.slot_floats;
+    const long n4 = q.slot_floats >> 2;
+    const float4* s4 = reinterpret_cast<const float4*>(src);
+    float4* d4 = reinterpret_cast<float4*>(q.dst);
+    const long stride = gridDim.x * 256L;
+    long i = blockIdx.x * 256L + threadIdx.x;
+    for (; i + 3 * stride < n4; i += 4 * stride) {
+      const float4 a = s4[i], b = s4[i + stride], c = s4[i + 2 * stride], d = s4[i + 3 * stride];
+      d4[i] = a; d4[i + stride] = b; d4[i + 2 * stride] = c; d4[i + 3 * stride] = d;
+    }
+    for (; i < n4; i += stride) d4[i] = s4[i];
+  }
+
+  const size_t n4 = q.n >> 2;
+  float4* p4 = reinterpret_cast<float4*>(q.p);
+  float4* g4 = reinterpret_cast<float4*>(q.g);
+  float4* m4 = reinterpret_cast<float4*>(q.m);
+  float4* s4 = reinterpret_cast<float4*>(q.s);
+  for (size_t i = blockIdx.x * (size_t)blockDim.x + threadIdx.x; i < n4;
+       i += (size_t)gridDim.x * blockDim.x) {
+    const int sgi = seg_find_lds(so, q.n_seg, 4 * i);
+    if (skip[sgi]) continue;
+    float4 gv = g4[i];
+    const float4 mv = m4[i], sv = s4[i];
+    float4 pv = p4[i];
+    if (gs != 1.f) { gv.x *= gs; gv.y *= gs; gv.z *= gs; gv.w *= gs; }
+    if (q.zero_g) g4[i] = make_float4(0.f, 0.f, 0.f, 0.f);
+    const float mult = sr[sgi] * wd;
+    float4 nm, ns;
+#define E2_ADAM1(c)                                                      \
+    nm.c = mom * mv.c + (1.f - mom) * gv.c;                              \
+    ns.c = b2 * sv.c + (1.f - b2) * gv.c * gv.c;                         \
+    {                                                                    \
+      float dir = fac * nm.c / sqrtf(ns.c + E2_EPS_ADAM);                \
+      if (mult != 0.f) dir += mult * pv.c;                               \
+      pv.c = pv.c - lr * dir;                                            \
+    }
+    E2_ADAM1(x) E2_ADAM1(y) E2_ADAM1(z) E2_ADAM1(w)
+#undef E2_ADAM1
+    m4[i] = nm; s4[i] = ns; p4[i] = pv;
+  }
+
+  __syncthreads();
+  if (threadIdx.x == 0) {
+    unsigned* arrivals = reinterpret_cast<unsigned*>(q.hyper + 7);
+    const unsigned prev = __hip_atomic_fetch_add(arrivals, 1u, __ATOMIC_RELAXED, __HIP_MEMORY_SCOPE_AGENT);
+    if (prev == gridDim.x - 1) {
+      __hip_atomic_store(arrivals, 0u, __ATOMIC_RELAXED, __HIP_MEMORY_SCOPE_AGENT);
+      q.hyper[4] = t;
+      q.hyper[5] = fac;
+      if (q.advance) q.state[0] = L + 1;
+    }
+  }
+}
+
+}
+
+extern "C" size_t e2_boundary_seg_bytes(void) { return sizeof(SlotSeg); }
+
+extern "C" int e2_boundary_seg_fill(void* rec, int kind, long off, int count, const void* part,
+                                    int n_slots, int taps, int row0) {
+  E2_REQUIRE(rec && part, "e2_boundary_seg_fill: null argument");
+  E2_REQUIRE(kind >= kSlotPlain && kind <= kSlotFirstB, "e2_boundary_seg_fill: kind %d", kind);
+  E2_REQUIRE(count > 0 && n_slots > 0 && row0 >= 0 && (kind == kSlotLoss || off >= 0),
+             "e2_boundary_seg_fill: bad extent");
+  E2_REQUIRE(kind != kSlotLoss || count == 1, "e2_boundary_seg_fill: the loss is one row");
+  E2_REQUIRE((kind != kSlotFirstW && kind != kSlotFirstB) || taps > 0, "e2_boundary_seg_fill: taps");
+  E2_REQUIRE(kind != kSlotFirstW || count % taps == 0,
+             "e2_boundary_seg_fill: %d weights are no multiple of %d taps", count, taps);
+  SlotSeg* s = (SlotSeg*)rec;
+  s->off = kind == kSlotLoss ? 0 : off; s->part = (const float*)part; s->count = count;
+  s->nslots = n_slots; s->kind = kind; s->T = taps; s->row0 = row0; s->pad_ = 0;
+  return 0;
+}
+
+extern "C" int e2_step_boundary(e2_ctx* ctx, float* p, float* g, float* m, float* s, size_t n,
+                                const int64_t* seg_off, const float* seg_reg, int n_seg,
+                                float* hyper, const float* gdiv, float gmul, int zero_g,
+                                const void* segs_dev, int n_slot_segs, int n_rows, float* stats,
+                                float* loss_out, float* count_out, float* hist, int hist_slots,
+                                const float* ring, int n_slots, size_t slot_floats, float* dst,
+                                int advance, void* state) {
+  E2_REQUIRE(ctx && p && g && m && s && seg_off && seg_reg && hyper && n_seg > 0,
+             "step_boundary: null argument");
+  E2_REQUIRE(n_seg <= kOptMaxSeg, "step_boundary: %d parameter tensors (at most %d)", n_seg, kOptMaxSeg);
+  E2_REQUIRE((((uintptr_t)p | (uintptr_t)g | (uintptr_t)m | (uintptr_t)s) & 15) == 0 && (n & 3) == 0,
+             "step_boundary: arenas must be 16-byte aligned and a multiple of four elements long");
+  E2_REQUIRE(n_slot_segs >= 0 && n_slot_segs <= kMaxSlotSeg && n_rows >= 0 &&
+                 (n_slot_segs == 0) == (n_rows == 0) && (n_slot_segs == 0 || segs_dev),
+             "step_boundary: bad slot table (%d segments, %d rows)", n_slot_segs, n_rows);
+  E2_REQUIRE(n_slot_segs == 0 || stats, "step_boundary: the slot table needs stats");
+  E2_REQUIRE(!hist || (hist_slots > 0 && state), "step_boundary: bad history arguments");
+  E2_REQUIRE(!advance || (state && ((uintptr_t)state & 7) == 0), "step_boundary: null / misaligned state");
+  E2_REQUIRE(!ring || (dst && n_slots > 0 && slot_floats > 0 &&
+                       (((uintptr_t)ring | (uintptr_t)dst) & 15) == 0 && (slot_floats & 3) == 0),
+             "step_boundary: ring / dst must be 16-byte aligned and slots a multiple of 16 bytes");
+  BoundaryP q;
+  q.p = p; q.g = g; q.m = m; q.s = s; q.n = n;
+  q.seg_off = seg_off; q.seg_reg = seg_reg; q.n_seg = n_seg;
+  q.hyper = hyper; q.gdiv = gdiv; q.gmul = gmul; q.zero_g = zero_g ? 1 : 0;
+  q.segs = (const SlotSeg*)segs_dev; q.n_slot_seg = n_slot_segs; q.n_rows = n_rows;
+  q.stats = stats; q.loss_out = loss_out; q.count_out = count_out; q.hist = hist; q.hist_slots = hist_slots;
+  q.ring = ring; q.n_slots = n_slots; q.slot_floats = (long)slot_floats; q.dst = dst;
+  q.advance = advance ? 1 : 0;
+  q.state = (unsigned long long*)state;
+  const int grid = (int)std::min<size_t>(std::max<size_t>((n / 4 + 255) / 256, 1), ctx->num_cu);
+  hipLaunchKernelGGL(step_boundary_kernel, dim3(grid), dim3(256), 0, ctx->stream, q);
+  E2_CHECK_HIP(hipGetLastError());
+  return 0;
+}
diff --git a/elektronn2_amd/neuromancer/loss.py b/elektronn2_amd/neuromancer/loss.py
--- a/elektronn2_amd/neuromancer/loss.py
+++ b/elektronn2_amd/neuromancer/loss.py
@@ -241,6 +241,8 @@
         tail = self._tail(plan)
         if tail is not None:
             par = tail.parent
+            if plan.boundary_on():
+                return
             gm = tail._tail_gm(plan) if plan.needs_grad(par) else None
             plan.ctx.tail_reduce(plan.scratch[tail, 'tail_ws'], plan.scratch[self, 'tail_slots'],
                                  tail.n_f, head.n_f, plan.pgrad(head.w).reshape(head.n_f, -1),
diff --git a/elektronn2_amd/neuromancer/neural.py b/elektronn2_amd/neuromancer/neural.py
--- a/elektronn2_amd/neuromancer/neural.py
+++ b/elektronn2_amd/neuromancer/neural.py
@@ -707,9 +707,12 @@
         if self._fused_first(plan):
             if plan.opt['side_join_first']:
                 plan.join_side()
-            ctx.conv1_pool_act_bwd(x, self._w5(plan.param(self.w)), plan.param(self.b), plan.grad[self],
-                                   self._p3, self.activation_func, plan.pgrad(self.w),
-                                   plan.pgrad(self.b), ws=plan.scratch[self, 'ws1'])
+            bnd = plan.boundary_on() and self.w.apply_train and self.b.apply_train
+            ns = ctx.conv1_pool_act_bwd(x, self._w5(plan.param(self.w)), plan.param(self.b), plan.grad[self],
+                                        self._p3, self.activation_func, plan.pgrad(self.w),
+                                        plan.pgrad(self.b), ws=plan.scratch[self, 'ws1'], slots=bnd)
+            if ns:
+                plan.boundary_first(self, ns)
             return
         dy = plan.scratch[self, 'dy']
         tail = self._tail(plan) is not None
diff --git a/elektronn2_amd/neuromancer/optimiser.py b/elektronn2_amd/neuromancer/optimiser.py
--- a/elektronn2_amd/neuromancer/optimiser.py
+++ b/elektronn2_amd/neuromancer/optimiser.py
@@ -237,6 +237,9 @@
             plan.ctx.adam_pack_step(m.P, m.G, self.momentum, self.squared_accum, plan._upd,
                                     self._hyper, **self._grad_scaling(plan))
             return
+        if plan.boundary_on():
+            plan.emit_boundary(self, **self._grad_scaling(plan))
+            return
         plan.ctx.adam_step(m.P[:m.n_train] if m.n_train < m.P.numel() else m.P, m.G,
                            self.momentum, self.squared_accum, m.seg_off, m.seg_reg,
                            self._hyper, **self._grad_scaling(plan))
diff --git a/elektronn2_amd/neuromancer/options.py b/elektronn2_amd/neuromancer/options.py
--- a/elektronn2_amd/neuromancer/options.py
+++ b/elektronn2_amd/neuromancer/options.py
@@ -50,6 +50,11 @@
                     "wherever the parent's producing launch writes a strided view (no pad launch); off: "
                     "every such conv pads by one e2_pad5 launch per step"),
     "zero_in_update": ("E2_ZERO_IN_UPDATE", _b, True, "the optimiser launch clears the gradient arena (finding 38)"),
+    "step_boundary": ("E2_STEP_BOUNDARY", _b, True,
+                      "single-GPU Adam step with a fused tail: ONE launch (e2_step_boundary) adds up the tail's "
+                      "and the first layer's slot sums, updates the parameters and, inside a run_steps graph, "
+                      "fetches the next step's batch -- instead of two reduce launches, the Adam launch and the "
+                      "next step's prologue (DESIGN finding 57)"),
     "image_stride": ("E2_IMAGE_STRIDE", _b, True,
                      "once a conv launch's tiling is known its packed weight image gets rows as long as that "
                      "tiling's tiles reach (+ 16), not the any-tiling formula (e2_set_image_rows; finding 52)"),
diff --git a/elektronn2_amd/neuromancer/plan.py b/elektronn2_amd/neuromancer/plan.py
--- a/elektronn2_amd/neuromancer/plan.py
+++ b/elektronn2_amd/neuromancer/plan.py
@@ -444,6 +444,10 @@
         self._hist = None
         self._step_state = None
         self._multi = {}
+        self._boundary = None
+        self._boundary_firsts = []
+        self._fetch_ahead = False
+        self._fetched = False
         self._built = True
 
     @property
@@ -554,6 +558,7 @@
             self._pack_dev = self.ctx.make_pack_jobs(jobs, rows, strides)
 
     def _emit_forward(self):
+        self._side_pending, self._side_dirty = None, False
         if self._upd is not None:
             if self._pack_dev_up is not None:
                 self.on_side(lambda: self.ctx.conv3d_pack_multi(*self._pack_dev_up), always=True)
@@ -592,6 +597,7 @@
             if not self._upd_zeroes_g():
                 self.zero_early(self.model.G)
             self._grad_written = set()
+            self._boundary_firsts = []
         drop = self._drop_ids
         for n in nodes:
             if id(n) in drop:
@@ -636,6 +642,68 @@
         if self.step in ('Adam', 'SGD'):
             self.model.optimisers[self.step].device_update(self)
 
+    def _boundary_nll(self):
+        m = self.model
+        if not (self.opt['step_boundary'] and self.step == 'Adam' and self._upd is None
+                and m.G.is_cuda and m.n_train >= 4 and m.n_train % 4 == 0):
+            return None
+        ln = self.loss_node
+        kids = ln.parent if isinstance(ln.parent, (list, tuple)) else [ln.parent]
+        if len(kids) != 1 or type(kids[0]).__name__ != 'MultinoulliNLL':
+            return None
+        nll = kids[0]
+        tail = nll._tail(self)
+        if tail is None or self._loss_dev().data_ptr() != self.scratch[nll, 'loss'].data_ptr():
+            return None
+        head, par = nll.pred._head(self), tail.parent
+        ps = [head.w, head.b, tail.b] + ([par.b] if self.needs_grad(par) and tail._tail_gm(self) is not None else [])
+        if not all(getattr(p, 'apply_train', False) and id(p) in m._slots for p in ps):
+            return None
+        return nll
+
+    def boundary_on(self):
+        return getattr(self, '_boundary', None) is not None
+
+    def boundary_first(self, node, n_slots):
+        self._boundary_firsts.append((node, int(n_slots)))
+
+    def _boundary_table(self):
+        m, ctx, nll = self.model, self.ctx, self._boundary
+        tail, head = nll._tail(self), nll.pred._head(self)
+        par = tail.parent
+        ws, nwg = self.scratch[tail, 'tail_ws'], int(self.scratch[nll, 'tail_slots'])
+        nc, c2 = int(head.n_f), int(tail.n_f)
+        off = lambda p: m._slots[id(p)][0]
+        ent = [(ctx.SLOT_PLAIN, off(head.w), nc * c2, ws, 0, nwg, 0),
+               (ctx.SLOT_PLAIN, off(head.b), nc, ws, nc * c2, nwg, 0),
+               (ctx.SLOT_PLAIN, off(tail.b), c2, ws, nc * c2 + nc, nwg, 0),
+               (ctx.SLOT_LOSS, 0, 1, ws, nc * c2 + nc + c2, nwg, 0)]
+        if self.needs_grad(par) and tail._tail_gm(self) is not None:
+            ent.append((ctx.SLOT_PLAIN, off(par.b), m._slots[id(par.b)][1], ws, nc * c2 + nc + c2 + 1, nwg, 0))
+        for node, ns in self._boundary_firsts:
+            taps = int(np.prod(self._w5(self.param(node.w)).shape[2:]))
+            ent.append((ctx.SLOT_FIRST_W, off(node.w), m._slots[id(node.w)][1], self.scratch[node, 'ws1'], 0, ns, taps))
+            ent.append((ctx.SLOT_FIRST_B, off(node.b), m._slots[id(node.b)][1], self.scratch[node, 'ws1'], 0, ns, taps))
+        key = tuple((e[0], e[1], e[2], e[3].data_ptr(), e[4], e[5], e[6]) for e in ent)
+        tabs = self.scratch.setdefault('boundary_tables', {})
+        if key not in tabs:
+            if self._capturing:
+                raise RuntimeError("step boundary: the slot table must exist before capture")
+            seg_off = [m._slots[id(p)][0] for p in m._param_list if p.apply_train] + [m.n_train]
+            tabs[key] = ctx.make_boundary_segs(ent, seg_off)
+        return tabs[key]
+
+    def emit_boundary(self, opt, **scaling):
+        m, nll = self.model, self._boundary
+        ahead = bool(self._fetch_ahead)
+        self.ctx.step_boundary(m.P[:m.n_train] if m.n_train < m.P.numel() else m.P, m.G,
+                               opt.momentum, opt.squared_accum, m.seg_off, m.seg_reg, opt._hyper,
+                               segs=self._boundary_table(), stats=self.scratch[nll.pred, 'stats'],
+                               loss_out=self.scratch[nll, 'loss'],
+                               hist=self._hist, state=self._step_state,
+                               ring=self._ring if ahead else None,
+                               dst=self.input_arena if ahead else None, advance=ahead, **scaling)
+
     def _upd_zeroes_g(self):
         return (self.training and self.step in ('Adam', 'SGD') and bool(self.opt['zero_in_update']))
 
@@ -680,6 +748,7 @@
         self._dp_scale_mode = self._dp_scale_now()
         host = [n for n in self.nodes if hasattr(n, '_plan_host')]
         upd = self.training and self.step in ('Adam', 'SGD')
+        self._boundary = self._boundary_nll() if (upd and not dp and not host) else None
         segs = []
         if host:
             def host_steps():
@@ -774,6 +843,7 @@
                         self._emit_seg(i, emit, zero_jobs)
                     except BaseException:
                         self._capturing = False
+                        self._side_pending, self._side_dirty = None, False
                         try:
                             ctx.graph_destroy(ctx.graph_end())
                         except Exception:
@@ -800,14 +870,18 @@
         ctx.record(self._ev0)
         if not capture:
             self._zero_seen = []
-        for i, (emit, after) in enumerate(self._segs):
-            self._seg_idx = i
-            if capture:
-                ctx.graph_launch(self._graphs[i])
-            else:
-                self._emit_seg(i, emit, None)
-            if after is not None:
-                after()
+        try:
+            for i, (emit, after) in enumerate(self._segs):
+                self._seg_idx = i
+                if capture:
+                    ctx.graph_launch(self._graphs[i])
+                else:
+                    self._emit_seg(i, emit, None)
+                if after is not None:
+                    after()
+        except BaseException:
+            self._side_pending, self._side_dirty = None, False
+            raise
         ctx.record(self._ev1)
         self._calls += 1
         if self.training:
@@ -819,9 +893,10 @@
         ctx = self.ctx
         if i == 0 and self._drop_nodes:
             ctx.dropout_tick(self.model.dropout_state_dev())
-        if i == 0 and (self._ring is not None or self._hist is not None):
+        if i == 0 and (self._ring is not None or self._hist is not None) and not self._fetched:
+            hist = None if self.boundary_on() else self._hist
             ctx.step_prologue(self._step_state, ring=self._ring, dst=self.input_arena,
-                              src=self._loss_dev() if self._hist is not None else None, hist=self._hist)
+                              src=self._loss_dev() if hist is not None else None, hist=hist)
         if zero_jobs and i in zero_jobs:
             ctx.fill_multi(*zero_jobs[i])
         emit()
@@ -925,10 +1000,14 @@
                     self._capturing = True
                     ctx.graph_begin()
                     try:
-                        for _ in range(k):
+                        for j in range(k):
+                            self._fetched = self.boundary_on() and j > 0
+                            self._fetch_ahead = self.boundary_on() and j < k - 1
                             self._emit_seg(0, emit, self._zero_keep)
                     except BaseException:
                         self._capturing = False
+                        self._fetched = self._fetch_ahead = False
+                        self._side_pending, self._side_dirty = None, False
                         try:
                             ctx.graph_destroy(ctx.graph_end())
                         except Exception:
@@ -936,6 +1015,7 @@
                         raise
                     g = ctx.graph_end()
                     self._capturing = False
+                    self._fetched = self._fetch_ahead = False
                     self._multi[k] = g
                 ctx.record(self._ev0)
                 ctx.graph_launch(g)
diff --git a/include/e2hip.h b/include/e2hip.h
--- a/include/e2hip.h
+++ b/include/e2hip.h
@@ -84,6 +84,10 @@
                           const float* bias, const e2_tensor5* dout, int kh,
                           int kw, int py, int px, int act, float* dw, float* dbias,
                           void* ws, size_t ws_bytes);
+int e2_conv1_pool_act_bwd_slots(e2_ctx*, const e2_tensor5* x, const float* w,
+                                const float* bias, const e2_tensor5* dout, int kh,
+                                int kw, int py, int px, int act, float* dw, float* dbias,
+                                void* ws, size_t ws_bytes, int* n_slots);
 
 int e2_conv3d_fwd_packed_parts(e2_ctx*, const e2_tensor5* x, const void* wp, int cout, int kd,
                                int kh, int kw, const e2_tensor5* y, int64_t part_stride,
@@ -154,6 +158,15 @@
 
 int e2_step_prologue(e2_ctx*, const float* ring, int n_slots, size_t slot_floats, float* dst,
                      const float* src, int n_vals, float* hist, int hist_slots, void* state);
+size_t e2_boundary_seg_bytes(void);
+int e2_boundary_seg_fill(void* rec, int kind, long off, int count, const void* part, int n_slots,
+                         int taps, int row0);
+int e2_step_boundary(e2_ctx*, float* p, float* g, float* m, float* s, size_t n,
+                     const int64_t* seg_off, const float* seg_reg, int n_seg, float* hyper,
+                     const float* gdiv, float gmul, int zero_g, const void* segs_dev,
+                     int n_slot_segs, int n_rows, float* stats, float* loss_out, float* count_out,
+                     float* hist, int hist_slots, const float* ring, int n_slots,
+                     size_t slot_floats, float* dst, int advance, void* state);
 int e2_set_input_slack(e2_ctx*, int bytes);
 int e2_conv_last_zero_fill(const e2_ctx*, void** ptr, size_t* n);
 int e2_set_dgrad_zinset(e2_ctx*, int planes);
```

New measurement: 525.2 million voxels/s, median of 6. About the same (+0.6%).
